# IGNF/StrataNet2-Vegetation-Coverage-Maps

Hardware: AMD Instinct MI355X
Metric: plots/s fwd+bwd, 32k-pt synthetic plots, batch 16/GPU (higher is better)
Workload: dtype f32; 1 GPU; C2 ref-arch: 16 plots/GPU x 32768 pts, SA npoint 1024/256 + global, r 1/2 m, train step fwd+P2+loss+bwd+Adam, inputs resident in HBM; plots_per_gpu=16, points_per_plot=32768, batches_per_geometry_pass=8, exchange=none (single GPU), parallelism=single GPU, ranks_seen=1, exchange_in_graph=False

## Files before the change

include/strata_hip.h:

```cpp
#ifndef STRATA_HIP_H
#define STRATA_HIP_H

#include <stddef.h>

#ifdef __cplusplus
extern "C" {
#endif

#define SN2_VERSION 102
#define SN2_EINVAL (-1)
#define SN2_ELIMIT (-2)

#define SN2_MAX_NEIGHBORS 2000
#define SN2_STAT_SLOTS 1024

int sn2_version(void);
int sn2_debug_mfma_chain(const float *a, const float *b, float *d, int mode, void *stream);
int sn2_debug_spin(int blocks, long long clocks, int *out, void *stream);

int sn2_debug_fp1_backward_parts(int mask);
int sn2_debug_fp_rows_form(int form);
int sn2_debug_fp_table_form(int form);
#define SN2_PROBE_SINK_WORDS 4096
int sn2_debug_stream_probe(const float *src, float *dst, size_t n_floats, int mode, float *sink, void *stream);
int sn2_debug_mfma_probe(int mode, int iters, float *sink, double *flops, void *stream);

typedef struct sn2_block {
    int cin, cout;
    const float *W, *b;
    const float *gamma, *beta;
    float *running_mean, *running_var;
    float *a, *c;
    float *mean, *invstd;
    float *stat_slots;
    float *dW, *db, *dgamma, *dbeta;
    int grad_replicas, grad_replica_stride;
    int mma_bf16;
    long long *num_batches_tracked;
    int frozen_stats;
} sn2_block;
#define SN2_BN_FROZEN_KEEP 2
int sn2_grad_reduce(float *flat, int n, int replicas, int stride, void *stream);


int sn2_pack_rows(const float *cloud, const float *xyz, int B, int C, int N, float *rows0, void *stream);

#define SN2_FPS_WS_WORDS(B, N) (6L * (B) * (N) + (4104L + 4096L) * (B) + 32L)
int sn2_fps(const float *pos_soa, int B, int N, int M, const int *start, int *idx, float *cpos_soa,
            float *cpos_aos, int *order_ws, void *stream);
int sn2_fps_waves(const float *pos_soa, int B, int N, int M, const int *start, int *idx, float *cpos_soa,
                  float *cpos_aos, int *order_ws, int waves, void *stream);
int sn2_fps_status(const float *pos_soa, int B, int N, int M, const int *start, int *idx, float *cpos_soa,
                   float *cpos_aos, int *order_ws, int waves, unsigned *status, void *stream);
int sn2_debug_fps_spin_limit(unsigned sweeps);

int sn2_ball_query(const float *src_soa, int B, int N, const float *cpos_soa, int M, float r2, int cap,
                   int *nbr, int *cnt, unsigned long long *total, const int *fps_ws, void *stream);

int sn2_count_sum(const int *cnt, int n, unsigned long long *total, void *stream);
int sn2_count_sum_group(const int *cnt, int G, int n, unsigned long long *total, size_t total_stride, void *stream);

#define SN2_THREE_NN_WS_WORDS(B, S) ((size_t)(B) * (4 * (size_t)(S) + 1032))
int sn2_three_nn(const float *src_soa, int B, int S, const float *dst_soa, int T, int k, int *idx, float *w,
                 void *ws, const int *dst_fps_ws, void *stream);
#define SN2_THREE_NN_XY_WS_WORDS(B, S, T) ((size_t)(B) * (4 * (size_t)(S) + 5 * (size_t)(T) + 1032))
int sn2_three_nn_xy(const float *src_soa, int B, int S, const float *dst_soa, int T, int k, int *idx, float *w,
                    void *ws, void *stream);

int sn2_prepare_plots(const float *raw, long T, const int *offsets, const float *centers, const float *fake_xy, int n_fake,
                      const int *idx, int B, int N, int train, const double *rot, const int *flips, const float *noise,
                      const long *noise_offsets, long noise_T, float z_max, float *cloud, float *xyz, void *stream);

#define SN2_SUBSAMPLE_LDS 1
#define SN2_SUBSAMPLE_GLOBAL 2
#define SN2_SUBSAMPLE_COARSE 4
#define SN2_SUBSAMPLE_LDS_MAX 16384
int sn2_subsample_form(int n_max, int N);
size_t sn2_subsample_ws_words(int B, int n_max, int N, int form);
int sn2_subsample(const int *offsets, int extra, int n_max, int B, int N, unsigned long long seed, const long long *plot_keys,
                  int form, int *ws, size_t ws_words, int *idx, void *stream);

#define SN2_ZNORM_WS_WORDS(n, cells) ((size_t)5 * (n) + 3 * (size_t)(cells) + 8)
int sn2_znorm(const float *x, const float *y, const float *z, int n, float radius, float x_min, float y_min, float x_max,
              float y_max, int *ws, float *zmin, float *z_out, void *stream);

size_t sn2_parcel_count_ws_words(int P, int rows);
size_t sn2_parcel_znorm_ws_words(long T, float radius, float x_min, float y_min, float x_max, float y_max);
int sn2_parcel_count(const float *cloud, long T, int L, int rows, const float *centers, int P, const int *cell_start,
                     const int *cell_items, int GX, int GY, double gx0, double gy0, double cell_inv, float radius, int *ws,
                     size_t ws_words, int *prefix, long long *total, void *stream);
int sn2_parcel_fill(const float *cloud, long T, int L, int rows, const float *centers, int P, const int *cell_start,
                    const int *cell_items, int GX, int GY, double gx0, double gy0, double cell_inv, float radius, int *prefix,
                    const int *plot_base, long sum_n, float *raw, int *point_index, void *stream);
int sn2_parcel_znorm(const float *cloud, long T, float x_min, float y_min, float x_max, float y_max, float radius,
                     float disc_radius, const int *offsets, const float *centers, int P, const int *point_index, long sum_n,
                     int *ws, size_t ws_words, float *raw, void *stream);

typedef struct sn2_sa {
    int B, Nsrc, M, cap;
    int cf;
    int nl;
    const float *feat; int feat_stride;
    const float *spos; int spos_stride;
    const float *cpos;
    const int *nbr, *cnt;
    const unsigned long long *total;
    const int *order;
    sn2_block blk[2];
    float *ext; int *arg;
    float *out;
    const float *dout;
    float *dfeat;
} sn2_sa;
#define SN2_SA_SOLO_MIN 64
#define SN2_SA_QUAD_MIN 8
#define SN2_SA_OCT_MIN 4
#define SN2_SA_SOLO_FLAG 0x40000000
#define SN2_SA_OCT_FLAG 0x20000000
#define SN2_SA_PACKED_ITEMS(M) ((M) / 8 + 2)
#define SN2_SA_ORDER_WORDS(B, M) ((size_t)4 * (B) * (M) + (size_t)16 * (B) * SN2_SA_PACKED_ITEMS(M) + 8)
int sn2_sa_order(const int *cnt, int B, int M, int *order, void *stream);
int sn2_sa_order_group(const int *cnt, int G, int B, int M, int *order, size_t stride_words, void *stream);
int sn2_sa_forward(const sn2_sa *p, int training, void *stream);
int sn2_sa_backward(const sn2_sa *p, void *stream);

typedef struct sn2_fp {
    int B, R_per_plot, S_per_plot;
    int ca, cb;
    const float *src; int src_stride; const float *src_a, *src_c;
    const int *knn_idx; const float *knn_w;
    const float *skip; int skip_stride;
    sn2_block blk;
    float *h; int h_stride;
    const float *dy;
    float *dsrc; int dsrc_stride;
    float *dskip; int dskip_stride;
    float *du_scratch;
    float *scatter_ws;
    int scatter_ready;
    const int *bn_sums_done;
    float *src_ws;
    int act_bf16;
    const int *row_perm;
} sn2_fp;
#define SN2_INTERP_CHUNKS(R, S) ((3 * (size_t)(R) + 62) / 63 + (size_t)(S))
#define SN2_FP_SRC_WS_WORDS(B, R, S, cout) ((size_t)(B) * SN2_INTERP_CHUNKS(R, S) * ((((cout) + 3) / 4) * 4))
#define SN2_INTERP_WS_WORDS(B, R, S) \
    ((size_t)(B) * (S) * (((R) + 2047) / 2048 + 6) + 6 * (size_t)(B) * (R) + 64 + 4 * (size_t)(B) * SN2_INTERP_CHUNKS(R, S))
int sn2_interp_index(const int *knn_idx, const float *knn_w, const float *src_pos, int B, int R_per_plot,
                     int S_per_plot, float *ws, void *stream);
int sn2_interp_index_perm(const int *knn_idx, const float *knn_w, const float *src_pos, const int *row_perm, int B,
                          int R_per_plot, int S_per_plot, float *ws, void *stream);
int sn2_interp_index_group(const int *knn_idx, const float *knn_w, const float *src_pos, const int *row_perm, int G, int B,
                           int R_per_plot, int S_per_plot, float *ws, size_t ws_stride_words, void *stream);
int sn2_fp_forward(const sn2_fp *p, int training, void *stream);
int sn2_fp_backward(const sn2_fp *p, void *stream);

int sn2_plot_max_forward(const float *h, const float *a, const float *c, int B, int R_per_plot, int C, float *out,
                         int *arg, void *stream);
int sn2_plot_max_backward(const float *dout, const int *arg, int B, int R_per_plot, int C, float *dy, void *stream);

int sn2_global_pool_backward(const float *du, int du_stride, const int *arg, const float *h, const float *mean,
                             const float *invstd, int B, int R_per_plot, int C, float *dx, float *dy, float *dgamma,
                             float *dbeta, void *stream);

#define SN2_GLOBAL_XCHG_WORDS(B) ((size_t)2 * (size_t)(B) * 4 * 128)
#define SN2_GLOBAL_CTL_WORDS 8
int sn2_global_level_forward(const sn2_fp *sa3, const sn2_fp *fp3, float *x3, int *arg3, unsigned long long *xchg,
                             unsigned *ctl, void *stream);
int sn2_debug_global_spin_limit(unsigned sweeps);

typedef struct sn2_head {
    int R, cin, f_stride;
    const float *f, *fa, *fc;
    const float *W1, *b1, *W2, *b2;
    float *coverages, *proba;
    const float *dcoverages, *dproba;
    float *dy;
    float *dW1, *db1, *dW2, *db2;
    int grad_replicas, grad_replica_stride;
    const int *drop_mask;
    float drop_scale;
    int act_bf16;
    float *zero_fill; long zero_fill_words;
} sn2_head;
int sn2_head_forward(const sn2_head *p, void *stream);
int sn2_fp_head_eval(const sn2_fp *p, const sn2_head *hd, void *stream);
int sn2_head_backward(const sn2_head *p, void *stream);
int sn2_head_bn_sums(const sn2_head *p, const float *gamma, const float *beta, const float *mean, const float *invstd,
                     float *dgamma, float *dbeta, int *ok, void *stream);
int sn2_fp_bn_sums(const sn2_fp *p, const float *gamma, const float *beta, const float *mean, const float *invstd,
                   float *dgamma, float *dbeta, int *ok, void *stream);


int sn2_plot_project_forward(const float *pred_pointwise, const float *cloud_xy, long plot_stride, int B, int N,
                             int D, unsigned long long *keys, int *pix, int *arg, int *nocc, float *pred,
                             void *stream);
#define SN2_P2_KEY_PARTS(N) (((N) + 4095) / 4096 < 1 ? 1 : (((N) + 4095) / 4096 > 64 ? 64 : ((N) + 4095) / 4096))
int sn2_plot_pixels(const float *cloud_xy, long plot_stride, int B, int N, int D, float *mm, int *pix, void *stream);
int sn2_plot_project_forward_pix(const float *pred_pointwise, const int *pix, int B, int N, int D,
                                 unsigned long long *keys, int *arg, int *nocc, float *pred, void *stream);
int sn2_plot_project_backward(const float *dpred, const int *arg, const int *nocc, const int *pix, int B, int N,
                              int D, float *dpointwise, void *stream);

int sn2_raster_project(const float *coverages, const float *cloud_xy, long plot_stride, int B, int N, int D,
                       int diam_meters, unsigned long long *keys, int *pix, float *rasters, void *stream);

int sn2_mosaic_merge(const float *rasters, const float *weights, const int *offsets, int B, int D, int H, int W,
                     float *mean, float *wsum, int win_y0, int win_x0, int win_h, int win_w, void *stream);

#define SN2_MOSAIC_HIST_WORDS 10004
int sn2_mosaic_finalize(const float *mean, const float *wsum, int H, int W, int *hist_ws, double *sum_ws, float *thr_out,
                        float *out, void *stream);

int sn2_kde_lookup(const float *cloud, int B, int C, int N, int z_channel, float z_max, const double *X, const double *Y,
                   int K, double *pdf, void *stream);
#define SN2_KDE_FIT_MAX_K 65536
#define SN2_KDE_FIT_ABS_SLOTS 256
#define SN2_KDE_FIT_SLICES 8
#define SN2_KDE_FIT_WS_WORDS(K) \
    (2 * ((4 + 3 * SN2_KDE_FIT_SLICES) * (size_t)(K) + 3 * (((size_t)(K) + 255) / 256)) + SN2_KDE_FIT_ABS_SLOTS)
int sn2_kde_fit(const float *z, long n, double bw, int K, void *ws, double *X, double *Y, void *stream);
#define SN2_LOSS_BLOCKS 1024
int sn2_loss_forward(const float *pred, const double *gt, int B, const float *proba, const double *pdf, int R, double m,
                     double e, double *partials, double *out, void *stream);
int sn2_loss_backward(const float *pred, const double *gt, int B, const float *proba, const double *pdf, int R, double m,
                      double e, const double *grad_total, float *dpred, float *dproba, void *stream);

#define SN2_PROJECTED_LOSS_WS (2 * 512 + 2)
int sn2_projected_loss_forward(const float *coverages, const int *pix, const float *proba, const double *pdf, const double *gt,
                               int B, int N, int D, double m, double e, unsigned long long *keys, int *arg, int *nocc,
                               float *pred, double *partials, double *out, void *stream);
int sn2_projected_loss_backward(const float *pred, const double *gt, int B, const float *proba, const double *pdf, int N, int D,
                                double m, double e, const double *grad_total, const int *arg, const int *nocc, const int *pix,
                                float *dcoverages, float *dproba, void *stream);

#define SN2_PLOT_LOSSES_SLICE_ROWS 2048
#define SN2_PLOT_LOSSES_SLICES(N) \
    (((N) + SN2_PLOT_LOSSES_SLICE_ROWS - 1) / SN2_PLOT_LOSSES_SLICE_ROWS < 1 ? 1 : \
     (((N) + SN2_PLOT_LOSSES_SLICE_ROWS - 1) / SN2_PLOT_LOSSES_SLICE_ROWS > 64 ? 64 : ((N) + SN2_PLOT_LOSSES_SLICE_ROWS - 1) / SN2_PLOT_LOSSES_SLICE_ROWS))
size_t sn2_plot_losses_ws_words(int B, int N, int D);
int sn2_plot_losses(const float *coverages, const int *pix, const float *proba, const double *pdf, const double *gt, int B, int N,
                    int D, double m, double e, void *ws, float *pred, double *out, void *stream);

int sn2_adam_step(float *param, const float *grad, float *exp_avg, float *exp_avg_sq, int n, float lr, float beta1,
                  float beta2, float eps, float weight_decay, int *step_dev ,
                  float grad_scale, void *stream);


typedef struct sn2_net_layer {
    int cin, cout;
    const float *W, *b, *gamma, *beta;
    float *running_mean, *running_var;
    long long *num_batches_tracked;
    int gW, gb, ggamma, gbeta;
    int mma_bf16;
} sn2_net_layer;

typedef struct sn2_net_model {
    sn2_net_layer sa1[2], sa2, sa3, fp3, fp2, fp1;
    const float *lin1_W, *lin1_b, *lin2_W, *lin2_b;
    int g_lin1_W, g_lin1_b, g_lin2_W, g_lin2_b;
    int n_flat;
    float r1_sq, r2_sq;
    int max_neighbors;
    float drop_p;
    int fuse_global_level;
    int fuse_eval_head;
    int source_side;
    int fps_waves_shared, fps_waves_many;
} sn2_net_model;

typedef struct sn2_net_dims {
    int B, N, M1, M2;
    int cap1, cap2;
    int act_bf16;
    int p2_diam_pix;
} sn2_net_dims;

typedef struct sn2_net_geo {
    const float *xyz;
    int *idx1; float *pos1_soa, *pos1_aos; int *ws1;
    int *nbr1, *cnt1; unsigned long long *tot1; int *ord1;
    int *idx2; float *pos2_soa, *pos2_aos; int *ws2;
    int *nbr2, *cnt2; unsigned long long *tot2; int *ord2;
    const float *pos3;
    int *knn3_idx; float *knn3_w;
    int *knn2_idx; float *knn2_w;
    int *knn1_idx; float *knn1_w;
    float *inv3, *inv2, *inv1;
    int *nn_ws2, *nn_ws1;
    const int *rank1;
    float *rows0;
    int *p2_pix; float *p2_mm;
} sn2_net_geo;

typedef struct sn2_net_act {
    float *aux;
    float *stats;
    float *ext1; int *arg1; float *x1;
    float *ext2; int *arg2; float *x2;
    float *h_sa3, *h3;
    float *x3; int *arg3;
    float *h2;
    void *h1;
    float *src_ws1, *src_ws2;
    float *cov, *proba;
    const int *drop_mask;
    float *bwd_arena; long bwd_arena_words;
} sn2_net_act;

typedef struct sn2_net_bwd {
    const float *dcov, *dproba;
    float *arena; long arena_words;
    int images, image_stride;
    float *dy2, *dy3, *dx1, *dx2, *dx3, *dy_sa3;
    void *dy1, *du1;
    float *du2, *du3;
    int *bn_ok;
    float *src_ws1, *src_ws2;
    int defer_grad_reduce;
    int arena_is_zero;
    int frozen_stats;
} sn2_net_bwd;

#define SN2_NET_FORK 1
#define SN2_NET_SHARED 2
#define SN2_NET_INVERTED 4
#define SN2_NET_DEFER_JOIN 8
#define SN2_NET_INPUT_ONLY 16
#define SN2_NET_HAS_ROWS0 32
#define SN2_NET_JOIN_PENDING 64
#define SN2_NET_WITH_GEOMETRY 128
#define SN2_NET_HAS_INVERTED 256

typedef struct sn2_net_io {
    const float *cloud;
    const int *fps_start;
    unsigned *fps_status;
    unsigned long long *gl_xchg; unsigned *gl_ctl;
    void *stream_b, *stream_c, *stream_pack;
    void *ctx;
    int flags;
    int training;
} sn2_net_io;

int sn2_net_ctx_create(void **ctx);
int sn2_net_ctx_destroy(void *ctx);
int sn2_net_geo_carve(const sn2_net_model *m, const sn2_net_dims *d, void *base, sn2_net_geo *out, size_t *bytes);
int sn2_net_act_carve(const sn2_net_model *m, const sn2_net_dims *d, int training, void *base, sn2_net_act *out, size_t *bytes);
int sn2_net_bwd_carve(const sn2_net_model *m, const sn2_net_dims *d, void *arena_base, void *scratch_base, sn2_net_bwd *out,
                      size_t *arena_bytes, size_t *scratch_bytes);
int sn2_net_geometry(const sn2_net_model *m, const sn2_net_dims *d, const sn2_net_geo *g, const sn2_net_io *io, void *stream);
int sn2_net_forward(const sn2_net_model *m, const sn2_net_dims *d, const sn2_net_geo *g, const sn2_net_act *a,
                    const sn2_net_io *io, void *stream);
int sn2_net_backward(const sn2_net_model *m, const sn2_net_dims *d, const sn2_net_geo *g, const sn2_net_act *a,
                     const sn2_net_bwd *b, void *stream);

int sn2_adam_step_images(float *param, float *grad_images, int replicas, int stride, float *exp_avg, float *exp_avg_sq, int n,
                         float lr, float beta1, float beta2, float eps, float weight_decay, int *step_dev, float grad_scale,
                         void *stream);

#ifdef __cplusplus
}
#endif
#endif
```

stratanet2_vegetation_coverage_maps_amd/_lib.py:

```python
import ctypes
import os
from ctypes import POINTER, Structure, c_double, c_float, c_int, c_long, c_longlong, c_void_p

HERE = os.path.dirname(os.path.abspath(__file__))
LIB_PATH = os.path.join(HERE, "csrc", "libstrata_hip.so")

SN2_VERSION = 102
MAX_NEIGHBORS = 2000
STAT_SLOTS = 1024


class Block(Structure):
    _fields_ = [("cin", c_int), ("cout", c_int), ("W", c_void_p), ("b", c_void_p), ("gamma", c_void_p),
                ("beta", c_void_p), ("running_mean", c_void_p), ("running_var", c_void_p), ("a", c_void_p),
                ("c", c_void_p), ("mean", c_void_p), ("invstd", c_void_p), ("stat_slots", c_void_p),
                ("dW", c_void_p), ("db", c_void_p), ("dgamma", c_void_p), ("dbeta", c_void_p),
                ("grad_replicas", c_int), ("grad_replica_stride", c_int), ("mma_bf16", c_int),
                ("num_batches_tracked", c_void_p), ("frozen_stats", c_int)]


BN_FROZEN_KEEP = 2


class SA(Structure):
    _fields_ = [("B", c_int), ("Nsrc", c_int), ("M", c_int), ("cap", c_int), ("cf", c_int), ("nl", c_int),
                ("feat", c_void_p), ("feat_stride", c_int), ("spos", c_void_p), ("spos_stride", c_int),
                ("cpos", c_void_p), ("nbr", c_void_p), ("cnt", c_void_p), ("total", c_void_p), ("order", c_void_p),
                ("blk", Block * 2),
                ("ext", c_void_p), ("arg", c_void_p), ("out", c_void_p), ("dout", c_void_p), ("dfeat", c_void_p)]


class FP(Structure):
    _fields_ = [("B", c_int), ("R_per_plot", c_int), ("S_per_plot", c_int), ("ca", c_int), ("cb", c_int),
                ("src", c_void_p), ("src_stride", c_int), ("src_a", c_void_p), ("src_c", c_void_p),
                ("knn_idx", c_void_p), ("knn_w", c_void_p), ("skip", c_void_p), ("skip_stride", c_int),
                ("blk", Block), ("h", c_void_p), ("h_stride", c_int), ("dy", c_void_p), ("dsrc", c_void_p),
                ("dsrc_stride", c_int), ("dskip", c_void_p), ("dskip_stride", c_int), ("du_scratch", c_void_p),
                ("scatter_ws", c_void_p), ("scatter_ready", c_int), ("bn_sums_done", c_void_p), ("src_ws", c_void_p),
                ("act_bf16", c_int), ("row_perm", c_void_p)]


class Head(Structure):
    _fields_ = [("R", c_int), ("cin", c_int), ("f_stride", c_int), ("f", c_void_p), ("fa", c_void_p),
                ("fc", c_void_p), ("W1", c_void_p), ("b1", c_void_p), ("W2", c_void_p), ("b2", c_void_p),
                ("coverages", c_void_p), ("proba", c_void_p), ("dcoverages", c_void_p), ("dproba", c_void_p),
                ("dy", c_void_p), ("dW1", c_void_p), ("db1", c_void_p), ("dW2", c_void_p), ("db2", c_void_p),
                ("grad_replicas", c_int), ("grad_replica_stride", c_int), ("drop_mask", c_void_p), ("drop_scale", c_float),
                ("act_bf16", c_int), ("zero_fill", c_void_p), ("zero_fill_words", c_long)]


class NetLayer(Structure):
    _fields_ = [("cin", c_int), ("cout", c_int), ("W", c_void_p), ("b", c_void_p), ("gamma", c_void_p), ("beta", c_void_p),
                ("running_mean", c_void_p), ("running_var", c_void_p), ("num_batches_tracked", c_void_p),
                ("gW", c_int), ("gb", c_int), ("ggamma", c_int), ("gbeta", c_int), ("mma_bf16", c_int)]


class NetModel(Structure):
    _fields_ = [("sa1", NetLayer * 2), ("sa2", NetLayer), ("sa3", NetLayer), ("fp3", NetLayer), ("fp2", NetLayer), ("fp1", NetLayer),
                ("lin1_W", c_void_p), ("lin1_b", c_void_p), ("lin2_W", c_void_p), ("lin2_b", c_void_p),
                ("g_lin1_W", c_int), ("g_lin1_b", c_int), ("g_lin2_W", c_int), ("g_lin2_b", c_int), ("n_flat", c_int),
                ("r1_sq", c_float), ("r2_sq", c_float), ("max_neighbors", c_int), ("drop_p", c_float),
                ("fuse_global_level", c_int), ("fuse_eval_head", c_int), ("source_side", c_int),
                ("fps_waves_shared", c_int), ("fps_waves_many", c_int)]


class NetDims(Structure):
    _fields_ = [("B", c_int), ("N", c_int), ("M1", c_int), ("M2", c_int), ("cap1", c_int), ("cap2", c_int), ("act_bf16", c_int),
                ("p2_diam_pix", c_int)]


class NetGeo(Structure):
    _fields_ = [(n, c_void_p) for n in (
        "xyz", "idx1", "pos1_soa", "pos1_aos", "ws1", "nbr1", "cnt1", "tot1", "ord1",
        "idx2", "pos2_soa", "pos2_aos", "ws2", "nbr2", "cnt2", "tot2", "ord2", "pos3",
        "knn3_idx", "knn3_w", "knn2_idx", "knn2_w", "knn1_idx", "knn1_w", "inv3", "inv2", "inv1", "nn_ws2", "nn_ws1",
        "rank1", "rows0", "p2_pix", "p2_mm")]


class NetAct(Structure):
    _fields_ = [(n, c_void_p) for n in (
        "aux", "stats", "ext1", "arg1", "x1", "ext2", "arg2", "x2", "h_sa3", "h3", "x3", "arg3", "h2", "h1", "src_ws1", "src_ws2",
        "cov", "proba", "drop_mask", "bwd_arena")] + [("bwd_arena_words", c_long)]


class NetBwd(Structure):
    _fields_ = [("dcov", c_void_p), ("dproba", c_void_p), ("arena", c_void_p), ("arena_words", c_long), ("images", c_int),
                ("image_stride", c_int)] + [(n, c_void_p) for n in (
                    "dy2", "dy3", "dx1", "dx2", "dx3", "dy_sa3", "dy1", "du1", "du2", "du3", "bn_ok", "src_ws1", "src_ws2")] + [
                        ("defer_grad_reduce", c_int), ("arena_is_zero", c_int), ("frozen_stats", c_int)]


class NetIO(Structure):
    _fields_ = [("cloud", c_void_p), ("fps_start", c_void_p), ("fps_status", c_void_p), ("gl_xchg", c_void_p), ("gl_ctl", c_void_p),
                ("stream_b", c_void_p), ("stream_c", c_void_p), ("stream_pack", c_void_p), ("ctx", c_void_p), ("flags", c_int),
                ("training", c_int)]


NET_FORK, NET_SHARED, NET_INVERTED, NET_DEFER_JOIN, NET_INPUT_ONLY = 1, 2, 4, 8, 16
NET_HAS_ROWS0, NET_JOIN_PENDING, NET_WITH_GEOMETRY, NET_HAS_INVERTED = 32, 64, 128, 256


SIGNATURES = {
    "sn2_version": [],
    "sn2_debug_mfma_chain": [c_void_p, c_void_p, c_void_p, c_int, c_void_p],
    "sn2_debug_spin": [c_int, c_longlong, c_void_p, c_void_p],
    "sn2_debug_fp1_backward_parts": [c_int],
    "sn2_debug_fp_rows_form": [c_int],
    "sn2_debug_fp_table_form": [c_int],
    "sn2_debug_stream_probe": [c_void_p, c_void_p, ctypes.c_size_t, c_int, c_void_p, c_void_p],
    "sn2_debug_mfma_probe": [c_int, c_int, c_void_p, POINTER(c_double), c_void_p],
    "sn2_pack_rows": [c_void_p, c_void_p, c_int, c_int, c_int, c_void_p, c_void_p],
    "sn2_fps": [c_void_p, c_int, c_int, c_int, c_void_p, c_void_p, c_void_p, c_void_p, c_void_p, c_void_p],
    "sn2_fps_waves": [c_void_p, c_int, c_int, c_int, c_void_p, c_void_p, c_void_p, c_void_p, c_void_p, c_int, c_void_p],
    "sn2_fps_status": [c_void_p, c_int, c_int, c_int, c_void_p, c_void_p, c_void_p, c_void_p, c_void_p, c_int, c_void_p, c_void_p],
    "sn2_debug_fps_spin_limit": [ctypes.c_uint],
    "sn2_ball_query": [c_void_p, c_int, c_int, c_void_p, c_int, c_float, c_int, c_void_p, c_void_p, c_void_p, c_void_p,
                       c_void_p],
    "sn2_three_nn": [c_void_p, c_int, c_int, c_void_p, c_int, c_int, c_void_p, c_void_p, c_void_p, c_void_p, c_void_p],
    "sn2_count_sum": [c_void_p, c_int, c_void_p, c_void_p],
    "sn2_count_sum_group": [c_void_p, c_int, c_int, c_void_p, ctypes.c_size_t, c_void_p],
    "sn2_three_nn_xy": [c_void_p, c_int, c_int, c_void_p, c_int, c_int, c_void_p, c_void_p, c_void_p, c_void_p],
    "sn2_prepare_plots": [c_void_p, c_long, c_void_p, c_void_p, c_void_p, c_int, c_void_p, c_int, c_int, c_int, c_void_p,
                          c_void_p, c_void_p, c_void_p, c_long, c_float, c_void_p, c_void_p, c_void_p],
    "sn2_znorm": [c_void_p, c_void_p, c_void_p, c_int, c_float, c_float, c_float, c_float, c_float, c_void_p, c_void_p,
                  c_void_p, c_void_p],
    "sn2_parcel_count": [c_void_p, c_long, c_int, c_int, c_void_p, c_int, c_void_p, c_void_p, c_int, c_int, c_double, c_double,
                         c_double, c_float, c_void_p, ctypes.c_size_t, c_void_p, c_void_p, c_void_p],
    "sn2_parcel_fill": [c_void_p, c_long, c_int, c_int, c_void_p, c_int, c_void_p, c_void_p, c_int, c_int, c_double, c_double,
                        c_double, c_float, c_void_p, c_void_p, c_long, c_void_p, c_void_p, c_void_p],
    "sn2_parcel_znorm": [c_void_p, c_long, c_float, c_float, c_float, c_float, c_float, c_float, c_void_p, c_void_p, c_int,
                         c_void_p, c_long, c_void_p, ctypes.c_size_t, c_void_p, c_void_p],
    "sn2_subsample_form": [c_int, c_int],
    "sn2_subsample": [c_void_p, c_int, c_int, c_int, c_int, ctypes.c_ulonglong, c_void_p, c_int, c_void_p, ctypes.c_size_t,
                      c_void_p, c_void_p],
    "sn2_sa_order": [c_void_p, c_int, c_int, c_void_p, c_void_p],
    "sn2_sa_order_group": [c_void_p, c_int, c_int, c_int, c_void_p, ctypes.c_size_t, c_void_p],
    "sn2_sa_forward": [POINTER(SA), c_int, c_void_p],
    "sn2_sa_backward": [POINTER(SA), c_void_p],
    "sn2_grad_reduce": [c_void_p, c_int, c_int, c_int, c_void_p],
    "sn2_interp_index": [c_void_p, c_void_p, c_void_p, c_int, c_int, c_int, c_void_p, c_void_p],
    "sn2_interp_index_perm": [c_void_p, c_void_p, c_void_p, c_void_p, c_int, c_int, c_int, c_void_p, c_void_p],
    "sn2_interp_index_group": [c_void_p, c_void_p, c_void_p, c_void_p, c_int, c_int, c_int, c_int, c_void_p, ctypes.c_size_t, c_void_p],
    "sn2_fp_forward": [POINTER(FP), c_int, c_void_p],
    "sn2_fp_backward": [POINTER(FP), c_void_p],
    "sn2_plot_max_forward": [c_void_p, c_void_p, c_void_p, c_int, c_int, c_int, c_void_p, c_void_p, c_void_p],
    "sn2_plot_max_backward": [c_void_p, c_void_p, c_int, c_int, c_int, c_void_p, c_void_p],
    "sn2_global_pool_backward": [c_void_p, c_int, c_void_p, c_void_p, c_void_p, c_void_p, c_int, c_int, c_int, c_void_p, c_void_p,
                                 c_void_p, c_void_p, c_void_p],
    "sn2_global_level_forward": [POINTER(FP), POINTER(FP), c_void_p, c_void_p, c_void_p, c_void_p, c_void_p],
    "sn2_debug_global_spin_limit": [ctypes.c_uint],
    "sn2_head_forward": [POINTER(Head), c_void_p],
    "sn2_fp_head_eval": [POINTER(FP), POINTER(Head), c_void_p],
    "sn2_fp_bn_sums": [POINTER(FP), c_void_p, c_void_p, c_void_p, c_void_p, c_void_p, c_void_p, c_void_p, c_void_p],
    "sn2_head_bn_sums": [POINTER(Head), c_void_p, c_void_p, c_void_p, c_void_p, c_void_p, c_void_p, c_void_p, c_void_p],
    "sn2_head_backward": [POINTER(Head), c_void_p],
    "sn2_plot_project_forward": [c_void_p, c_void_p, c_long, c_int, c_int, c_int, c_void_p, c_void_p, c_void_p,
                                 c_void_p, c_void_p, c_void_p],
    "sn2_plot_pixels": [c_void_p, c_long, c_int, c_int, c_int, c_void_p, c_void_p, c_void_p],
    "sn2_plot_project_forward_pix": [c_void_p, c_void_p, c_int, c_int, c_int, c_void_p, c_void_p, c_void_p, c_void_p, c_void_p],
    "sn2_plot_project_backward": [c_void_p, c_void_p, c_void_p, c_void_p, c_int, c_int, c_int, c_void_p, c_void_p],
    "sn2_raster_project": [c_void_p, c_void_p, c_long, c_int, c_int, c_int, c_int, c_void_p, c_void_p, c_void_p,
                           c_void_p],
    "sn2_mosaic_merge": [c_void_p, c_void_p, c_void_p, c_int, c_int, c_int, c_int, c_void_p, c_void_p,
                         c_int, c_int, c_int, c_int, c_void_p],
    "sn2_mosaic_finalize": [c_void_p, c_void_p, c_int, c_int, c_void_p, c_void_p, c_void_p, c_void_p, c_void_p],
    "sn2_kde_lookup": [c_void_p, c_int, c_int, c_int, c_int, c_float, c_void_p, c_void_p, c_int, c_void_p, c_void_p],
    "sn2_kde_fit": [c_void_p, c_long, c_double, c_int, c_void_p, c_void_p, c_void_p, c_void_p],
    "sn2_loss_forward": [c_void_p, c_void_p, c_int, c_void_p, c_void_p, c_int, c_double, c_double, c_void_p, c_void_p,
                         c_void_p],
    "sn2_loss_backward": [c_void_p, c_void_p, c_int, c_void_p, c_void_p, c_int, c_double, c_double, c_void_p, c_void_p,
                          c_void_p, c_void_p],
    "sn2_adam_step": [c_void_p, c_void_p, c_void_p, c_void_p, c_int, c_float, c_float, c_float, c_float, c_float,
                      c_void_p, c_float, c_void_p],
    "sn2_projected_loss_forward": [c_void_p, c_void_p, c_void_p, c_void_p, c_void_p, c_int, c_int, c_int, c_double, c_double, c_void_p,
                                   c_void_p, c_void_p, c_void_p, c_void_p, c_void_p, c_void_p],
    "sn2_projected_loss_backward": [c_void_p, c_void_p, c_int, c_void_p, c_void_p, c_int, c_int, c_double, c_double, c_void_p, c_void_p,
                                    c_void_p, c_void_p, c_void_p, c_void_p, c_void_p],
    "sn2_plot_losses": [c_void_p, c_void_p, c_void_p, c_void_p, c_void_p, c_int, c_int, c_int, c_double, c_double, c_void_p, c_void_p,
                        c_void_p, c_void_p],
    "sn2_adam_step_images": [c_void_p, c_void_p, c_int, c_int, c_void_p, c_void_p, c_int, c_float, c_float, c_float, c_float, c_float,
                             c_void_p, c_float, c_void_p],
    "sn2_net_ctx_create": [POINTER(c_void_p)],
    "sn2_net_ctx_destroy": [c_void_p],
    "sn2_net_geo_carve": [POINTER(NetModel), POINTER(NetDims), c_void_p, POINTER(NetGeo), POINTER(ctypes.c_size_t)],
    "sn2_net_act_carve": [POINTER(NetModel), POINTER(NetDims), c_int, c_void_p, POINTER(NetAct), POINTER(ctypes.c_size_t)],
    "sn2_net_bwd_carve": [POINTER(NetModel), POINTER(NetDims), c_void_p, c_void_p, POINTER(NetBwd), POINTER(ctypes.c_size_t),
                          POINTER(ctypes.c_size_t)],
    "sn2_net_geometry": [POINTER(NetModel), POINTER(NetDims), POINTER(NetGeo), POINTER(NetIO), c_void_p],
    "sn2_net_forward": [POINTER(NetModel), POINTER(NetDims), POINTER(NetGeo), POINTER(NetAct), POINTER(NetIO), c_void_p],
    "sn2_net_backward": [POINTER(NetModel), POINTER(NetDims), POINTER(NetGeo), POINTER(NetAct), POINTER(NetBwd), c_void_p],
}

SIZE_HELPERS = {
    "sn2_parcel_count_ws_words": [c_int, c_int],
    "sn2_parcel_znorm_ws_words": [c_long, c_float, c_float, c_float, c_float, c_float],
    "sn2_subsample_ws_words": [c_int, c_int, c_int, c_int],
    "sn2_plot_losses_ws_words": [c_int, c_int, c_int],
}

_lib = None


class StrataHipError(RuntimeError):
    pass


def load():
    global _lib
    if _lib is not None:
        return _lib
    if not os.path.exists(LIB_PATH):
        raise StrataHipError(
            f"{LIB_PATH} not found: build it with `python -m stratanet2_vegetation_coverage_maps_amd._build` "
            "(or __graft_entry__.build()); the HIP library is mandatory, there is no fallback path")
    lib = ctypes.CDLL(LIB_PATH)
    for name, argtypes in SIGNATURES.items():
        fn = getattr(lib, name)
        fn.argtypes = argtypes
        fn.restype = c_int
    for name, argtypes in SIZE_HELPERS.items():
        fn = getattr(lib, name)
        fn.argtypes = argtypes
        fn.restype = ctypes.c_size_t
    if lib.sn2_version() != SN2_VERSION:
        raise StrataHipError(f"libstrata_hip.so version {lib.sn2_version()} != binding {SN2_VERSION}: rebuild")
    _lib = lib
    return lib


def check(rc: int, what: str):
    if rc != 0:
        kind = "hipError_t" if rc > 0 else {-1: "SN2_EINVAL", -2: "SN2_ELIMIT"}.get(rc, "error")
        raise StrataHipError(f"{what} failed: {kind} {rc}")
```

stratanet2_vegetation_coverage_maps_amd/csrc/net.hip:

```cpp
#include "common.h"

#include <cstring>
#include <new>

namespace {

constexpr int WIDTHS[7] = {16, 16, 32, 64, 64, 34, 34};
constexpr int WIDTH_SUM = 260;
constexpr int GRAD_IMAGES = 32;

struct NetCtx {
    hipEvent_t fork, b_tables, b_nn, b_done, c_nn, c_done, pack_fork, packed;
};

inline long rows_stat_limit() { return 64L * SN2_STAT_SLOTS; }

inline bool fps_fills_ws(int B, int N, int m) {
    const bool many_small = N <= 4096 && B > 32;
    return N > 2048 && !many_small && m > 16 && ((long)B * N) % 4 == 0 && N <= 131072;
}
inline bool three_nn_uses_grid(int S, int T) { return S >= 128 && S <= 8192 && T > 2048; }
inline bool fp_src_ws_wanted(const sn2_net_model* m, long R, int cb, bool force) {
    return m->source_side && cb > 0 && cb <= 16 && cb % 4 == 0 && (R > rows_stat_limit() || force);
}

struct Carver {
    uintptr_t base;
    size_t off = 0;
    explicit Carver(void* b) : base(reinterpret_cast<uintptr_t>(b)) {}
    template <class T>
    T* take(size_t n_elems) {
        off = (off + 255) & ~(size_t)255;
        T* p = reinterpret_cast<T*>(base + off);
        off += n_elems * sizeof(T);
        return p;
    }
    size_t bytes() const { return (off + 255) & ~(size_t)255; }
};

int check_dims(const sn2_net_model* m, const sn2_net_dims* d) {
    if (!m || !d) return SN2_EINVAL;
    if (d->B <= 0 || d->N <= 0 || d->M1 <= 0 || d->M2 <= 0 || d->M1 > d->N || d->M2 > d->M1) return SN2_EINVAL;
    if (m->max_neighbors <= 0) return SN2_EINVAL;
    const int c1 = m->max_neighbors < d->N ? m->max_neighbors : d->N, c2 = m->max_neighbors < d->M1 ? m->max_neighbors : d->M1;
    if (d->cap1 != c1 || d->cap2 != c2) return SN2_EINVAL;
    if ((long)d->B * d->N >= (1L << 31) / 64) return SN2_ELIMIT;
    const int cin[7] = {11, 16, 19, 35, 96, 80, 42};
    const sn2_net_layer* L[7] = {&m->sa1[0], &m->sa1[1], &m->sa2, &m->sa3, &m->fp3, &m->fp2, &m->fp1};
    for (int i = 0; i < 7; ++i)
        if (L[i]->cin != cin[i] || L[i]->cout != WIDTHS[i]) return SN2_ELIMIT;
    return 0;
}

int check_model_ptrs(const sn2_net_model* m) {
    const sn2_net_layer* L[7] = {&m->sa1[0], &m->sa1[1], &m->sa2, &m->sa3, &m->fp3, &m->fp2, &m->fp1};
    for (int i = 0; i < 7; ++i)
        if (!L[i]->W || !L[i]->b || !L[i]->gamma || !L[i]->beta || !L[i]->running_mean || !L[i]->running_var) return SN2_EINVAL;
    if (!m->lin1_W || !m->lin1_b || !m->lin2_W || !m->lin2_b) return SN2_EINVAL;
    return 0;
}

struct GradDst {
    float* flat;
    int stride;
    int frozen;
};

void fill_block(sn2_block* blk, const sn2_net_layer* L, int k, const sn2_net_act* a, GradDst g) {
    int aux_off = 0, st_off = 0;
    for (int i = 0; i < k; ++i) aux_off += 4 * WIDTHS[i], st_off += SN2_STAT_SLOTS * 2 * WIDTHS[i];
    const int c = L->cout;
    blk->cin = L->cin, blk->cout = c;
    blk->W = L->W, blk->b = L->b, blk->gamma = L->gamma, blk->beta = L->beta;
    blk->running_mean = L->running_mean, blk->running_var = L->running_var;
    float* aux = a->aux + aux_off;
    blk->a = aux, blk->c = aux + c, blk->mean = aux + 2 * c, blk->invstd = aux + 3 * c;
    blk->stat_slots = a->stats + st_off;
    blk->mma_bf16 = L->mma_bf16 ? 1 : 0;
    blk->num_batches_tracked = L->num_batches_tracked;
    blk->frozen_stats = g.frozen;
    if (g.flat) {
        blk->dW = g.flat + L->gW, blk->db = g.flat + L->gb, blk->dgamma = g.flat + L->ggamma, blk->dbeta = g.flat + L->gbeta;
        blk->grad_replicas = GRAD_IMAGES, blk->grad_replica_stride = g.stride;
    } else {
        blk->dW = blk->db = blk->dgamma = blk->dbeta = nullptr;
        blk->grad_replicas = 1, blk->grad_replica_stride = 0;
    }
}

inline float* aux_row(const sn2_net_act* a, int k, int row) {
    int off = 0;
    for (int i = 0; i < k; ++i) off += 4 * WIDTHS[i];
    return a->aux + off + row * WIDTHS[k];
}

void sa1_desc(sn2_sa* s, const sn2_net_model* m, const sn2_net_dims* d, const sn2_net_geo* g, const sn2_net_act* a,
              GradDst gd, const float* dout) {
    memset(s, 0, sizeof(*s));
    s->B = d->B, s->Nsrc = d->N, s->M = d->M1, s->cap = d->cap1, s->cf = 8, s->nl = 2;
    s->feat = g->rows0, s->feat_stride = 12, s->spos = g->rows0 + 8, s->spos_stride = 12;
    s->cpos = g->pos1_aos, s->nbr = g->nbr1, s->cnt = g->cnt1, s->total = g->tot1, s->order = g->ord1;
    fill_block(&s->blk[0], &m->sa1[0], 0, a, gd);
    fill_block(&s->blk[1], &m->sa1[1], 1, a, gd);
    s->ext = a->ext1, s->arg = a->arg1, s->out = a->x1;
    s->dout = dout, s->dfeat = nullptr;
}
void sa2_desc(sn2_sa* s, const sn2_net_model* m, const sn2_net_dims* d, const sn2_net_geo* g, const sn2_net_act* a,
              GradDst gd, const float* dout, float* dfeat) {
    memset(s, 0, sizeof(*s));
    s->B = d->B, s->Nsrc = d->M1, s->M = d->M2, s->cap = d->cap2, s->cf = 16, s->nl = 1;
    s->feat = a->x1, s->feat_stride = 16, s->spos = g->pos1_aos, s->spos_stride = 4;
    s->cpos = g->pos2_aos, s->nbr = g->nbr2, s->cnt = g->cnt2, s->total = g->tot2, s->order = g->ord2;
    fill_block(&s->blk[0], &m->sa2, 2, a, gd);
    s->ext = a->ext2, s->arg = a->arg2, s->out = a->x2;
    s->dout = dout, s->dfeat = dfeat;
}

struct FpIn {
    int k;
    const sn2_net_layer* L;
    int Rp, Sp, ca, cb;
    const float* src; int src_stride; const float *src_a, *src_c;
    const int* knn_idx; const float* knn_w;
    const float* skip; int skip_stride;
    void* h;
    float* src_ws;
    int act_bf16;
};
void fp_desc(sn2_fp* p, const sn2_net_dims* d, const sn2_net_act* a, const FpIn& in, GradDst gd) {
    memset(p, 0, sizeof(*p));
    p->B = d->B, p->R_per_plot = in.Rp, p->S_per_plot = in.Sp, p->ca = in.ca, p->cb = in.cb;
    p->src = in.src, p->src_stride = in.src_stride, p->src_a = in.src_a, p->src_c = in.src_c;
    p->knn_idx = in.knn_idx, p->knn_w = in.knn_w;
    p->skip = in.cb > 0 ? in.skip : nullptr, p->skip_stride = in.cb > 0 ? in.skip_stride : 0;
    fill_block(&p->blk, in.L, in.k, a, gd);
    if ((long)d->B * in.Rp > rows_stat_limit()) p->blk.mma_bf16 = 0;
    p->h = static_cast<float*>(in.h), p->h_stride = (in.L->cout + 3) / 4 * 4;
    p->src_ws = in.src_ws;
    p->act_bf16 = in.act_bf16;
}

FpIn sa3_in(const sn2_net_model* m, const sn2_net_dims* d, const sn2_net_geo* g, const sn2_net_act* a) {
    FpIn in{};
    in.k = 3, in.L = &m->sa3, in.Rp = d->M2, in.Sp = d->M2, in.ca = 32, in.cb = 3;
    in.src = a->x2, in.src_stride = 32;
    in.skip = g->pos2_aos, in.skip_stride = 4;
    in.h = a->h_sa3;
    return in;
}
FpIn fp3_in(const sn2_net_model* m, const sn2_net_dims* d, const sn2_net_geo* g, const sn2_net_act* a) {
    FpIn in{};
    in.k = 4, in.L = &m->fp3, in.Rp = d->M2, in.Sp = 1, in.ca = 64, in.cb = 32;
    in.src = a->x3, in.src_stride = 64;
    in.knn_idx = g->knn3_idx, in.knn_w = g->knn3_w;
    in.skip = a->x2, in.skip_stride = 32;
    in.h = a->h3;
    return in;
}
FpIn fp2_in(const sn2_net_model* m, const sn2_net_dims* d, const sn2_net_geo* g, const sn2_net_act* a, float* src_ws) {
    FpIn in{};
    in.k = 5, in.L = &m->fp2, in.Rp = d->M1, in.Sp = d->M2, in.ca = 64, in.cb = 16;
    in.src = a->h3, in.src_stride = 64, in.src_a = aux_row(a, 4, 0), in.src_c = aux_row(a, 4, 1);
    in.knn_idx = g->knn2_idx, in.knn_w = g->knn2_w;
    in.skip = a->x1, in.skip_stride = 16;
    in.h = a->h2;
    in.src_ws = src_ws;
    return in;
}
FpIn fp1_in(const sn2_net_model* m, const sn2_net_dims* d, const sn2_net_geo* g, const sn2_net_act* a, float* src_ws) {
    FpIn in{};
    in.k = 6, in.L = &m->fp1, in.Rp = d->N, in.Sp = d->M1, in.ca = 34, in.cb = 8;
    in.src = a->h2, in.src_stride = 36, in.src_a = aux_row(a, 5, 0), in.src_c = aux_row(a, 5, 1);
    in.knn_idx = g->knn1_idx, in.knn_w = g->knn1_w;
    in.skip = g->rows0, in.skip_stride = 12;
    in.h = a->h1;
    in.src_ws = src_ws;
    in.act_bf16 = d->act_bf16;
    return in;
}

void head_desc(sn2_head* h, const sn2_net_model* m, const sn2_net_dims* d, const sn2_net_act* a, int training) {
    memset(h, 0, sizeof(*h));
    h->R = d->B * d->N, h->cin = 34, h->f_stride = 36;
    h->f = static_cast<const float*>(a->h1), h->fa = aux_row(a, 6, 0), h->fc = aux_row(a, 6, 1);
    h->W1 = m->lin1_W, h->b1 = m->lin1_b, h->W2 = m->lin2_W, h->b2 = m->lin2_b;
    h->coverages = a->cov, h->proba = a->proba;
    h->grad_replicas = 1, h->grad_replica_stride = 0;
    h->act_bf16 = d->act_bf16;
    if (training && a->drop_mask) {
        h->drop_mask = a->drop_mask;
        h->drop_scale = m->drop_p < 1.f ? 1.f / (1.f - m->drop_p) : 0.f;
    } else {
        h->drop_mask = nullptr, h->drop_scale = 1.f;
    }
}

#define NET_HIP(expr)                                         \
    do {                                                      \
        hipError_t e__ = (expr);                              \
        if (e__ != hipSuccess) return (int)e__;               \
    } while (0)

int inverted_tables(const sn2_net_dims* d, const sn2_net_geo* g, int which, void* st) {
    if (which == 3) {
        SN2_TRY(sn2_count_sum(g->cnt1, d->B * d->M1, g->tot1, st));
        SN2_TRY(sn2_count_sum(g->cnt2, d->B * d->M2, g->tot2, st));
    }
    if (which & 1) {
        if (!g->inv3 || !g->inv2) return SN2_EINVAL;
        SN2_TRY(sn2_interp_index_perm(g->knn3_idx, g->knn3_w, nullptr, nullptr, d->B, d->M2, 1, g->inv3, st));
        SN2_TRY(sn2_interp_index_perm(g->knn2_idx, g->knn2_w, nullptr, nullptr, d->B, d->M1, d->M2, g->inv2, st));
    }
    if (which & 2) {
        if (!g->inv1) return SN2_EINVAL;
        SN2_TRY(sn2_interp_index_perm(g->knn1_idx, g->knn1_w, g->pos1_aos, g->rank1, d->B, d->N, d->M1, g->inv1, st));
    }
    return 0;
}

int check_geo(const sn2_net_dims* d, const sn2_net_geo* g) {
    if (!g || !g->xyz || !g->idx1 || !g->pos1_soa || !g->pos1_aos || !g->nbr1 || !g->cnt1 || !g->tot1 || !g->ord1 || !g->idx2 ||
        !g->pos2_soa || !g->pos2_aos || !g->nbr2 || !g->cnt2 || !g->tot2 || !g->ord2 || !g->pos3 || !g->knn3_idx || !g->knn3_w ||
        !g->knn2_idx || !g->knn2_w || !g->knn1_idx || !g->knn1_w || !g->rows0)
        return SN2_EINVAL;
    return 0;
}
int check_geo_workspaces(const sn2_net_dims* d, const sn2_net_geo* g) {
    if (three_nn_uses_grid(d->M2, d->M1) && !g->nn_ws2) return SN2_EINVAL;
    if (three_nn_uses_grid(d->M1, d->N) && !g->nn_ws1) return SN2_EINVAL;
    return 0;
}

int three_nn_any(const float* src, int B, int S, const float* dst, int T, int k, int* idx, float* w, int* ws, void* st) {
    if (three_nn_uses_grid(S, T)) return sn2_three_nn_xy(src, B, S, dst, T, k, idx, w, ws, st);
    return sn2_three_nn(src, B, S, dst, T, k, idx, w, nullptr, nullptr, st);
}

int geometry_impl(const sn2_net_model* m, const sn2_net_dims* d, const sn2_net_geo* g, const sn2_net_io* io, int flags,
                  hipStream_t cur) {
    const int B = d->B, N = d->N, M1 = d->M1, M2 = d->M2;
    NetCtx* ctx = static_cast<NetCtx*>(io->ctx);
    const bool fork = (flags & SN2_NET_FORK) && ctx && io->stream_b && io->stream_c;
    const bool inverted = flags & SN2_NET_INVERTED;
    const int* start0 = io->fps_start;
    const int* start1 = io->fps_start ? io->fps_start + B : nullptr;
    int* ws1 = fps_fills_ws(B, N, M1) ? g->ws1 : nullptr;
    int* ws2 = fps_fills_ws(B, M1, M2) ? g->ws2 : nullptr;
    int waves = 0;
    if (flags & SN2_NET_SHARED) waves = B > 32 ? m->fps_waves_many : m->fps_waves_shared;
    SN2_TRY(sn2_fps_status(g->xyz, B, N, M1, start0, g->idx1, g->pos1_soa, g->pos1_aos, ws1, waves, io->fps_status, cur));
    hipStream_t sb = cur, sc = cur;
    if (fork) {
        sb = (hipStream_t)io->stream_b, sc = (hipStream_t)io->stream_c;
        NET_HIP(hipEventRecord(ctx->fork, cur));
        NET_HIP(hipStreamWaitEvent(sb, ctx->fork, 0));
        NET_HIP(hipStreamWaitEvent(sc, ctx->fork, 0));
    }
    SN2_TRY(sn2_fps_status(g->pos1_soa, B, M1, M2, start1, g->idx2, g->pos2_soa, g->pos2_aos, ws2, 0, io->fps_status, sb));
    SN2_TRY(sn2_ball_query(g->pos1_soa, B, M1, g->pos2_soa, M2, m->r2_sq, d->cap2, g->nbr2, g->cnt2, inverted ? g->tot2 : nullptr, ws2, sb));
    SN2_TRY(sn2_sa_order(g->cnt2, B, M2, g->ord2, sb));
    if (fork) NET_HIP(hipEventRecord(ctx->b_tables, sb));
    SN2_TRY(sn2_three_nn(g->pos3, B, 1, g->pos2_soa, M2, 1, g->knn3_idx, g->knn3_w, nullptr, nullptr, sb));
    SN2_TRY(three_nn_any(g->pos2_soa, B, M2, g->pos1_soa, M1, 3, g->knn2_idx, g->knn2_w, g->nn_ws2, sb));
    if (fork) NET_HIP(hipEventRecord(ctx->b_nn, sb));
    if (inverted) SN2_TRY(inverted_tables(d, g, 1, sb));
    SN2_TRY(three_nn_any(g->pos1_soa, B, M1, g->xyz, N, 3, g->knn1_idx, g->knn1_w, g->nn_ws1, sc));
    if (fork) NET_HIP(hipEventRecord(ctx->c_nn, sc));
    if (inverted) SN2_TRY(inverted_tables(d, g, 2, sc));
    if (flags & SN2_NET_INPUT_ONLY) {
        if (!io->cloud) return SN2_EINVAL;
        SN2_TRY(sn2_pack_rows(io->cloud, g->xyz, B, 10, N, g->rows0, cur));
        if (d->p2_diam_pix > 0 && g->p2_pix && g->p2_mm)
            SN2_TRY(sn2_plot_pixels(io->cloud, 10L * N, B, N, d->p2_diam_pix, g->p2_mm, g->p2_pix, cur));
    }
    SN2_TRY(sn2_ball_query(g->xyz, B, N, g->pos1_soa, M1, m->r1_sq, d->cap1, g->nbr1, g->cnt1, inverted ? g->tot1 : nullptr, ws1, cur));
    SN2_TRY(sn2_sa_order(g->cnt1, B, M1, g->ord1, cur));
    if (fork) {
        NET_HIP(hipEventRecord(ctx->b_done, sb));
        NET_HIP(hipEventRecord(ctx->c_done, sc));
        if (!(flags & SN2_NET_DEFER_JOIN)) {
            NET_HIP(hipStreamWaitEvent(cur, ctx->b_done, 0));
            NET_HIP(hipStreamWaitEvent(cur, ctx->c_done, 0));
        }
    }
    return 0;
}

}

extern "C" int sn2_net_ctx_create(void** out) {
    if (!out) return SN2_EINVAL;
    NetCtx* c = new (std::nothrow) NetCtx();
    if (!c) return SN2_EINVAL;
    hipEvent_t* ev[8] = {&c->fork, &c->b_tables, &c->b_nn, &c->b_done, &c->c_nn, &c->c_done, &c->pack_fork, &c->packed};
    for (int i = 0; i < 8; ++i) {
        hipError_t e = hipEventCreateWithFlags(ev[i], hipEventDisableTiming);
        if (e != hipSuccess) {
            for (int j = 0; j < i; ++j) (void)hipEventDestroy(*ev[j]);
            delete c;
            return (int)e;
        }
    }
    *out = c;
    return 0;
}

extern "C" int sn2_net_ctx_destroy(void* ctx) {
    if (!ctx) return SN2_EINVAL;
    NetCtx* c = static_cast<NetCtx*>(ctx);
    (void)hipEventDestroy(c->fork);
    (void)hipEventDestroy(c->b_tables);
    (void)hipEventDestroy(c->b_nn);
    (void)hipEventDestroy(c->b_done);
    (void)hipEventDestroy(c->c_nn);
    (void)hipEventDestroy(c->c_done);
    (void)hipEventDestroy(c->pack_fork);
    (void)hipEventDestroy(c->packed);
    delete c;
    return 0;
}

extern "C" int sn2_net_geo_carve(const sn2_net_model* m, const sn2_net_dims* d, void* base, sn2_net_geo* g, size_t* bytes) {
    SN2_TRY(check_dims(m, d));
    if (!g || !bytes) return SN2_EINVAL;
    const size_t B = d->B, N = d->N, M1 = d->M1, M2 = d->M2;
    memset(g, 0, sizeof(*g));
    Carver c(base);
    g->idx1 = c.take<int>(B * M1), g->pos1_soa = c.take<float>(B * 3 * M1), g->pos1_aos = c.take<float>(B * M1 * 4);
    g->ws1 = fps_fills_ws(d->B, d->N, d->M1) ? c.take<int>((size_t)SN2_FPS_WS_WORDS(B, N)) : nullptr;
    g->nbr1 = c.take<int>(B * M1 * (size_t)d->cap1), g->cnt1 = c.take<int>(B * M1);
    g->tot1 = c.take<unsigned long long>(1), g->ord1 = c.take<int>(SN2_SA_ORDER_WORDS(B, M1));
    g->idx2 = c.take<int>(B * M2), g->pos2_soa = c.take<float>(B * 3 * M2), g->pos2_aos = c.take<float>(B * M2 * 4);
    g->ws2 = fps_fills_ws(d->B, d->M1, d->M2) ? c.take<int>((size_t)SN2_FPS_WS_WORDS(B, M1)) : nullptr;
    g->nbr2 = c.take<int>(B * M2 * (size_t)d->cap2), g->cnt2 = c.take<int>(B * M2);
    g->tot2 = c.take<unsigned long long>(1), g->ord2 = c.take<int>(SN2_SA_ORDER_WORDS(B, M2));
    g->knn3_idx = c.take<int>(B * M2 * 3), g->knn3_w = c.take<float>(B * M2 * 3);
    g->knn2_idx = c.take<int>(B * M1 * 3), g->knn2_w = c.take<float>(B * M1 * 3);
    g->knn1_idx = c.take<int>(B * N * 3), g->knn1_w = c.take<float>(B * N * 3);
    g->inv3 = c.take<float>(SN2_INTERP_WS_WORDS(B, M2, 1));
    g->inv2 = c.take<float>(SN2_INTERP_WS_WORDS(B, M1, M2));
    g->inv1 = c.take<float>(SN2_INTERP_WS_WORDS(B, N, M1));
    g->nn_ws2 = three_nn_uses_grid(d->M2, d->M1) ? c.take<int>(SN2_THREE_NN_XY_WS_WORDS(B, M2, M1)) : nullptr;
    g->nn_ws1 = three_nn_uses_grid(d->M1, d->N) ? c.take<int>(SN2_THREE_NN_XY_WS_WORDS(B, M1, N)) : nullptr;
    g->rows0 = c.take<float>(B * N * 12);
    if (d->p2_diam_pix > 0) g->p2_pix = c.take<int>(B * N), g->p2_mm = c.take<float>(B * 4);
    *bytes = c.bytes();
    return 0;
}

extern "C" int sn2_net_act_carve(const sn2_net_model* m, const sn2_net_dims* d, int training, void* base, sn2_net_act* a,
                                 size_t* bytes) {
    SN2_TRY(check_dims(m, d));
    if (!a || !bytes) return SN2_EINVAL;
    const size_t B = d->B, N = d->N, M1 = d->M1, M2 = d->M2;
    memset(a, 0, sizeof(*a));
    Carver c(base);
    a->aux = c.take<float>(4 * WIDTH_SUM), a->stats = c.take<float>((size_t)SN2_STAT_SLOTS * 2 * WIDTH_SUM);
    a->ext1 = c.take<float>(B * M1 * 16), a->arg1 = c.take<int>(B * M1 * 16), a->x1 = c.take<float>(B * M1 * 16);
    a->ext2 = c.take<float>(B * M2 * 32), a->arg2 = c.take<int>(B * M2 * 32), a->x2 = c.take<float>(B * M2 * 32);
    a->h_sa3 = c.take<float>(B * M2 * 64), a->h3 = c.take<float>(B * M2 * 64);
    a->x3 = c.take<float>(B * 64), a->arg3 = c.take<int>(B * 64);
    a->h2 = c.take<float>(B * M1 * 36);
    const bool fused_eval = !training && m->fuse_eval_head && !d->act_bf16 && m->source_side;
    if (!fused_eval) a->h1 = d->act_bf16 ? (void*)c.take<unsigned short>(B * N * 36) : (void*)c.take<float>(B * N * 36);
    if (fp_src_ws_wanted(m, (long)B * N, 8, fused_eval)) a->src_ws1 = c.take<float>(SN2_FP_SRC_WS_WORDS(B, N, M1, 34));
    if (fp_src_ws_wanted(m, (long)B * M1, 16, false)) a->src_ws2 = c.take<float>(SN2_FP_SRC_WS_WORDS(B, M1, M2, 34));
    *bytes = c.bytes();
    return 0;
}

extern "C" int sn2_net_bwd_carve(const sn2_net_model* m, const sn2_net_dims* d, void* arena_base, void* scratch_base,
                                 sn2_net_bwd* b, size_t* arena_bytes, size_t* scratch_bytes) {
    SN2_TRY(check_dims(m, d));
    if (!b || !arena_bytes || !scratch_bytes || m->n_flat <= 0) return SN2_EINVAL;
    const size_t B = d->B, N = d->N, M1 = d->M1, M2 = d->M2;
    memset(b, 0, sizeof(*b));
    const size_t stride = ((size_t)m->n_flat + 63) / 64 * 64;
    float* ar = static_cast<float*>(arena_base);
    size_t o = GRAD_IMAGES * stride;
    auto take = [&](size_t n) {
        float* p = ar + o;
        o += (n + 3) / 4 * 4;
        return p;
    };
    b->arena = ar, b->images = GRAD_IMAGES, b->image_stride = (int)stride;
    b->dy2 = take(B * M1 * 36), b->dy3 = take(B * M2 * 64), b->dx1 = take(B * M1 * 16), b->dx2 = take(B * M2 * 32);
    b->dx3 = take(B * 64), b->dy_sa3 = take(B * M2 * 64);
    b->arena_words = (long)o;
    *arena_bytes = o * sizeof(float);
    Carver c(scratch_base);
    if (d->act_bf16) {
        b->dy1 = c.take<unsigned short>(B * N * 36), b->du1 = c.take<unsigned short>(B * N * 36);
    } else {
        b->dy1 = c.take<float>(B * N * 36), b->du1 = c.take<float>(B * N * 36);
    }
    b->du2 = c.take<float>(B * M1 * 64), b->du3 = c.take<float>(B * M2 * 64);
    b->bn_ok = c.take<int>(4);
    if (fp_src_ws_wanted(m, (long)B * N, 8, false)) b->src_ws1 = c.take<float>(SN2_FP_SRC_WS_WORDS(B, N, M1, 34));
    if (fp_src_ws_wanted(m, (long)B * M1, 16, false)) b->src_ws2 = c.take<float>(SN2_FP_SRC_WS_WORDS(B, M1, M2, 34));
    *scratch_bytes = c.bytes();
    return 0;
}

extern "C" int sn2_net_geometry(const sn2_net_model* m, const sn2_net_dims* d, const sn2_net_geo* g, const sn2_net_io* io,
                                void* stream) {
    SN2_TRY(check_dims(m, d));
    if (!io) return SN2_EINVAL;
    SN2_TRY(check_geo(d, g));
    SN2_TRY(check_geo_workspaces(d, g));
    if ((io->flags & SN2_NET_INVERTED) && (!g->inv1 || !g->inv2 || !g->inv3)) return SN2_EINVAL;
    return geometry_impl(m, d, g, io, io->flags, (hipStream_t)stream);
}

extern "C" int sn2_net_forward(const sn2_net_model* m, const sn2_net_dims* d, const sn2_net_geo* g, const sn2_net_act* a,
                               const sn2_net_io* io, void* stream) {
    SN2_TRY(check_dims(m, d));
    SN2_TRY(check_model_ptrs(m));
    if (!io || !a) return SN2_EINVAL;
    SN2_TRY(check_geo(d, g));
    if (!a->aux || !a->stats || !a->ext1 || !a->arg1 || !a->x1 || !a->ext2 || !a->arg2 || !a->x2 || !a->h_sa3 || !a->h3 || !a->x3 ||
        !a->arg3 || !a->h2 || !a->cov || !a->proba)
        return SN2_EINVAL;
    if (io->training < 0 || io->training > SN2_BN_FROZEN_KEEP) return SN2_EINVAL;
    const int mode = io->training, training = mode != 0 ? 1 : 0, batch_stats = mode == 1 ? 1 : 0, flags = io->flags;
    const int B = d->B, N = d->N, M2 = d->M2;
    hipStream_t cur = (hipStream_t)stream;
    NetCtx* ctx = static_cast<NetCtx*>(io->ctx);
    const bool fused_eval = !training && m->fuse_eval_head && !d->act_bf16 && m->source_side;
    if (!fused_eval && !a->h1) return SN2_EINVAL;
    if (training && !(g->inv1 && g->inv2 && g->inv3)) return SN2_EINVAL;
    const GradDst nograd{nullptr, 0, 0};
    bool join_b = false, join_c = false, wait_pack = false;
    bool have_rows0 = flags & SN2_NET_HAS_ROWS0;
    if (flags & SN2_NET_WITH_GEOMETRY) {
        if (!io->cloud) return SN2_EINVAL;
        SN2_TRY(check_geo_workspaces(d, g));
        int gflags = (flags & (SN2_NET_FORK | SN2_NET_SHARED)) | (training ? SN2_NET_INVERTED : 0);
        const bool fork = (flags & SN2_NET_FORK) && ctx && io->stream_b && io->stream_c;
        if (fork) {
            gflags |= SN2_NET_DEFER_JOIN;
            if (io->stream_pack && !have_rows0) {
                hipStream_t sp = (hipStream_t)io->stream_pack;
                NET_HIP(hipEventRecord(ctx->pack_fork, cur));
                NET_HIP(hipStreamWaitEvent(sp, ctx->pack_fork, 0));
                SN2_TRY(sn2_pack_rows(io->cloud, g->xyz, B, 10, N, g->rows0, sp));
                NET_HIP(hipEventRecord(ctx->packed, sp));
                wait_pack = have_rows0 = true;
            }
        } else {
            gflags &= ~SN2_NET_FORK;
        }
        SN2_TRY(geometry_impl(m, d, g, io, gflags, cur));
        join_b = join_c = fork;
    } else {
        if (flags & SN2_NET_JOIN_PENDING) {
            if (!ctx) return SN2_EINVAL;
            join_b = join_c = true;
        }
        if (training && !(flags & SN2_NET_HAS_INVERTED)) {
            if (join_b) NET_HIP(hipStreamWaitEvent(cur, ctx->b_done, 0));
            if (join_c) NET_HIP(hipStreamWaitEvent(cur, ctx->c_done, 0));
            join_b = join_c = false;
            SN2_TRY(inverted_tables(d, g, 3, cur));
        }
    }
    if (wait_pack) NET_HIP(hipStreamWaitEvent(cur, ctx->packed, 0));
    if (!have_rows0) {
        if (!io->cloud) return SN2_EINVAL;
        SN2_TRY(sn2_pack_rows(io->cloud, g->xyz, B, 10, N, g->rows0, cur));
    }
    sn2_sa sa;
    sa1_desc(&sa, m, d, g, a, nograd, nullptr);
    SN2_TRY(sn2_sa_forward(&sa, mode, cur));
    if (join_b) NET_HIP(hipStreamWaitEvent(cur, ctx->b_tables, 0));
    sa2_desc(&sa, m, d, g, a, nograd, nullptr, nullptr);
    SN2_TRY(sn2_sa_forward(&sa, mode, cur));
    if (join_b) NET_HIP(hipStreamWaitEvent(cur, ctx->b_nn, 0));
    sn2_fp p3, pf3;
    fp_desc(&p3, d, a, sa3_in(m, d, g, a), nograd);
    fp_desc(&pf3, d, a, fp3_in(m, d, g, a), nograd);
    if (batch_stats && m->fuse_global_level && io->gl_xchg && io->gl_ctl && B <= GL_MAX_PLOTS && !m->sa3.mma_bf16 &&
        !m->fp3.mma_bf16) {
        SN2_TRY(sn2_global_level_forward(&p3, &pf3, a->x3, a->arg3, io->gl_xchg, io->gl_ctl, cur));
    } else {
        SN2_TRY(sn2_fp_forward(&p3, mode, cur));
        SN2_TRY(sn2_plot_max_forward(a->h_sa3, p3.blk.a, p3.blk.c, B, M2, 64, a->x3, a->arg3, cur));
        SN2_TRY(sn2_fp_forward(&pf3, mode, cur));
    }
    sn2_fp p2;
    fp_desc(&p2, d, a, fp2_in(m, d, g, a, a->src_ws2), nograd);
    SN2_TRY(sn2_fp_forward(&p2, mode, cur));
    if (join_c) NET_HIP(hipStreamWaitEvent(cur, ctx->c_nn, 0));
    sn2_fp p1;
    sn2_head hd;
    if (fused_eval) {
        if (!a->src_ws1) return SN2_EINVAL;
        sn2_net_act a2 = *a;
        a2.h1 = nullptr;
        fp_desc(&p1, d, &a2, fp1_in(m, d, g, &a2, a->src_ws1), nograd);
        head_desc(&hd, m, d, &a2, 0);
        SN2_TRY(sn2_fp_head_eval(&p1, &hd, cur));
    } else {
        fp_desc(&p1, d, a, fp1_in(m, d, g, a, a->src_ws1), nograd);
        SN2_TRY(sn2_fp_forward(&p1, mode, cur));
        head_desc(&hd, m, d, a, batch_stats);
        if (training && a->bwd_arena && a->bwd_arena_words > 0) hd.zero_fill = a->bwd_arena, hd.zero_fill_words = a->bwd_arena_words;
        SN2_TRY(sn2_head_forward(&hd, cur));
    }
    if (join_b) NET_HIP(hipStreamWaitEvent(cur, ctx->b_done, 0));
    if (join_c) NET_HIP(hipStreamWaitEvent(cur, ctx->c_done, 0));
    return 0;
}

extern "C" int sn2_net_backward(const sn2_net_model* m, const sn2_net_dims* d, const sn2_net_geo* g, const sn2_net_act* a,
                                const sn2_net_bwd* b, void* stream) {
    SN2_TRY(check_dims(m, d));
    SN2_TRY(check_model_ptrs(m));
    if (!a || !b) return SN2_EINVAL;
    SN2_TRY(check_geo(d, g));
    if (!g->inv1 || !g->inv2 || !g->inv3) return SN2_EINVAL;
    if (!a->aux || !a->stats || !a->h1 || !a->h2 || !a->h3 || !a->h_sa3 || !a->x3 || !a->arg3) return SN2_EINVAL;
    if (!b->arena || b->images != GRAD_IMAGES || b->image_stride < m->n_flat || !b->dy1 || !b->du1 || !b->du2 || !b->du3 || !b->bn_ok ||
        !b->dy2 || !b->dy3 || !b->dx1 || !b->dx2 || !b->dx3 || !b->dy_sa3 || b->arena_words <= 0)
        return SN2_EINVAL;
    const int B = d->B, M2 = d->M2;
    hipStream_t cur = (hipStream_t)stream;
    if (!b->arena_is_zero) {
        sn2_fill_words(b->arena, 0u, (size_t)b->arena_words, cur);
        NET_HIP(hipGetLastError());
    }
    const GradDst gd{b->arena, b->image_stride, b->frozen_stats ? 1 : 0};
    sn2_head hd;
    head_desc(&hd, m, d, a, b->frozen_stats ? 0 : 1);
    hd.coverages = hd.proba = nullptr;
    hd.dcoverages = b->dcov, hd.dproba = b->dproba, hd.dy = static_cast<float*>(b->dy1);
    hd.dW1 = b->arena + m->g_lin1_W, hd.db1 = b->arena + m->g_lin1_b, hd.dW2 = b->arena + m->g_lin2_W, hd.db2 = b->arena + m->g_lin2_b;
    hd.grad_replicas = GRAD_IMAGES, hd.grad_replica_stride = b->image_stride;
    SN2_TRY(sn2_head_backward(&hd, cur));
    SN2_TRY(sn2_head_bn_sums(&hd, m->fp1.gamma, m->fp1.beta, aux_row(a, 6, 2), aux_row(a, 6, 3), b->arena + m->fp1.ggamma,
                             b->arena + m->fp1.gbeta, b->bn_ok + 0, cur));
    sn2_fp p1;
    fp_desc(&p1, d, a, fp1_in(m, d, g, a, b->src_ws1), gd);
    p1.dy = static_cast<const float*>(b->dy1), p1.dsrc = b->dy2, p1.dsrc_stride = 36, p1.dskip = nullptr, p1.dskip_stride = 0;
    p1.du_scratch = static_cast<float*>(b->du1), p1.scatter_ws = g->inv1, p1.scatter_ready = 1, p1.bn_sums_done = b->bn_ok + 0;
    p1.row_perm = (g->rank1 && p1.src_ws) ? g->rank1 : nullptr;
    SN2_TRY(sn2_fp_backward(&p1, cur));
    SN2_TRY(sn2_fp_bn_sums(&p1, m->fp2.gamma, m->fp2.beta, aux_row(a, 5, 2), aux_row(a, 5, 3), b->arena + m->fp2.ggamma,
                           b->arena + m->fp2.gbeta, b->bn_ok + 1, cur));
    sn2_fp p2;
    fp_desc(&p2, d, a, fp2_in(m, d, g, a, b->src_ws2), gd);
    p2.dy = b->dy2, p2.dsrc = b->dy3, p2.dsrc_stride = 64, p2.dskip = b->dx1, p2.dskip_stride = 16;
    p2.du_scratch = b->du2, p2.scatter_ws = g->inv2, p2.scatter_ready = 1, p2.bn_sums_done = b->bn_ok + 1;
    SN2_TRY(sn2_fp_backward(&p2, cur));
    SN2_TRY(sn2_fp_bn_sums(&p2, m->fp3.gamma, m->fp3.beta, aux_row(a, 4, 2), aux_row(a, 4, 3), b->arena + m->fp3.ggamma,
                           b->arena + m->fp3.gbeta, b->bn_ok + 2, cur));
    sn2_fp pf3;
    fp_desc(&pf3, d, a, fp3_in(m, d, g, a), gd);
    pf3.dy = b->dy3, pf3.dsrc = b->dx3, pf3.dsrc_stride = 64, pf3.dskip = b->dx2, pf3.dskip_stride = 32;
    pf3.du_scratch = b->du3, pf3.scatter_ws = g->inv3, pf3.scatter_ready = -1, pf3.bn_sums_done = b->bn_ok + 2;
    SN2_TRY(sn2_fp_backward(&pf3, cur));
    SN2_TRY(sn2_global_pool_backward(b->du3, 64, a->arg3, a->h_sa3, aux_row(a, 3, 2), aux_row(a, 3, 3), B, M2, 64, b->dx3, b->dy_sa3,
                                     b->arena + m->sa3.ggamma, b->arena + m->sa3.gbeta, cur));
    sn2_fp p3;
    fp_desc(&p3, d, a, sa3_in(m, d, g, a), gd);
    p3.dy = b->dy_sa3, p3.dsrc = b->dx2, p3.dsrc_stride = 32, p3.bn_sums_done = b->bn_ok + 3;
    SN2_TRY(sn2_fp_backward(&p3, cur));
    sn2_sa sa;
    sa2_desc(&sa, m, d, g, a, gd, b->dx2, b->dx1);
    SN2_TRY(sn2_sa_backward(&sa, cur));
    sa1_desc(&sa, m, d, g, a, gd, b->dx1);
    SN2_TRY(sn2_sa_backward(&sa, cur));
    if (b->defer_grad_reduce) return 0;
    return sn2_grad_reduce(b->arena, m->n_flat, GRAD_IMAGES, b->image_stride, cur);
}
```

stratanet2_vegetation_coverage_maps_amd/csrc/sa.hip:

```cpp
#include "mlp.h"

template <int CF, int NL, int C1, int C2, int PASS>
int sa_mfma_launch_fwd(const sn2_sa* p, int training, hipStream_t st, int* nblocks_out);
template <int CF, int NL, int C1, int C2, int PASS>
int sa_mfma_launch_bwd(const sn2_sa* p, hipStream_t st);

namespace {


__global__ __launch_bounds__(256) void sa_bwd_prep_kernel(const float* __restrict__ dout, const float* __restrict__ ext,
                                                          const int* __restrict__ arg, const float* __restrict__ mean,
                                                          const float* __restrict__ invstd, int rows, int C,
                                                          float* __restrict__ dgamma, float* __restrict__ dbeta) {
    const int o = threadIdx.x % C, g = threadIdx.x / C, G = 256 / C;
    float sb = 0.f, sg = 0.f;
    const float mu = mean[o], is = invstd[o];
    const int step = gridDim.x * G;
    for (int r0 = blockIdx.x * G + g; g < G && r0 < rows; r0 += 8 * step) {
        int ar[8];
        float dv[8], ev[8];
#pragma unroll
        for (int u = 0; u < 8; ++u) {
            const int r = r0 + u * step;
            const size_t i = (size_t)(r < rows ? r : r0) * C + o;
            ar[u] = r < rows ? arg[i] : -1;
            dv[u] = dout[i];
            ev[u] = ext[i];
        }
#pragma unroll
        for (int u = 0; u < 8; ++u)
            if (ar[u] >= 0) {
                sb += dv[u];
                sg = fmaf(dv[u], (ev[u] - mu) * is, sg);
            }
    }
    __shared__ float s_red[128];
    for (int i = threadIdx.x; i < 2 * C; i += 256) s_red[i] = 0.f;
    __syncthreads();
    if (g < G) {
        atomicAdd(&s_red[o], sb);
        atomicAdd(&s_red[C + o], sg);
    }
    __syncthreads();
    if (threadIdx.x < 2 * C) {
        const float v = s_red[threadIdx.x];
        if (v != 0.f) atomicAdd(threadIdx.x < C ? &dbeta[threadIdx.x] : &dgamma[threadIdx.x - C], v);
    }
}

int check(const sn2_sa* p) {
    if (!p || p->B <= 0 || p->Nsrc <= 0 || p->M <= 0 || p->cap <= 0) return SN2_EINVAL;
    if (!p->feat || !p->spos || !p->cpos || !p->nbr || !p->cnt || !p->total || !p->ext || !p->arg || !p->out)
        return SN2_EINVAL;
    if (p->feat_stride < p->cf || (p->feat_stride & 3) || p->spos_stride < 4 || (p->spos_stride & 3)) return SN2_EINVAL;
    const bool sa1 = p->cf == 8 && p->nl == 2 && p->blk[0].cin == 11 && p->blk[0].cout == 16 && p->blk[1].cin == 16 &&
                     p->blk[1].cout == 16;
    const bool sa2 = p->cf == 16 && p->nl == 1 && p->blk[0].cin == 19 && p->blk[0].cout == 32;
    const bool sa3 = p->cf == 32 && p->nl == 1 && p->blk[0].cin == 35 && p->blk[0].cout == 64;
    return (sa1 || sa2 || sa3) ? 0 : SN2_ELIMIT;
}

template <int CF, int NL, int C1, int C2>
int forward_t(const sn2_sa* p, int training, hipStream_t st) {
    const sn2_block* last = &p->blk[NL - 1];
    int nb = 0;
    const int batch_stats = training == 1;
    if constexpr (NL == 2) {
        if (batch_stats) SN2_TRY((sa_mfma_launch_fwd<CF, NL, C1, C2, 0>(p, training, st, &nb)));
        SN2_TRY(sn2_bn_finalize(&p->blk[0], nb, p->total, 0, batch_stats, st));
    }
    if (!training) {
        SN2_TRY(sn2_bn_finalize(last, 0, p->total, 0, 0, st));
        return sa_mfma_launch_fwd<CF, NL, C1, C2, 1>(p, 0, st, &nb);
    }
    SN2_TRY((sa_mfma_launch_fwd<CF, NL, C1, C2, 1>(p, training, st, &nb)));
    return sn2_bn_finalize_apply(last, batch_stats ? nb : 0, p->total, 0, batch_stats, p->ext, p->arg, p->out, (long)p->B * p->M, st);
}

template <int CF, int NL, int C1, int C2>
int backward_t(const sn2_sa* p, hipStream_t st) {
    const sn2_block* last = &p->blk[NL - 1];
    const int rows = p->B * p->M, C = last->cout;
    int pb = sn2_cdiv(rows, 256 / C);
    if (pb > 256) pb = 256;
    hipLaunchKernelGGL(sa_bwd_prep_kernel, dim3(pb), dim3(256), 0, st, p->dout, p->ext, p->arg, last->mean, last->invstd,
                       rows, C, last->dgamma, last->dbeta);
    if constexpr (NL == 2) SN2_TRY((sa_mfma_launch_bwd<CF, NL, C1, C2, 2>(p, st)));
    SN2_TRY((sa_mfma_launch_bwd<CF, NL, C1, C2, 3>(p, st)));
    return 0;
}

}

namespace {
__global__ __launch_bounds__(1024) void sa_order_sort_kernel(const int* __restrict__ cnt, int B, int M, int P2,
                                                             int* __restrict__ order_all, size_t stride) {
    extern __shared__ __attribute__((aligned(16))) unsigned s_key[];
    __shared__ int s_n[3];
    const int bg = blockIdx.x, tid = threadIdx.x, NT = (int)blockDim.x;
    const int hb = bg / B, b = bg - hb * B;
    int* __restrict__ order = order_all + (size_t)hb * stride;
    const int* cb = cnt + (size_t)bg * M;
    if (tid < 3) s_n[tid] = 0;
    __syncthreads();
    int n_here[3] = {0, 0, 0};
    for (int i = tid; i < P2; i += NT) {
        unsigned key = 0xFFFFFFFFu;
        if (i < M) {
            const int c = cb[i];
            key = ((unsigned)(0x3FFFF - c) << 14) | (unsigned)i;
            n_here[0] += c > SN2_SA_SOLO_MIN ? 1 : 0;
            n_here[1] += (c > SN2_SA_QUAD_MIN && c <= SN2_SA_SOLO_MIN) ? 1 : 0;
            n_here[2] += (c > SN2_SA_OCT_MIN && c <= SN2_SA_QUAD_MIN) ? 1 : 0;
        }
        s_key[i] = key;
    }
#pragma unroll
    for (int k = 0; k < 3; ++k)
        if (n_here[k]) atomicAdd(&s_n[k], n_here[k]);
    __syncthreads();
    for (int k = 2; k <= P2; k <<= 1) {
        for (int j = k >> 1; j > 0; j >>= 1) {
            for (int t = tid; t < (P2 >> 1); t += NT) {
                const int lo = ((t & ~(j - 1)) << 1) | (t & (j - 1)), hi = lo | j;
                const unsigned a = s_key[lo], c = s_key[hi];
                const bool up = (lo & k) == 0;
                if ((a > c) == up) {
                    s_key[lo] = c;
                    s_key[hi] = a;
                }
            }
            __syncthreads();
        }
    }
    const int nsolo = s_n[0], r_oct = nsolo + s_n[1], r_hex = r_oct + s_n[2];
    const int items_a = nsolo + ((s_n[1] + 3) >> 2), n_oct_items = (s_n[2] + 7) >> 3, n_hex_items = (M - r_hex + 15) >> 4;
    int* packed = order + (size_t)4 * B * M;
    for (int r = tid; r < M; r += NT) {
        const int id = b * M + (int)(s_key[r] & 0x3FFFu);
        if (r < nsolo) {
            int* dst = order + 4 * ((size_t)r * B + b);
            dst[0] = dst[1] = dst[2] = dst[3] = id | SN2_SA_SOLO_FLAG;
        } else if (r < r_oct) {
            const int rl = r - nsolo;
            order[4 * ((size_t)(nsolo + (rl >> 2)) * B + b) + (rl & 3)] = id;
        } else if (r < r_hex) {
            const int rl = r - r_oct;
            int* dst = packed + 16 * ((size_t)(rl >> 3) * B + b) + 2 * (rl & 7);
            dst[0] = dst[1] = id | SN2_SA_OCT_FLAG;
        } else {
            const int rl = r - r_hex;
            packed[16 * ((size_t)(n_oct_items + (rl >> 4)) * B + b) + (rl & 15)] = id;
        }
    }
    if (tid == 0) {
        int* trailer = packed + (size_t)16 * B * SN2_SA_PACKED_ITEMS(M);
        atomicMax(&trailer[0], items_a);
        atomicMax(&trailer[1], n_oct_items + n_hex_items);
    }
}
}

static int sa_order_impl(const int* cnt, int G, int B, int M, int* order, size_t stride, hipStream_t st);
extern "C" int sn2_sa_order(const int* cnt, int B, int M, int* order, void* stream) {
    if (!cnt || !order || B <= 0 || M <= 0) return SN2_EINVAL;
    return sa_order_impl(cnt, 1, B, M, order, SN2_SA_ORDER_WORDS(B, M), (hipStream_t)stream);
}
extern "C" int sn2_sa_order_group(const int* cnt, int G, int B, int M, int* order, size_t stride_words, void* stream) {
    if (!cnt || !order || G <= 0 || B <= 0 || M <= 0 || stride_words < SN2_SA_ORDER_WORDS(B, M)) return SN2_EINVAL;
    return sa_order_impl(cnt, G, B, M, order, stride_words, (hipStream_t)stream);
}
static int sa_order_impl(const int* cnt, int G, int B, int M, int* order, size_t stride, hipStream_t st) {
    if (M > 16384) return SN2_ELIMIT;
    sn2_fill_words(order, 0xFFFFFFFFu, (size_t)(G - 1) * stride + (size_t)SN2_SA_ORDER_WORDS(B, M), st);
    int P2 = 2;
    while (P2 < M) P2 <<= 1;
    if ((size_t)P2 * 4 > 48 * 1024)
        (void)hipFuncSetAttribute(reinterpret_cast<const void*>(&sa_order_sort_kernel),
                                  hipFuncAttributeMaxDynamicSharedMemorySize, P2 * 4);
    hipLaunchKernelGGL(sa_order_sort_kernel, dim3(G * B), dim3(sn2_small_sort_wg(B) ? 256 : 1024), (size_t)P2 * 4, st, cnt, B, M, P2,
                       order, stride);
    SN2_RETURN_LAUNCH();
}

extern "C" int sn2_sa_forward(const sn2_sa* p, int training, void* stream) {
    SN2_TRY(check(p));
    if (training < 0 || training > SN2_BN_FROZEN_KEEP) return SN2_EINVAL;
    if (p->nl == 2) return forward_t<8, 2, 16, 16>(p, training, (hipStream_t)stream);
    if (p->cf == 32) return forward_t<32, 1, 64, 64>(p, training, (hipStream_t)stream);
    return forward_t<16, 1, 32, 32>(p, training, (hipStream_t)stream);
}

extern "C" int sn2_sa_backward(const sn2_sa* p, void* stream) {
    SN2_TRY(check(p));
    if (!p->dout) return SN2_EINVAL;
    if (p->nl == 2) return backward_t<8, 2, 16, 16>(p, (hipStream_t)stream);
    if (p->cf == 32) return backward_t<32, 1, 64, 64>(p, (hipStream_t)stream);
    return backward_t<16, 1, 32, 32>(p, (hipStream_t)stream);
}
```

stratanet2_vegetation_coverage_maps_amd/csrc/sa_mfma.hip:

```cpp
#include "mlp.h"

namespace {

struct SaFwdArgs {
    int B, Nsrc, M, cap, feat_stride, spos_stride, group;
    const float *feat, *spos, *cpos;
    const int *nbr, *cnt, *order;
    const float *W0, *b0, *a0, *c0, *gamma0;
    const float *W1, *b1, *gamma1;
    float *slots;
    float* ext;
    int* arg;
    const float *al, *cl;
    float* out;
};

__device__ __forceinline__ float row_max(float v) {
    v = fmaxf(v, __int_as_float(SN2_DPP(__float_as_int(v), 0xB1, 0xF)));
    v = fmaxf(v, __int_as_float(SN2_DPP(__float_as_int(v), 0x4E, 0xF)));
    v = fmaxf(v, __int_as_float(SN2_DPP(__float_as_int(v), 0x141, 0xF)));
    v = fmaxf(v, __int_as_float(SN2_DPP(__float_as_int(v), 0x140, 0xF)));
    return v;
}
__device__ __forceinline__ unsigned row_min_u32(unsigned v) {
// ... 239 lines not shown
#pragma unroll
                    for (int r = 0; r < 4; ++r) acc[r] = fmaxf(acc[r], 0.f);
                    D1[io][t] = acc;
                }
            }
            if constexpr (PASS == 0) {
#pragma unroll
                for (int io = 0; io < TO1; ++io)
#pragma unroll
                    for (int t = 0; t < 4; ++t)
#pragma unroll
                        for (int r = 0; r < 4; ++r) {
                            const float h = val[t] ? D1[io][t][r] : 0.f;
                            ssum[io][r] += h;
                            ssq[io][r] = fmaf(h, h, ssq[io][r]);
                        }
            } else {
                f32x4 DL[TOL][4];
                if constexpr (NL == 2) {
#pragma unroll
                    for (int is = 0; is < TO1; ++is)
#pragma unroll
                        for (int t = 0; t < 4; ++t)
#pragma unroll
                            for (int r = 0; r < 4; ++r) D1[is][t][r] = fmaf(a1v[is][r], D1[is][t][r], c1v[is][r]);
#pragma unroll
                    for (int io = 0; io < TO2; ++io)
#pragma unroll
                        for (int t = 0; t < 4; ++t) {
                            f32x4 acc = {bias2[io][0], bias2[io][1], bias2[io][2], bias2[io][3]};
                            acc = contract<BF16, 4 * TO1>(acc, [&](int kk) { return A2[io][kk >> 2][kk & 3]; },
                                                          [&](int kk) { return D1[kk >> 2][t][kk & 3]; });
#pragma unroll
                            for (int r = 0; r < 4; ++r) acc[r] = fmaxf(acc[r], 0.f);
                            DL[io][t] = acc;
                        }
                } else {
#pragma unroll
                    for (int io = 0; io < TOL; ++io)
#pragma unroll
                        for (int t = 0; t < 4; ++t) DL[io][t] = D1[io][t];
                }
#pragma unroll
                for (int io = 0; io < TOL; ++io)
#pragma unroll
                    for (int t = 0; t < 4; ++t) {
                        const int e = e0 + it.le0 + it.eoff * t;
#pragma unroll
                        for (int r = 0; r < 4; ++r) {
                            if constexpr (STATS) {
                                const float h = val[t] ? DL[io][t][r] : 0.f;
                                ssum[io][r] += h;
                                ssq[io][r] = fmaf(h, h, ssq[io][r]);
                            }
                            const float s = sgn[io][r] * DL[io][t][r];
                            if constexpr (STATS) {
                                if (val[t] && s > best[t][io][r]) {
                                    best[t][io][r] = s;
                                    barg[t][io][r] = e;
                                }
                            } else {
                                best[t][io][r] = fmaxf(best[t][io][r], val[t] ? s : -INFINITY);
                            }
                        }
                    }
            }
        }
        if constexpr (PASS == 1) {
            if (it.solo) {
#pragma unroll
                for (int t = 1; t < 4; ++t)
#pragma unroll
                    for (int io = 0; io < TOL; ++io)
#pragma unroll
                        for (int r = 0; r < 4; ++r) {
                            if constexpr (STATS) {
                                const bool take = best[t][io][r] > best[0][io][r] ||
                                                  (best[t][io][r] == best[0][io][r] && barg[t][io][r] < barg[0][io][r]);
                                best[0][io][r] = take ? best[t][io][r] : best[0][io][r];
                                barg[0][io][r] = take ? barg[t][io][r] : barg[0][io][r];
                            } else {
                                best[0][io][r] = fmaxf(best[0][io][r], best[t][io][r]);
                            }
                        }
            }
            const int W = it.W;
            const bool writer = (c & (W - 1)) == 0;
#pragma unroll
            for (int t = 0; t < 4; ++t) {
                if (it.solo && t > 0) continue;
#pragma unroll
                for (int io = 0; io < TOL; ++io) {
                    float ev[4];
                    int av[4];
#pragma unroll
                    for (int r = 0; r < 4; ++r) {
                        const float m = seg_max(best[t][io][r], W);
                        ev[r] = it.ln[t] > 0 ? sgn[io][r] * m : 0.f;
                        if constexpr (STATS) {
                            const unsigned am = seg_min_u32(best[t][io][r] == m ? (unsigned)barg[t][io][r] : 0xFFFFFFFFu, W);
                            av[r] = it.ln[t] > 0 ? (int)am : -1;
                        } else {
                            av[r] = 0;
                            ev[r] = it.ln[t] > 0 ? fmaf(alv[io][r], ev[r], clv[io][r]) : 0.f;
                        }
                    }
                    if (writer && it.ln[t] >= 0) {
                        const size_t o = (size_t)it.lc[t] * CL + 16 * io + 4 * q;
                        if constexpr (STATS) {
                            *reinterpret_cast<float4*>(a.ext + o) = make_float4(ev[0], ev[1], ev[2], ev[3]);
                            *reinterpret_cast<int4*>(a.arg + o) = make_int4(av[0], av[1], av[2], av[3]);
                        } else {
                            *reinterpret_cast<float4*>(a.out + o) = make_float4(ev[0], ev[1], ev[2], ev[3]);
                        }
                    }
                }
            }
        }
    }

    if (STATS && a.slots) {
        const int wv = threadIdx.x >> 6;
        for (int i = threadIdx.x; i < 4 * 2 * CS; i += 256) (&s_red[0][0])[i] = 0.f;
        __syncthreads();
#pragma unroll
        for (int io = 0; io < TOS; ++io)
#pragma unroll
            for (int r = 0; r < 4; ++r) {
                const float s1 = row_sum(ssum[io][r]), s2 = row_sum(ssq[io][r]);
                if (c == 0) {
                    s_red[wv][16 * io + 4 * q + r] = s1;
                    s_red[wv][CS + 16 * io + 4 * q + r] = s2;
                }
            }
        __syncthreads();
        for (int i = threadIdx.x; i < 2 * CS; i += 256)
            a.slots[(size_t)blockIdx.x * 2 * CS + i] = (s_red[0][i] + s_red[1][i]) + (s_red[2][i] + s_red[3][i]);
    }
}


struct SaBwdArgs {
    int B, Nsrc, M, cap, feat_stride, spos_stride, group, frozen;
    const float *feat, *spos, *cpos;
    const int *nbr, *cnt, *order;
    const unsigned long long* total;
    const float *W0, *b0, *a0, *c0, *gamma0, *mean0, *invstd0, *dgamma0, *dbeta0;
    const float *W1, *b1, *gamma1, *mean1, *invstd1, *dgamma1, *dbeta1;
    const float* dout;
    const int* arg;
    float *dW0, *db0, *dW1, *db1, *dgamma0_out, *dbeta0_out;
    int rep_k, rep_stride;
    float* dfeat;
};

#ifdef SN2_SA_STAMPS
__device__ unsigned long long g_sa_dbg[4096 * 10];
extern "C" int sn2_debug_sa_stamps(unsigned long long* out) {
    return (int)hipMemcpyFromSymbol(out, HIP_SYMBOL(g_sa_dbg), sizeof(g_sa_dbg));
}
#define SASTAMP(i)                                                                                  \
    if (CF == 8 && PASS == 3 && (threadIdx.x & 63) == 0 && wave < 4096) {                              \
        unsigned long long t_;                                                                      \
        asm volatile("s_memtime %0\n\ts_waitcnt lgkmcnt(0)" : "=s"(t_)::"memory");                   \
        g_sa_dbg[wave * 10 + (i)] = t_;                                                              \
    }
#define SACOUNT(i, v) if (CF == 8 && PASS == 3 && (threadIdx.x & 63) == 0 && wave < 4096) g_sa_dbg[wave * 10 + (i)] = (v);
#else
#define SASTAMP(i)
#define SACOUNT(i, v)
#endif

template <int CF, int NL, int C1, int C2, int PASS, bool BF16>
__global__ __launch_bounds__(256) void sa_mfma_bwd_kernel(const SaBwdArgs a) {
    constexpr int CIN = CF + 3, KB1 = CF / 4 + 1, TO1 = C1 / 16, TO2 = C2 / 16;
    constexpr bool LAST2 = NL == 2 && PASS == 2;
    constexpr int PO = LAST2 ? C2 : C1;
    constexpr int QK = LAST2 ? C1 : CIN + 1;
    using Acc = OuterAcc<PO, QK>;
    constexpr int PS = Acc::PS, QS = Acc::QS, TP = Acc::TO, TQ = Acc::TK;
    extern __shared__ __attribute__((aligned(16))) float smem[];
    const int lane = threadIdx.x & 63, q = lane >> 4, c = lane & 15;
    const int wib = threadIdx.x >> 6;
    const int wave = __builtin_amdgcn_readfirstlane((int)(blockIdx.x * 4 + wib));
    const int nwaves = gridDim.x * 4;
    const int ncent = a.B * a.M;
    const SaFirst first = sa_first(a.order, a.cnt, a.B, a.M, wave);
    float* lds_p = smem + wib * Acc::LDS_FLOATS;
    float* lds_q = lds_p + 64 * PS;
    SASTAMP(0);
    for (int i = lane; i < Acc::LDS_FLOATS; i += 64) lds_p[i] = 0.f;

    const unsigned long long etot = *a.total;
    const float invE = (etot > 0 && !a.frozen) ? (float)(1.0 / (double)etot) : 0.f;

    float A1[TO1][KB1], bias1[TO1][4];
#pragma unroll
    for (int io = 0; io < TO1; ++io) {
#pragma unroll
        for (int kb = 0; kb < KB1; ++kb) {
            const int k = 4 * kb + q, o = 16 * io + c;
            A1[io][kb] = k < CIN ? a.W0[o * CIN + k] : ((k == CIN && !BF16) ? a.b0[o] : 0.f);
        }
#pragma unroll
        for (int r = 0; r < 4; ++r) bias1[io][r] = BF16 ? a.b0[16 * io + 4 * q + r] : 0.f;
    }
    float A2[NL == 2 ? TO2 : 1][TO1][4], A2T[TO1][NL == 2 ? TO2 : 1][4], bias2[NL == 2 ? TO2 : 1][4], a1v[TO1][4], c1v[TO1][4];
    float cA0[TO1][4], cC0[TO1][4], cD0[TO1][4], mu0[TO1][4], is0[TO1][4];
    float cA1[NL == 2 ? TO2 : 1][4], cC1[NL == 2 ? TO2 : 1][4], cD1[NL == 2 ? TO2 : 1][4];
#pragma unroll
    for (int is = 0; is < TO1; ++is)
#pragma unroll
        for (int r = 0; r < 4; ++r) {
            const int ch = 16 * is + 4 * q + r;
            mu0[is][r] = a.mean0[ch];
            is0[is][r] = a.invstd0[ch];
            a1v[is][r] = NL == 2 ? a.a0[ch] : 0.f;
            c1v[is][r] = NL == 2 ? a.c0[ch] : 0.f;
            if (NL == 1 || PASS == 3) {
                const float g = a.gamma0[ch], dg = a.dgamma0[ch], db = a.dbeta0[ch], m = mu0[is][r], s = is0[is][r];
                cA0[is][r] = g * s;
                cC0[is][r] = g * s * s * dg * invE;
                cD0[is][r] = g * s * (m * s * dg - db) * invE;
            } else {
                cA0[is][r] = cC0[is][r] = cD0[is][r] = 0.f;
            }
        }
    if constexpr (NL == 2) {
#pragma unroll
        for (int io = 0; io < TO2; ++io) {
#pragma unroll
            for (int is = 0; is < TO1; ++is)
#pragma unroll
                for (int kb = 0; kb < 4; ++kb) {
                    A2[io][is][kb] = a.W1[(16 * io + c) * C1 + 16 * is + 4 * q + kb];
                    A2T[is][io][kb] = a.W1[(16 * io + 4 * q + kb) * C1 + 16 * is + c];
                }
#pragma unroll
            for (int r = 0; r < 4; ++r) {
                const int ch = 16 * io + 4 * q + r;
                bias2[io][r] = a.b1[ch];
                const float g = a.gamma1[ch], dg = a.dgamma1[ch], db = a.dbeta1[ch], m = a.mean1[ch], s = a.invstd1[ch];
                cA1[io][r] = g * s;
                cC1[io][r] = g * s * s * dg * invE;
                cD1[io][r] = g * s * (m * s * dg - db) * invE;
            }
        }
    }
    constexpr int TF = CF / 16 > 0 ? CF / 16 : 1;
    float A0T[TF][TO1][4];
    if (PASS == 3 && a.dfeat) {
#pragma unroll
        for (int kt = 0; kt < TF; ++kt)
#pragma unroll
            for (int io = 0; io < TO1; ++io)
#pragma unroll
                for (int kb = 0; kb < 4; ++kb) {
                    const int k = 16 * kt + c;
                    A0T[kt][io][kb] = k < CF ? a.W0[(16 * io + 4 * q + kb) * CIN + k] : 0.f;
                }
    }

    f32x4 acc[TP][TQ];
#pragma unroll
    for (int i = 0; i < TP; ++i)
#pragma unroll
        for (int j = 0; j < TQ; ++j) acc[i][j] = f32x4{0.f, 0.f, 0.f, 0.f};
    float dbias[LAST2 ? TO2 : 1][4], dbe0[TO1][4], dga0[TO1][4];
#pragma unroll
    for (int i = 0; i < (LAST2 ? TO2 : 1); ++i)
#pragma unroll
        for (int r = 0; r < 4; ++r) dbias[i][r] = 0.f;
#pragma unroll
    for (int i = 0; i < TO1; ++i)
#pragma unroll
        for (int r = 0; r < 4; ++r) dbe0[i][r] = dga0[i][r] = 0.f;

    constexpr int CL = NL == 2 ? C2 : C1, TOL = CL / 16;
    SASTAMP(1);
    unsigned long long n_items_dbg = 0, n_steps_dbg = 0;
    const int nA = first.nA, nB = first.nB;
    const int G = a.group > 0 && a.group < a.B ? a.group : a.B;
    const int nitems = a.order ? (nA + nB) * G * ((a.B + G - 1) / G) : (ncent + 3) >> 2;
    for (int round = 0;; ++round) {
        const int qi = round * nwaves + ((round & 1) ? nwaves - 1 - wave : wave);
        if (round * nwaves >= nitems) break;
        if (qi >= nitems) continue;
        SaItem it;
        if (!sa_item(it, a.order, a.cnt, a.B, a.M, nA, nB, G, qi, c, round == 0 ? first.rec : nullptr)) continue;
        if (n_items_dbg == 0) { SASTAMP(2); }
        ++n_items_dbg;
        n_steps_dbg += (it.nmax + it.estep - 1) / it.estep;
        const int nmax = it.nmax, estep = it.estep;
        float cpq[4];
        float dov[4][TOL][4];
        int arv[4][TOL][4];
#pragma unroll
        for (int t = 0; t < 4; ++t) {
            cpq[t] = a.cpos[(size_t)it.lc[t] * 4 + (q < 3 ? q : 0)];
#pragma unroll
            for (int io = 0; io < TOL; ++io) {
                const size_t o = (size_t)it.lc[t] * CL + 16 * io + 4 * q;
                const float4 dv = *reinterpret_cast<const float4*>(a.dout + o);
                const int4 av = *reinterpret_cast<const int4*>(a.arg + o);
                dov[t][io][0] = dv.x; dov[t][io][1] = dv.y; dov[t][io][2] = dv.z; dov[t][io][3] = dv.w;
                arv[t][io][0] = av.x; arv[t][io][1] = av.y; arv[t][io][2] = av.z; arv[t][io][3] = av.w;
            }
        }
        int jn[4];
#pragma unroll
        for (int t = 0; t < 4; ++t) {
            const int e = it.le0 + it.eoff * t;
            jn[t] = a.nbr[(size_t)it.lc[t] * a.cap + (e < a.cap ? e : 0)];
        }
#pragma unroll
        for (int t = 0; t < 4; ++t) jn[t] = it.le0 + it.eoff * t < it.ln[t] ? jn[t] : 0;
        for (int e0 = 0; e0 < nmax; e0 += estep) {
            f32x4 D1[TO1][4];
            float bks[4][KB1];
            bool val[4];
            size_t rows[4];
            int jc[4];
#pragma unroll
            for (int t = 0; t < 4; ++t) {
                jc[t] = jn[t];
                const int en = e0 + estep + it.le0 + it.eoff * t;
                const bool more = en < it.ln[t];
                const int jr = a.nbr[(size_t)it.lc[t] * a.cap + (more ? en : 0)];
                jn[t] = more ? jr : 0;
                rows[t] = (size_t)it.bt[t] * a.Nsrc + jc[t];
#pragma unroll
                for (int kb = 0; kb < KB1 - 1; ++kb) bks[t][kb] = a.feat[rows[t] * a.feat_stride + 4 * kb + q];
                bks[t][KB1 - 1] = a.spos[rows[t] * a.spos_stride + (q < 3 ? q : 0)];
            }
#pragma unroll
            for (int t = 0; t < 4; ++t) {
                const int e = e0 + it.le0 + it.eoff * t;
                val[t] = e < it.ln[t];
                bks[t][KB1 - 1] = q < 3 ? bks[t][KB1 - 1] - cpq[t] : 1.0f;
#pragma unroll
                for (int io = 0; io < TO1; ++io) {
                    f32x4 v = {bias1[io][0], bias1[io][1], bias1[io][2], bias1[io][3]};
                    v = contract<BF16, KB1>(v, [&](int kb) { return A1[io][kb]; }, [&](int kb) { return bks[t][kb]; });
#pragma unroll
                    for (int r = 0; r < 4; ++r) v[r] = fmaxf(v[r], 0.f);
                    D1[io][t] = v;
                }
            }
            f32x4 dy1[TO1][4];
            if constexpr (NL == 2) {
                f32x4 Y1[TO1][4], dp2[TO2][4];
#pragma unroll
                for (int is = 0; is < TO1; ++is)
#pragma unroll
                    for (int t = 0; t < 4; ++t)
#pragma unroll
                        for (int r = 0; r < 4; ++r) Y1[is][t][r] = fmaf(a1v[is][r], D1[is][t][r], c1v[is][r]);
#pragma unroll
                for (int io = 0; io < TO2; ++io)
#pragma unroll
                    for (int t = 0; t < 4; ++t) {
                        f32x4 v = {bias2[io][0], bias2[io][1], bias2[io][2], bias2[io][3]};
                        v = contract<BF16, 4 * TO1>(v, [&](int kk) { return A2[io][kk >> 2][kk & 3]; },
                                                    [&](int kk) { return Y1[kk >> 2][t][kk & 3]; });
                        const int e = e0 + it.le0 + it.eoff * t;
#pragma unroll
                        for (int r = 0; r < 4; ++r) {
                            const float h = fmaxf(v[r], 0.f);
                            const float dy = (val[t] && arv[t][io][r] == e) ? dov[t][io][r] : 0.f;
                            dp2[io][t][r] = (val[t] && h > 0.f) ? fmaf(cA1[io][r], dy, fmaf(-cC1[io][r], h, cD1[io][r])) : 0.f;
                        }
                    }
#pragma unroll
                for (int is = 0; is < TO1; ++is)
#pragma unroll
                    for (int t = 0; t < 4; ++t) {
                        f32x4 v = {0.f, 0.f, 0.f, 0.f};
                        v = contract<BF16, 4 * TO2>(v, [&](int kk) { return A2T[is][kk >> 2][kk & 3]; },
                                                    [&](int kk) { return dp2[kk >> 2][t][kk & 3]; });
                        dy1[is][t] = v;
                    }
                if constexpr (PASS == 2) {
#pragma unroll
                    for (int t = 0; t < 4; ++t) {
#pragma unroll
                        for (int io = 0; io < TO2; ++io)
                            *reinterpret_cast<float4*>(lds_p + (16 * t + c) * PS + 16 * io + 4 * q) =
                                make_float4(dp2[io][t][0], dp2[io][t][1], dp2[io][t][2], dp2[io][t][3]);
#pragma unroll
                        for (int is = 0; is < TO1; ++is)
                            *reinterpret_cast<float4*>(lds_q + (16 * t + c) * QS + 16 * is + 4 * q) =
                                make_float4(Y1[is][t][0], Y1[is][t][1], Y1[is][t][2], Y1[is][t][3]);
                    }
#pragma unroll
                    for (int io = 0; io < TO2; ++io)
#pragma unroll
                        for (int t = 0; t < 4; ++t)
#pragma unroll
                            for (int r = 0; r < 4; ++r) dbias[io][r] += dp2[io][t][r];
#pragma unroll
                    for (int is = 0; is < TO1; ++is)
#pragma unroll
                        for (int t = 0; t < 4; ++t)
#pragma unroll
                            for (int r = 0; r < 4; ++r) {
                                dbe0[is][r] += dy1[is][t][r];
                                dga0[is][r] = fmaf(dy1[is][t][r], (D1[is][t][r] - mu0[is][r]) * is0[is][r], dga0[is][r]);
                            }
                }
            } else {
#pragma unroll
                for (int is = 0; is < TO1; ++is)
#pragma unroll
                    for (int t = 0; t < 4; ++t) {
                        const int e = e0 + it.le0 + it.eoff * t;
#pragma unroll
                        for (int r = 0; r < 4; ++r) dy1[is][t][r] = (val[t] && arv[t][is][r] == e) ? dov[t][is][r] : 0.f;
                    }
            }
            if constexpr (PASS == 3) {
                f32x4 dp1[TO1][4];
#pragma unroll
                for (int is = 0; is < TO1; ++is)
#pragma unroll
                    for (int t = 0; t < 4; ++t)
#pragma unroll
                        for (int r = 0; r < 4; ++r) {
                            const float h = D1[is][t][r];
                            dp1[is][t][r] = (val[t] && h > 0.f)
                                                ? fmaf(cA0[is][r], dy1[is][t][r], fmaf(-cC0[is][r], h, cD0[is][r])) : 0.f;
                        }
#pragma unroll
                for (int t = 0; t < 4; ++t) {
#pragma unroll
                    for (int is = 0; is < TO1; ++is)
                        *reinterpret_cast<float4*>(lds_p + (16 * t + c) * PS + 16 * is + 4 * q) =
                            make_float4(dp1[is][t][0], dp1[is][t][1], dp1[is][t][2], dp1[is][t][3]);
#pragma unroll
                    for (int kb = 0; kb < KB1; ++kb) lds_q[(16 * t + c) * QS + 4 * kb + q] = bks[t][kb];
                }
                if (a.dfeat) {
#pragma unroll
                    for (int kt = 0; kt < TF; ++kt)
#pragma unroll
                        for (int t = 0; t < 4; ++t) {
                            f32x4 v = {0.f, 0.f, 0.f, 0.f};
                            v = contract<BF16, 4 * TO1>(v, [&](int kk) { return A0T[kt][kk >> 2][kk & 3]; },
                                                        [&](int kk) { return dp1[kk >> 2][t][kk & 3]; });
                            if (val[t]) {
#pragma unroll
                                for (int r = 0; r < 4; ++r) {
                                    const int k = 16 * kt + 4 * q + r;
                                    if (k < CF) atomicAdd(&a.dfeat[rows[t] * CF + k], v[r]);
                                }
                            }
                        }
                }
            }
            __builtin_amdgcn_fence(__ATOMIC_RELEASE, "wavefront");
            __builtin_amdgcn_wave_barrier();
            {
                const float* rp = lds_p + q * PS + c;
                const float* rq = lds_q + q * QS + c;
                if constexpr (!BF16) {
#pragma unroll 4
                    for (int st = 0; st < 16; ++st) {
                        float av[TP], bv[TQ];
#pragma unroll
                        for (int i = 0; i < TP; ++i) av[i] = rp[st * 4 * PS + 16 * i];
#pragma unroll
                        for (int j = 0; j < TQ; ++j) bv[j] = rq[st * 4 * QS + 16 * j];
#pragma unroll
                        for (int i = 0; i < TP; ++i)
#pragma unroll
                            for (int j = 0; j < TQ; ++j)
                                acc[i][j] = __builtin_amdgcn_mfma_f32_16x16x4f32(av[i], bv[j], acc[i][j], 0, 0, 0);
                    }
                } else {
#pragma unroll
                    for (int s8 = 0; s8 < 2; ++s8) {
                        float av[TP][8], bv[TQ][8];
#pragma unroll
                        for (int u = 0; u < 8; ++u) {
#pragma unroll
                            for (int i = 0; i < TP; ++i) av[i][u] = rp[(8 * s8 + u) * 4 * PS + 16 * i];
#pragma unroll
                            for (int j = 0; j < TQ; ++j) bv[j][u] = rq[(8 * s8 + u) * 4 * QS + 16 * j];
                        }
#pragma unroll
                        for (int i = 0; i < TP; ++i)
#pragma unroll
                            for (int j = 0; j < TQ; ++j)
                                acc[i][j] = contract<true, 8>(acc[i][j], [&](int u) { return av[i][u]; }, [&](int u) { return bv[j][u]; });
                    }
                }
            }
            __builtin_amdgcn_fence(__ATOMIC_ACQUIRE, "wavefront");
            __builtin_amdgcn_wave_barrier();
        }
        if (n_items_dbg == 1) { SASTAMP(3); }
    }
    SASTAMP(4);
    SACOUNT(8, n_items_dbg);
    SACOUNT(9, n_steps_dbg);

    constexpr int NW = PO * QK, NB = LAST2 ? C2 : 0, NG = LAST2 ? 2 * C1 : 0;
    static_assert(NW + NB + NG <= Acc::LDS_FLOATS, "a wave's image fits its staging region");
    float* slab = lds_p;
#pragma unroll
    for (int i = 0; i < TP; ++i)
#pragma unroll
        for (int j = 0; j < TQ; ++j)
#pragma unroll
            for (int r = 0; r < 4; ++r) {
                const int o = 16 * i + 4 * q + r, k = 16 * j + c;
                if (o < PO && k < QK) slab[o * QK + k] = acc[i][j][r];
            }
    if constexpr (LAST2) {
#pragma unroll
        for (int io = 0; io < TO2; ++io)
#pragma unroll
            for (int r = 0; r < 4; ++r) {
                const float v = row_sum(dbias[io][r]);
                if (c == 0) slab[NW + 16 * io + 4 * q + r] = v;
            }
#pragma unroll
        for (int is = 0; is < TO1; ++is)
#pragma unroll
            for (int r = 0; r < 4; ++r) {
                const float v1 = row_sum(dbe0[is][r]), v2 = row_sum(dga0[is][r]);
                if (c == 0) {
                    slab[NW + NB + 16 * is + 4 * q + r] = v1;
                    slab[NW + NB + C1 + 16 * is + 4 * q + r] = v2;
                }
            }
    }
    SASTAMP(5);
    __syncthreads();
    SASTAMP(6);
    const int img = sn2_grad_image(a.rep_k, a.rep_stride);
    for (int i = threadIdx.x; i < NW + NB + NG; i += 256) {
        const float v = (smem[i] + smem[Acc::LDS_FLOATS + i]) + (smem[2 * Acc::LDS_FLOATS + i] + smem[3 * Acc::LDS_FLOATS + i]);
        if (v == 0.f) continue;
        if (i < NW) {
            if constexpr (LAST2) {
                SN2_FLUSH_ADD(&a.dW1[img + i], v);
            } else {
                const int o = i / QK, k = i - o * QK;
                if (k < CIN) SN2_FLUSH_ADD(&a.dW0[img + o * CIN + k], v);
                else SN2_FLUSH_ADD(&a.db0[img + o], v);
            }
        } else if (i < NW + NB) {
            SN2_FLUSH_ADD(&a.db1[img + i - NW], v);
        } else if (i < NW + NB + C1) {
            SN2_FLUSH_ADD(&a.dbeta0_out[i - NW - NB], v);
        } else {
            SN2_FLUSH_ADD(&a.dgamma0_out[i - NW - NB - C1], v);
        }
    }
    SASTAMP(7);
}

}

static int sa_plot_group(int B) {
    static const int g_env = getenv("SN2_SA_GROUP") ? atoi(getenv("SN2_SA_GROUP")) : 0;
    if (g_env > 0) return g_env;
    return B <= 32 ? B : 8;
}

template <int CF, int NL, int C1, int C2, int PASS>
int sa_mfma_launch_fwd(const sn2_sa* p, int training, hipStream_t st, int* nblocks_out) {
    const bool bf16 = p->blk[0].mma_bf16 != 0;
    SaFwdArgs a;
    a.B = p->B; a.Nsrc = p->Nsrc; a.M = p->M; a.cap = p->cap; a.feat_stride = p->feat_stride; a.spos_stride = p->spos_stride;
    a.feat = p->feat; a.spos = p->spos; a.cpos = p->cpos; a.nbr = p->nbr; a.cnt = p->cnt; a.order = p->order;
    a.group = sa_plot_group(p->B);
    const sn2_block& k0 = p->blk[0];
    const sn2_block& k1 = p->blk[NL == 2 ? 1 : 0];
    a.W0 = k0.W; a.b0 = k0.b; a.a0 = k0.a; a.c0 = k0.c; a.gamma0 = k0.gamma;
    a.W1 = k1.W; a.b1 = k1.b; a.gamma1 = k1.gamma;
    a.slots = training == 1 ? (PASS == 0 ? k0.stat_slots : k1.stat_slots) : nullptr;
    a.ext = p->ext; a.arg = p->arg;
    a.al = k1.a; a.cl = k1.c; a.out = p->out;
    int blocks = sn2_cdiv((long)p->B * p->M, 16);
    if (blocks > SN2_STAT_SLOTS) blocks = SN2_STAT_SLOTS;
    static const int occ_env = getenv("SN2_SA_FWD_OCC") ? atoi(getenv("SN2_SA_FWD_OCC")) : 0;
    const int occ = occ_env > 0 ? occ_env : (CF == 8 ? (PASS == 0 ? 4 : 3) : (CF == 16 ? 2 : 1));
    if (blocks > sn2_cu_count() * occ) blocks = sn2_cu_count() * occ;
    if (nblocks_out) *nblocks_out = blocks;
    if constexpr (PASS == 1) {
        if (!training) {
            if (bf16) hipLaunchKernelGGL((sa_mfma_fwd_kernel<CF, NL, C1, C2, PASS, true, false>), dim3(blocks), dim3(256), 0, st, a);
            else hipLaunchKernelGGL((sa_mfma_fwd_kernel<CF, NL, C1, C2, PASS, false, false>), dim3(blocks), dim3(256), 0, st, a);
            SN2_RETURN_LAUNCH();
        }
    }
    if (bf16) hipLaunchKernelGGL((sa_mfma_fwd_kernel<CF, NL, C1, C2, PASS, true>), dim3(blocks), dim3(256), 0, st, a);
    else hipLaunchKernelGGL((sa_mfma_fwd_kernel<CF, NL, C1, C2, PASS, false>), dim3(blocks), dim3(256), 0, st, a);
    SN2_RETURN_LAUNCH();
}

template int sa_mfma_launch_fwd<8, 2, 16, 16, 0>(const sn2_sa*, int, hipStream_t, int*);
template int sa_mfma_launch_fwd<8, 2, 16, 16, 1>(const sn2_sa*, int, hipStream_t, int*);
template int sa_mfma_launch_fwd<16, 1, 32, 32, 1>(const sn2_sa*, int, hipStream_t, int*);
template int sa_mfma_launch_fwd<32, 1, 64, 64, 1>(const sn2_sa*, int, hipStream_t, int*);

template <int CF, int NL, int C1, int C2, int PASS>
int sa_mfma_launch_bwd(const sn2_sa* p, hipStream_t st) {
    constexpr int CIN = CF + 3;
    constexpr bool LAST2 = NL == 2 && PASS == 2;
    using Acc = OuterAcc<(LAST2 ? C2 : C1), (LAST2 ? C1 : CIN + 1)>;
    SaBwdArgs a;
    a.B = p->B; a.Nsrc = p->Nsrc; a.M = p->M; a.cap = p->cap; a.feat_stride = p->feat_stride; a.spos_stride = p->spos_stride;
    a.feat = p->feat; a.spos = p->spos; a.cpos = p->cpos; a.nbr = p->nbr; a.cnt = p->cnt; a.order = p->order; a.total = p->total;
    a.group = sa_plot_group(p->B);
    const sn2_block& k0 = p->blk[0];
    const sn2_block& k1 = p->blk[NL == 2 ? 1 : 0];
    a.frozen = (k0.frozen_stats || k1.frozen_stats) ? 1 : 0;
    a.W0 = k0.W; a.b0 = k0.b; a.a0 = k0.a; a.c0 = k0.c; a.gamma0 = k0.gamma; a.mean0 = k0.mean; a.invstd0 = k0.invstd;
    a.dgamma0 = k0.dgamma; a.dbeta0 = k0.dbeta;
    a.W1 = k1.W; a.b1 = k1.b; a.gamma1 = k1.gamma; a.mean1 = k1.mean; a.invstd1 = k1.invstd; a.dgamma1 = k1.dgamma;
    a.dbeta1 = k1.dbeta;
    a.dout = p->dout; a.arg = p->arg;
    a.dW0 = k0.dW; a.db0 = k0.db; a.dW1 = k1.dW; a.db1 = k1.db; a.dgamma0_out = k0.dgamma; a.dbeta0_out = k0.dbeta;
    a.rep_k = k0.grad_replicas; a.rep_stride = k0.grad_replica_stride;
    a.dfeat = p->dfeat;
    int blocks = sn2_cdiv((long)p->B * p->M, 16);
    static const int occ_env = getenv("SN2_SA_BWD_OCC") ? atoi(getenv("SN2_SA_BWD_OCC")) : 0;
    const int occ = occ_env > 0 ? occ_env : (CF == 8 ? 2 : 1);
    if (blocks > sn2_cu_count() * occ) blocks = sn2_cu_count() * occ;
    const size_t lds = (size_t)Acc::LDS_FLOATS * 4 * sizeof(float);
    auto kern = p->blk[0].mma_bf16 ? &sa_mfma_bwd_kernel<CF, NL, C1, C2, PASS, true> : &sa_mfma_bwd_kernel<CF, NL, C1, C2, PASS, false>;
    if (lds > 48 * 1024)
        (void)hipFuncSetAttribute(reinterpret_cast<const void*>(kern), hipFuncAttributeMaxDynamicSharedMemorySize, (int)lds);
    hipLaunchKernelGGL(kern, dim3(blocks), dim3(256), lds, st, a);
    SN2_RETURN_LAUNCH();
}

template int sa_mfma_launch_bwd<8, 2, 16, 16, 2>(const sn2_sa*, hipStream_t);
template int sa_mfma_launch_bwd<8, 2, 16, 16, 3>(const sn2_sa*, hipStream_t);
template int sa_mfma_launch_bwd<16, 1, 32, 32, 3>(const sn2_sa*, hipStream_t);
template int sa_mfma_launch_bwd<32, 1, 64, 64, 3>(const sn2_sa*, hipStream_t);
```

stratanet2_vegetation_coverage_maps_amd/hip_ops.py:

```python
import math
from typing import Optional

import numpy as np
import torch

from . import _lib
from ._lib import FP, SA, Block, Head, StrataHipError, check

I32, F32, F64, I64, BF16 = torch.int32, torch.float32, torch.float64, torch.int64, torch.bfloat16


_timing = None


class timing:

    def __init__(self, names=None):
        self.names = None if names is None else set(names)
        self.events = []

    def __enter__(self):
        global _timing
        self._prev, _timing = _timing, self
        return self
# ... 451 lines not shown
          _ptr(rot), _ptr(flips), _ptr(noise), _ptr(noise_offsets), Tn, float(z_max), _ptr(cloud), _ptr(xyz), _stream())
    return cloud, xyz


SUBSAMPLE_LDS, SUBSAMPLE_GLOBAL, SUBSAMPLE_COARSE = 1, 2, 4
SUBSAMPLE_LDS_MAX = 16384


def subsample_form(n_max: int, N: int) -> int:
    return int(_lib.load().sn2_subsample_form(int(n_max), int(N)))


def subsample_ws_words(B: int, n_max: int, N: int, form: int = 0) -> int:
    return int(_lib.load().sn2_subsample_ws_words(int(B), int(n_max), int(N), int(form)))


def subsample(offsets, extra: int, N: int, seed: int, plot_keys, n_max: Optional[int] = None, form: int = 0):
    _chk(offsets, I32, None, "offsets")
    if offsets.dim() != 1 or offsets.numel() < 2:
        raise ValueError("offsets: expected (B+1,) with B >= 1")
    B = offsets.numel() - 1
    _chk(plot_keys, I64, (B,), "plot_keys")
    extra, N, seed, form = int(extra), int(N), int(seed), int(form)
    if N <= 0 or extra < 0:
        raise ValueError("subsample: N must be positive and extra non-negative")
    if not 0 <= seed < 2 ** 64:
        raise ValueError("subsample: seed must fit 64 unsigned bits")
    if n_max is None:
        n_max = int((offsets[1:] - offsets[:-1]).max()) + extra
    n_max = int(n_max)
    if n_max <= 0 or n_max >= 2 ** 31:
        raise ValueError("subsample: n_max must be in 1 .. 2^31 - 1 (a plot needs at least one candidate)")
    if form not in (0, 1, 2, 5, 6):
        raise ValueError("subsample: form must be 0, SUBSAMPLE_LDS or SUBSAMPLE_GLOBAL (| SUBSAMPLE_COARSE)")
    if form & 3 == SUBSAMPLE_LDS and n_max > SUBSAMPLE_LDS_MAX:
        raise ValueError(f"subsample: the LDS form takes at most {SUBSAMPLE_LDS_MAX} candidates per plot")
    dev = offsets.device
    nw = subsample_ws_words(B, n_max, N, form)
    ws = torch.empty(nw + 4, dtype=I32, device=dev) if nw else None
    idx = torch.empty(B, N, dtype=I32, device=dev)
    _call("sn2_subsample", _ptr(offsets), extra, n_max, B, N, seed, _ptr(plot_keys), form, _ptr(ws), nw, _ptr(idx), _stream())
    return idx


def znorm(xyz: torch.Tensor, radius: float):
    _, n = xyz.shape
    _chk(xyz, F32, (3, n), "xyz")
    if not radius > 0:
        raise ValueError("znorm: radius must be positive")
    lo = xyz[:2].min(1).values.tolist()
    hi = xyz[:2].max(1).values.tolist()
    cells = (int((hi[0] - lo[0]) / radius) + 2) * (int((hi[1] - lo[1]) / radius) + 2)
    ws = torch.empty(5 * n + 3 * cells + 8, dtype=I32, device=xyz.device)
    zmin = torch.empty(n, dtype=F32, device=xyz.device)
    zout = torch.empty(n, dtype=F32, device=xyz.device)
    _call("sn2_znorm", _ptr(xyz[0]), _ptr(xyz[1]), _ptr(xyz[2]), n, float(radius), lo[0], lo[1], hi[0], hi[1], _ptr(ws),
          _ptr(zmin), _ptr(zout), _stream())
    return zmin, zout


def parcel_count_ws_words(P: int, rows: int) -> int:
    return int(_lib.load().sn2_parcel_count_ws_words(int(P), int(rows)))


def parcel_znorm_ws_words(T: int, radius: float, x_min: float, y_min: float, x_max: float, y_max: float) -> int:
    return int(_lib.load().sn2_parcel_znorm_ws_words(int(T), float(radius), float(x_min), float(y_min), float(x_max),
                                                     float(y_max)))


def _chk_center_grid(grid, P: int):
    start, items, GX, GY, gx0, gy0, inv = grid
    _chk(start, I32, (GX * GY + 1,), "cell_start")
    _chk(items, I32, None, "cell_items")
    if items.dim() != 1 or items.numel() < 1 or items.numel() > P:
        raise ValueError("cell_items: expected 1..P centre ids")
    return start, items, int(GX), int(GY), float(gx0), float(gy0), float(inv)


def parcel_count(cloud: torch.Tensor, centers: torch.Tensor, grid, radius: float, L: int, rows: int):
    _, T = cloud.shape
    _chk(cloud, F32, (10, T), "cloud")
    P = centers.shape[0]
    _chk(centers, F32, (P, 2), "centers")
    start, items, GX, GY, gx0, gy0, inv = _chk_center_grid(grid, P)
    dev = cloud.device
    nw = parcel_count_ws_words(P, rows)
    ws = torch.empty(nw + 4, dtype=I32, device=dev)
    prefix = torch.empty(P * rows + 1, dtype=I32, device=dev)
    total = torch.empty(1, dtype=I64, device=dev)
    _call("sn2_parcel_count", _ptr(cloud), T, int(L), int(rows), _ptr(centers), P, _ptr(start), _ptr(items), GX, GY, gx0, gy0,
          inv, float(radius), _ptr(ws), nw, _ptr(prefix), _ptr(total), _stream())
    return prefix, total


def parcel_fill(cloud: torch.Tensor, centers: torch.Tensor, grid, radius: float, L: int, rows: int, prefix: torch.Tensor,
                plot_base: torch.Tensor, sum_n: int):
    _, T = cloud.shape
    _chk(cloud, F32, (10, T), "cloud")
    P = centers.shape[0]
    _chk(centers, F32, (P, 2), "centers")
    start, items, GX, GY, gx0, gy0, inv = _chk_center_grid(grid, P)
    _chk(prefix, I32, (P * rows + 1,), "prefix")
    _chk(plot_base, I32, (P,), "plot_base")
    dev = cloud.device
    raw = torch.empty(10, sum_n, dtype=F32, device=dev)
    pidx = torch.empty(sum_n, dtype=I32, device=dev)
    _call("sn2_parcel_fill", _ptr(cloud), T, int(L), int(rows), _ptr(centers), P, _ptr(start), _ptr(items), GX, GY, gx0, gy0,
          inv, float(radius), _ptr(prefix), _ptr(plot_base), int(sum_n), _ptr(raw), _ptr(pidx), _stream())
    return raw, pidx


def parcel_znorm(cloud: torch.Tensor, bbox, radius: float, disc_radius: float, offsets: torch.Tensor, centers: torch.Tensor,
                 point_index: torch.Tensor, raw: torch.Tensor):
    _, T = cloud.shape
    _chk(cloud, F32, (10, T), "cloud")
    P = centers.shape[0]
    _chk(centers, F32, (P, 2), "centers")
    _chk(offsets, I32, (P + 1,), "offsets")
    sum_n = point_index.shape[0]
    _chk(point_index, I32, (sum_n,), "point_index")
    _chk(raw, F32, (10, sum_n), "raw")
    nw = parcel_znorm_ws_words(T, radius, *bbox)
    if nw == 0:
        raise ValueError("parcel_znorm: the parcel's extent needs more than 2^26 cells of the z-norm radius")
    ws = torch.empty(nw + 4, dtype=I32, device=cloud.device)
    _call("sn2_parcel_znorm", _ptr(cloud), T, *[float(v) for v in bbox], float(radius), float(disc_radius), _ptr(offsets),
          _ptr(centers), P, _ptr(point_index), sum_n, _ptr(ws), nw, _ptr(raw), _stream())
    return raw


def sa_order_len(B: int, M: int) -> int:
    return 4 * B * M + 16 * B * (M // 8 + 2) + 8


def sa_order(cnt: torch.Tensor, B: int, M: int, out: Optional[torch.Tensor] = None) -> torch.Tensor:
    _chk(cnt, I32, (B * M,), "cnt")
    n = sa_order_len(B, M)
    if out is None:
        out = torch.empty(n, dtype=I32, device=cnt.device)
    else:
        _chk(out, I32, (n,), "out order")
    _call("sn2_sa_order", _ptr(cnt), B, M, _ptr(out), _stream())
    return out


def sa_order_group(cnt: torch.Tensor, G: int, B: int, M: int, out_all: torch.Tensor, stride: int):
    _chk(cnt, I32, (G * B * M,), "cnt")
    if stride < sa_order_len(B, M):
        raise ValueError("sa_order_group: stride smaller than a table")
    _chk(out_all, I32, (G * stride,), "out order tables")
    _call("sn2_sa_order_group", _ptr(cnt), G, B, M, _ptr(out_all), stride, _stream(), key="sn2_sa_order")


def sa_desc(blocks, feat, cf, spos, cpos_aos, nbr, cnt, total, B, Nsrc, M, ext, arg, out, dout=None, dfeat=None,
            with_grads=False, order=None) -> SA:
    cap = nbr.shape[1]
    cl = blocks[-1].cout
    feat_stride = _chk_rows(feat, F32, B * Nsrc, cf, "feat")
    spos_stride = _chk_rows(spos, F32, B * Nsrc, 4, "spos")
    _chk(cpos_aos, F32, (B * M, 4), "cpos_aos")
    _chk(nbr, I32, (B * M, cap), "nbr")
    _chk(cnt, I32, (B * M,), "cnt")
    _chk(total, I64, (1,), "total")
    _chk(ext, F32, (B * M, cl), "ext")
    _chk(arg, I32, (B * M, cl), "arg")
    _chk(out, F32, (B * M, cl), "out")
    d = SA()
    d.B, d.Nsrc, d.M, d.cap, d.cf, d.nl = B, Nsrc, M, cap, cf, len(blocks)
    d.feat, d.feat_stride, d.spos, d.spos_stride = _ptr(feat), feat_stride, _ptr(spos), spos_stride
    d.cpos, d.nbr, d.cnt, d.total = _ptr(cpos_aos), _ptr(nbr), _ptr(cnt), _ptr(total)
    if order is not None:
        _chk(order, I32, (sa_order_len(B, M),), "order")
    d.order = _ptr(order)
    for i, bb in enumerate(blocks):
        bb.fill(d.blk[i], with_grads)
    d.ext, d.arg, d.out = _ptr(ext), _ptr(arg), _ptr(out)
    if dout is not None:
        _chk(dout, F32, (B * M, cl), "dout")
    if dfeat is not None:
        _chk(dfeat, F32, (B * Nsrc, cf), "dfeat")
    d.dout, d.dfeat = _ptr(dout), _ptr(dfeat)
    return d


def sa_forward(d: SA, training: bool):
    _call("sn2_sa_forward", d, int(training), _stream(), tag=f"cf={d.cf}")


def sa_backward(d: SA):
    _call("sn2_sa_backward", d, _stream(), tag=f"cf={d.cf}")


def interp_ws_words(B: int, R_per_plot: int, S_per_plot: int) -> int:
    return (B * S_per_plot * ((R_per_plot + 2047) // 2048 + 6) + 6 * B * R_per_plot + 64
            + 4 * B * interp_chunks(R_per_plot, S_per_plot))


def interp_chunks(R_per_plot: int, S_per_plot: int) -> int:
    return (3 * R_per_plot + 62) // 63 + S_per_plot


def interp_index(knn, B: int, R_per_plot: int, S_per_plot: int, out: Optional[torch.Tensor] = None,
                 src_pos: Optional[torch.Tensor] = None, row_perm: Optional[torch.Tensor] = None) -> torch.Tensor:
    if src_pos is not None:
        _chk(src_pos, F32, (B * S_per_plot, 4), "src_pos")
    if row_perm is not None:
        _chk(row_perm, I32, (B * R_per_plot,), "row_perm")
    R = B * R_per_plot
    _chk(knn[0], I32, (R, 3), "knn_idx")
    _chk(knn[1], F32, (R, 3), "knn_w")
    n = interp_ws_words(B, R_per_plot, S_per_plot)
    if out is None:
        out = torch.empty(n, dtype=F32, device=knn[0].device)
    else:
        _chk(out, F32, (n,), "out index")
    _call("sn2_interp_index_perm", _ptr(knn[0]), _ptr(knn[1]), _ptr(src_pos), _ptr(row_perm), B, R_per_plot, S_per_plot, _ptr(out),
          _stream(), key="sn2_interp_index")
    return out


def interp_index_group(knn, G: int, B: int, R_per_plot: int, S_per_plot: int, out_all: torch.Tensor, stride: int,
                       src_pos: Optional[torch.Tensor] = None, row_perm: Optional[torch.Tensor] = None):
    R = G * B * R_per_plot
    _chk(knn[0], I32, (R, 3), "knn_idx")
    _chk(knn[1], F32, (R, 3), "knn_w")
    if src_pos is not None:
        _chk(src_pos, F32, (G * B * S_per_plot, 4), "src_pos")
    if row_perm is not None:
        _chk(row_perm, I32, (R,), "row_perm")
    if stride % 4 or stride < interp_ws_words(B, R_per_plot, S_per_plot):
        raise ValueError("interp_index_group: stride must be a multiple of 4 words and hold one index")
    _chk(out_all, F32, (G * stride,), "out indices")
    _call("sn2_interp_index_group", _ptr(knn[0]), _ptr(knn[1]), _ptr(src_pos), _ptr(row_perm), G, B, R_per_plot, S_per_plot, _ptr(out_all),
          stride, _stream(), key="sn2_interp_index")


SOURCE_SIDE = True


def fp_desc(block: BlockBuffers, B, R_per_plot, S_per_plot, ca, cb, src, h, src_affine=None, knn=None, skip=None,
            dy=None, dsrc=None, dskip=None, du_scratch=None, with_grads=False, interp_index=None,
            bn_sums_done=None, row_perm=None, force_src_ws=False, gather=True) -> FP:
    R = B * R_per_plot
    hs = (block.cout + 3) // 4 * 4
    AT = BF16 if (h is not None and h.dtype == BF16) else F32
    n_src_rows = R if knn is None else B * S_per_plot
    src_stride = _chk_rows(src, F32, n_src_rows, ca, "src")
    if src.shape[1] < (ca + 3) // 4 * 4 and src_stride < (ca + 3) // 4 * 4:
        raise ValueError("fp: src rows must be padded to a multiple of 4 floats")
    if h is not None or not force_src_ws:
        _chk(h, AT, (R, hs), "h")
    d = FP()
    d.B, d.R_per_plot, d.S_per_plot, d.ca, d.cb = B, R_per_plot, S_per_plot, ca, cb
    d.src, d.src_stride = _ptr(src), src_stride
    if src_affine is not None:
        _chk(src_affine[0], F32, (ca,), "src_a")
        _chk(src_affine[1], F32, (ca,), "src_c")
        d.src_a, d.src_c = _ptr(src_affine[0]), _ptr(src_affine[1])
    else:
        d.src_a = d.src_c = None
    if knn is not None:
        _chk(knn[0], I32, (R, 3), "knn_idx")
        _chk(knn[1], F32, (R, 3), "knn_w")
        d.knn_idx, d.knn_w = _ptr(knn[0]), _ptr(knn[1])
    else:
        d.knn_idx = d.knn_w = None
    if cb > 0:
        d.skip_stride = _chk_rows(skip, F32, R, cb, "skip", align=4 if cb % 4 == 0 else 1)
        d.skip = _ptr(skip)
    else:
        d.skip, d.skip_stride = None, 0
    block.fill(d.blk, with_grads)
    if R > 64 * _lib.STAT_SLOTS:
        d.blk.mma_bf16 = 0
    d.h, d.h_stride = _ptr(h), hs
    if dy is not None:
        _chk(dy, AT, (R, hs), "dy")
    d.dsrc_stride = d.dskip_stride = 0
    if dsrc is not None:
        d.dsrc_stride = _chk_rows(dsrc, F32, n_src_rows, ca, "dsrc", align=1)
    if dskip is not None:
        d.dskip_stride = _chk_rows(dskip, F32, R, cb, "dskip", align=1)
    d.scatter_ws, d.scatter_ready = None, 0
    if bn_sums_done is not None:
        _chk(bn_sums_done, I32, (1,), "bn_sums_done")
    d.bn_sums_done = _ptr(bn_sums_done)
    d._src_ws = None
    if SOURCE_SIDE and knn is not None and 0 < cb <= 16 and cb % 4 == 0 and (R > 64 * _lib.STAT_SLOTS or force_src_ws):
        d._src_ws = torch.empty(B * interp_chunks(R_per_plot, S_per_plot) * hs, dtype=F32, device=src.device)
    d.src_ws = _ptr(d._src_ws)
    d.row_perm = None
    if row_perm is not None and d._src_ws is not None and du_scratch is not None:
        _chk(row_perm, I32, (R,), "row_perm")
        d.row_perm = _ptr(row_perm)
    d.act_bf16 = int(AT == BF16)
    if d.act_bf16 and d._src_ws is None:
        raise ValueError("fp: bfloat16 activation rows need the source-side form (a k-NN layer of more than 65 536 rows)")
    if du_scratch is not None:
        _chk(du_scratch, AT, (R, max(ca, hs)), "du_scratch")
        if knn is not None and dsrc is not None:
            words = interp_ws_words(B, R_per_plot, S_per_plot)
            if interp_index is not None:
                _chk(interp_index, F32, (words,), "interp_index")
                d._scatter_ws, d.scatter_ready = interp_index, 1
            else:
                d._scatter_ws = torch.empty(words, dtype=F32, device=src.device)
            d.scatter_ws = _ptr(d._scatter_ws)
            if not gather:
                d.scatter_ready = -1
    d.dy, d.dsrc, d.dskip, d.du_scratch = _ptr(dy), _ptr(dsrc), _ptr(dskip), _ptr(du_scratch)
    return d


def fp_bn_sums(d: FP, gamma, beta, mean, invstd, dgamma, dbeta, ok):
    for t, n in ((gamma, "gamma"), (beta, "beta"), (mean, "mean"), (invstd, "invstd"), (dgamma, "dgamma"), (dbeta, "dbeta")):
        _chk(t, F32, (d.ca,), n)
    _chk(ok, I32, (1,), "ok")
    _call("sn2_fp_bn_sums", d, _ptr(gamma), _ptr(beta), _ptr(mean), _ptr(invstd), _ptr(dgamma), _ptr(dbeta), _ptr(ok), _stream())


def fp_forward(d: FP, training: bool):
    _call("sn2_fp_forward", d, int(training), _stream(), tag=f"{d.ca}+{d.cb}->{d.blk.cout}")


def fp_backward(d: FP):
    _call("sn2_fp_backward", d, _stream(), tag=f"{d.ca}+{d.cb}->{d.blk.cout}")


def plot_max_forward(h, a, c, B, R_per_plot, C):
    hs = (C + 3) // 4 * 4
    _chk(h, F32, (B * R_per_plot, hs), "h")
    _chk(a, F32, (C,), "a")
    _chk(c, F32, (C,), "c")
    out = torch.empty(B, C, dtype=F32, device=h.device)
# ... 463 lines not shown
```

stratanet2_vegetation_coverage_maps_amd/point_net2.py:

```python
import os
from collections import OrderedDict

import torch
import torch.nn as nn
from torch.nn import BatchNorm1d as BN
from torch.nn import Linear as Lin
from torch.nn import ReLU
from torch.nn import Sequential as Seq

from . import executor as X
from . import hip_ops as ops
from ._lib import BN_FROZEN_KEEP, MAX_NEIGHBORS as _MAXN, STAT_SLOTS, StrataHipError

MAX_NEIGHBORS = _MAXN

F32, I32, I64, F64 = torch.float32, torch.int32, torch.int64, torch.float64


def MLP(channels):
    return Seq(*[Seq(Lin(channels[i - 1], channels[i]), ReLU(), BN(channels[i])) for i in range(1, len(channels))])


class PointConv(nn.Module):

# ... 409 lines not shown
            g.has_rows0 = cloud2 is not None
            g.p2_diam_pix = gp.p2_diam_pix if cloud2 is not None else None
            g.has_inverted = True
            if clouds is not None and cloud2 is None:
                self._input_only(g, clouds[h], g.xyz)
        return halves

    def prefetch_geometry(self, cloud_data, lane: int = 0):
        dev = self.lin1.weight.device
        if dev.type != "cuda":
            raise StrataHipError("prefetch_geometry needs a HIP device")
        with torch.cuda.device(dev):
            xyz_d, fs = self._stage_positions(cloud_data, dev)
            side = ops.shared_stream(dev, f"side{lane}")
            side.wait_stream(torch.cuda.current_stream())
            xyz_d.record_stream(side)
            fs.record_stream(side)
            with torch.cuda.stream(side):
                cl = cloud_data.get("cloud", None) if isinstance(cloud_data, dict) else None
                cl = cl if (isinstance(cl, torch.Tensor) and cl.is_cuda and cl.dtype == F32 and cl.is_contiguous()) else None
                g = self._geometry(xyz_d, fs, shared=True, fork=False, inverted=self.training, cloud=cl)
                g.fps_start = fs
                g.ready = torch.cuda.Event()
                g.ready.record(side)
            g.stream = side
        return g

    def _stage_positions(self, cloud_data, dev, ring=None):
        xyz = cloud_data["xyz"]
        if ring is not None and not xyz.is_cuda:
            xyz_d = ring.upload(xyz, dtype=F32)
        else:
            xyz_d = xyz.to(device=dev, dtype=F32, non_blocking=True).contiguous()
        B, _, N = xyz_d.shape
        fs = cloud_data.get("fps_start", None) if isinstance(cloud_data, dict) else None
        if fs is None:
            m1 = ops.fps_num_samples(N, self.sa1_module.ratio)
            fs = torch.stack([torch.randint(0, N, (B,)), torch.randint(0, m1, (B,))])
        fs = torch.as_tensor(fs).to(device=dev, dtype=I32, non_blocking=True).contiguous()
        if fs.shape != (2, B):
            raise ValueError(f"fps_start must have shape (2,{B})")
        return xyz_d, fs

    def _forward_impl(self, xyz, cloud, fps_start, training, geo=None, drop_keep=None, need_grad=True):
        if self._use_executor():
            cov, proba, s = X.forward(self, self._net_model(), xyz, cloud, fps_start, training, geo, drop_keep, need_grad=need_grad)
            if self.log_embeddings:
                self.last_G_tensor = s.x3
            return cov, proba, s
        dev = xyz.device
        B, _, N = xyz.shape
        M1, M2 = self._sizes(N)
        cur_stream = torch.cuda.current_stream(dev)
        frozen = (not training) and bool(need_grad)
        keep = bool(training) or frozen
        mode = 1 if training else (BN_FROZEN_KEEP if frozen else 0)
        rows0, packed = None, None
        if geo is not None and getattr(geo, "has_rows0", False) and geo.rows0.shape[0] == B * N:
            rows0 = geo.rows0
        if geo is None:
            if self.geometry_fork:
                rows0 = torch.empty(B * N, 12, dtype=F32, device=dev)
                pack_stream = ops.shared_stream(dev, "pack")
                pack_stream.wait_stream(cur_stream)
                with torch.cuda.stream(pack_stream):
                    ops.pack_rows(cloud, xyz, out=rows0)
                    packed = torch.cuda.Event()
                    packed.record(pack_stream)
            geo = self._geometry(xyz, fps_start, defer_join=True, inverted=keep)
        elif (geo.B, geo.N, geo.M1, geo.M2) != (B, N, M1, M2):
            raise ValueError("prefetched geometry does not match this batch")
        join = getattr(geo, "_join", None)
        geo._join = None
        if join == "ctx":
            raise StrataHipError("a geometry pass launched by the executor with a deferred join must be consumed by the executor")
        if keep and not getattr(geo, "has_inverted", True):
            if join is not None:
                cur_stream.wait_stream(join[0])
                cur_stream.wait_stream(join[1])
                join = None
            ops.count_sum(geo.cnt1, geo.tot1)
            ops.count_sum(geo.cnt2, geo.tot2)
            ops.interp_index(geo.knn3, B, M2, 1, out=geo.inv3)
            ops.interp_index(geo.knn2, B, M1, M2, out=geo.inv2)
            ops.interp_index(geo.knn1, B, N, M1, out=geo.inv1, src_pos=geo.pos1_aos, row_perm=getattr(geo, "rank1", None))
            geo.has_inverted = True
        s = _Saved()
        s.__dict__.update({k: v for k, v in geo.__dict__.items()
                           if k not in ("ready", "stream", "ws1", "ws2", "totals", "nn_ws", "fps_start", "_join", "has_rows0")})
        s.xyz = xyz
        widths = [16, 16, 32, 64, 64, 34, 34]
        aux = torch.empty(4 * sum(widths), dtype=F32, device=dev)
        stats = torch.empty(STAT_SLOTS * 2 * sum(widths), dtype=F32, device=dev)
        cur = [0, 0]
        bf = lambda prefix: self.mma_dtype == "bf16" and prefix in self.BF16_BLOCKS
        s.b_sa1 = _blocks_of(self.sa1_module.conv.local_nn, aux, stats, cur, bf("sa1_module.conv.local_nn"))
        s.b_sa2 = _blocks_of(self.sa2_module.conv.local_nn, aux, stats, cur, bf("sa2_module.conv.local_nn"))
        s.b_sa3 = _blocks_of(self.sa3_module.nn, aux, stats, cur, bf("sa3_module.nn"))[0]
        s.b_fp3 = _blocks_of(self.fp3_module.nn, aux, stats, cur, bf("fp3_module.nn"))[0]
        s.b_fp2 = _blocks_of(self.fp2_module.nn, aux, stats, cur, bf("fp2_module.nn"))[0]
        s.b_fp1 = _blocks_of(self.fp1_module.nn, aux, stats, cur)[0]
        s.aux, s.stats = aux, stats
        for bb in s.b_sa1 + s.b_sa2 + [s.b_sa3, s.b_fp3, s.b_fp2, s.b_fp1]:
            bb.frozen = frozen

        if packed is not None:
            cur_stream.wait_event(packed)
            s.rows0 = rows0
        elif rows0 is not None:
            s.rows0 = rows0
        else:
            s.rows0 = ops.pack_rows(cloud, xyz)
        s.ext1 = torch.empty(B * M1, 16, dtype=F32, device=dev)
        s.arg1 = torch.empty(B * M1, 16, dtype=I32, device=dev)
        s.x1 = torch.empty(B * M1, 16, dtype=F32, device=dev)
        ops.sa_forward(self._sa1_desc(s), mode)
        if join is not None:
            cur_stream.wait_stream(join[0])
        s.ext2 = torch.empty(B * M2, 32, dtype=F32, device=dev)
        s.arg2 = torch.empty(B * M2, 32, dtype=I32, device=dev)
        s.x2 = torch.empty(B * M2, 32, dtype=F32, device=dev)
        ops.sa_forward(self._sa2_desc(s), mode)
        s.h_sa3 = torch.empty(B * M2, 64, dtype=F32, device=dev)
        s.h3 = torch.empty(B * M2, 64, dtype=F32, device=dev)
        if training and self.fuse_global_level and B <= 28 and not (s.b_sa3.mma_bf16 or s.b_fp3.mma_bf16):
            s.x3 = torch.empty(B, 64, dtype=F32, device=dev)
            s.arg3 = torch.empty(B, 64, dtype=I32, device=dev)
            ops.global_level_forward(self._sa3_desc(s), self._fp3_desc(s), s.x3, s.arg3, owner=self)
        else:
            ops.fp_forward(self._sa3_desc(s), mode)
            s.x3, s.arg3 = ops.plot_max_forward(s.h_sa3, s.b_sa3.a, s.b_sa3.c, B, M2, 64)
            ops.fp_forward(self._fp3_desc(s), mode)
        if self.log_embeddings:
            self.last_G_tensor = s.x3
        s.h2 = torch.empty(B * M1, 36, dtype=F32, device=dev)
        ops.fp_forward(self._fp2_desc(s), mode)
        if join is not None:
            cur_stream.wait_stream(join[1])
        cov = torch.empty(B * N, 4, dtype=F32, device=dev)
        proba = torch.empty(B * N, 4, dtype=F32, device=dev)
        s.drop_keep = drop_keep
        if not keep and self.fuse_eval_head and self._act_dtype(B * N) == F32 and ops.SOURCE_SIDE:
            s.h1 = None
            d1 = ops.fp_desc(s.b_fp1, B, N, M1, 34, 8, s.h2, None, src_affine=(s.b_fp2.a, s.b_fp2.c), knn=s.knn1,
                             skip=s.rows0[:, 0:8], force_src_ws=True)
            ops.fp_head_eval(d1, ops.head_desc(None, s.b_fp1.a, s.b_fp1.c, self.lin1, self.lin2, cov, proba, rows=B * N))
            return cov, proba, s
        s.h1 = torch.empty(B * N, 36, dtype=self._act_dtype(B * N), device=dev)
        ops.fp_forward(self._fp1_desc(s), mode)
        ops.head_forward(ops.head_desc(s.h1, s.b_fp1.a, s.b_fp1.c, self.lin1, self.lin2, cov, proba, drop_mask=drop_keep,
                                       drop_p=self.drop))
        return cov, proba, s

    def _sa1_desc(self, s, dout=None, g=False):
        return ops.sa_desc(s.b_sa1, s.rows0[:, 0:8], 8, s.rows0[:, 8:12], s.pos1_aos, s.nbr1, s.cnt1, s.tot1, s.B, s.N,
                           s.M1, s.ext1, s.arg1, s.x1, dout=dout, dfeat=None, with_grads=g, order=getattr(s, "ord1", None))

    def _sa2_desc(self, s, dout=None, dfeat=None, g=False):
        return ops.sa_desc(s.b_sa2, s.x1, 16, s.pos1_aos, s.pos2_aos, s.nbr2, s.cnt2, s.tot2, s.B, s.M1, s.M2, s.ext2,
                           s.arg2, s.x2, dout=dout, dfeat=dfeat, with_grads=g, order=getattr(s, "ord2", None))

    def _sa3_desc(self, s, **kw):
        return ops.fp_desc(s.b_sa3, s.B, s.M2, s.M2, 32, 3, s.x2, s.h_sa3, skip=s.pos2_aos, **kw)

    def _fp3_desc(self, s, **kw):
        return ops.fp_desc(s.b_fp3, s.B, s.M2, 1, 64, 32, s.x3, s.h3, knn=s.knn3, skip=s.x2, **kw)

    def _fp2_desc(self, s, **kw):
        return ops.fp_desc(s.b_fp2, s.B, s.M1, s.M2, 64, 16, s.h3, s.h2, src_affine=(s.b_fp3.a, s.b_fp3.c), knn=s.knn2,
                           skip=s.x1, **kw)

    def _fp1_desc(self, s, **kw):
        return ops.fp_desc(s.b_fp1, s.B, s.N, s.M1, 34, 8, s.h2, s.h1, src_affine=(s.b_fp2.a, s.b_fp2.c), knn=s.knn1,
                           skip=s.rows0[:, 0:8], row_perm=getattr(s, "rank1", None), **kw)

    def _backward_impl(self, s, dcov, dproba):
        if isinstance(s, X.NetSaved):
            return X.backward(self, s, dcov, dproba)
        dev = s.xyz.device
        B, N, M1, M2 = s.B, s.N, s.M1, s.M2
        params = self._params()
        sizes = OrderedDict(dy2=B * M1 * 36, dy3=B * M2 * 64, dx1=B * M1 * 16, dx2=B * M2 * 32, dx3=B * 64,
                            dy_sa3=B * M2 * 64)
        flat, buf, views, images, arena = self._grad_arena(params, sizes, dev)

        def attach(bb):
            bb.grads = (views[id(bb.lin.weight)], views[id(bb.lin.bias)], views[id(bb.bn.weight)], views[id(bb.bn.bias)])
            bb.grad_images = images

        for bb in s.b_sa1 + s.b_sa2 + [s.b_sa3, s.b_fp3, s.b_fp2, s.b_fp1]:
            attach(bb)
        dcov = None if dcov is None else dcov.contiguous()
        dproba = None if dproba is None else dproba.contiguous()
        dy1 = torch.empty(B * N, 36, dtype=s.h1.dtype, device=dev)
        hg = (views[id(self.lin1.weight)], views[id(self.lin1.bias)], views[id(self.lin2.weight)], views[id(self.lin2.bias)])
        hd = ops.head_desc(s.h1, s.b_fp1.a, s.b_fp1.c, self.lin1, self.lin2, dcov=dcov, dproba=dproba, dy=dy1, grads=hg,
                           grad_images=images, drop_mask=getattr(s, "drop_keep", None), drop_p=self.drop)
        ops.head_backward(hd)
        bn1 = self.fp1_module.nn[0][2]
        bn_ok = torch.empty(4, dtype=I32, device=dev)
        ops.head_bn_sums(hd, bn1.weight.detach(), bn1.bias.detach(), s.b_fp1.aux[2], s.b_fp1.aux[3], views[id(bn1.weight)],
                         views[id(bn1.bias)], bn_ok[0:1])
        dy2 = buf["dy2"].view(B * M1, 36)
        d1 = self._fp1_desc(s, dy=dy1, dsrc=dy2, du_scratch=torch.empty(B * N, 36, dtype=s.h1.dtype, device=dev), with_grads=True,
                            interp_index=s.inv1, bn_sums_done=bn_ok[0:1])
        ops.fp_backward(d1)
        bn2 = self.fp2_module.nn[0][2]
        ops.fp_bn_sums(d1, bn2.weight.detach(), bn2.bias.detach(), s.b_fp2.aux[2], s.b_fp2.aux[3], views[id(bn2.weight)],
                       views[id(bn2.bias)], bn_ok[1:2])
        dy3, dx1 = buf["dy3"].view(B * M2, 64), buf["dx1"].view(B * M1, 16)
        d2 = self._fp2_desc(s, dy=dy2, dsrc=dy3, dskip=dx1, du_scratch=torch.empty(B * M1, 64, dtype=F32, device=dev),
                            with_grads=True, interp_index=s.inv2, bn_sums_done=bn_ok[1:2])
        ops.fp_backward(d2)
        bn3 = self.fp3_module.nn[0][2]
        ops.fp_bn_sums(d2, bn3.weight.detach(), bn3.bias.detach(), s.b_fp3.aux[2], s.b_fp3.aux[3], views[id(bn3.weight)],
                       views[id(bn3.bias)], bn_ok[2:3])
        dx3, dx2 = buf["dx3"].view(B, 64), buf["dx2"].view(B * M2, 32)
        du3 = torch.empty(B * M2, 64, dtype=F32, device=dev)
        ops.fp_backward(self._fp3_desc(s, dy=dy3, dsrc=dx3, dskip=dx2, du_scratch=du3, with_grads=True,
                                       interp_index=s.inv3, bn_sums_done=bn_ok[2:3], gather=False))
        dy_sa3 = buf["dy_sa3"].view(B * M2, 64)
        bn_sa3 = self.sa3_module.nn[0][2]
        ops.global_pool_backward(du3, s.arg3, s.h_sa3, s.b_sa3.aux[2], s.b_sa3.aux[3], B, M2, dx3, dy_sa3,
                                 views[id(bn_sa3.weight)], views[id(bn_sa3.bias)])
        ops.fp_backward(self._sa3_desc(s, dy=dy_sa3, dsrc=dx2, with_grads=True, bn_sums_done=bn_ok[3:4]))
        ops.sa_backward(self._sa2_desc(s, dout=dx2, dfeat=dx1, g=True))
        ops.sa_backward(self._sa1_desc(s, dout=dx1, g=True))
        if getattr(self, "defer_grad_reduce", False):
            self._grad_images_pending = (arena,) + tuple(images)
        else:
            ops.grad_reduce(arena, flat.numel(), images)
            self._grad_images_pending = None
        s.flat_grad = flat
        self._last_flat_grad = flat
        return [views[id(p)] for p in params]

    @staticmethod
    def _grad_arena(params, sizes, dev):
        poffs, n_flat = ops.flat_layout(params)
        offs, tot = {}, 0
        for k, n in sizes.items():
            offs[k] = tot
            tot += (n + 3) // 4 * 4
        arena, flat, images, extra = ops.grad_images_alloc(n_flat, dev, tot)
        buf = {k: extra[offs[k]:offs[k] + n] for k, n in sizes.items()}
        views = {id(p): flat[o:o + p.numel()].view(p.shape) for p, o in zip(params, poffs)}
        return flat, buf, views, images, arena

    @staticmethod
    def get_long_form(data):
        B, f, N = data.shape
        return data.permute(1, 0, 2).reshape(f, B * N).transpose(1, 0)

    def get_batch_format(self, data):
        n = self.subsample_size
        return data.view(-1, n, data.shape[1]).transpose(1, 2)

    def set_patience_attributes(self, args):
        self.stopped_early = False
        self.best_metric_value = 10 ** 6
        self.best_metric_epoch = 1
        self.patience_in_epochs = args.patience_in_epochs

    def stop_early(self, val_metric, epoch, args):
        if val_metric < self.best_metric_value:
            self.best_metric_value, self.best_metric_epoch = val_metric, epoch
            self.save_state(args)
            return False
        if epoch < args.epoch_to_start_early_stop:
            return False
        if epoch >= self.best_metric_epoch + self.patience_in_epochs:
            self.stopped_early = True
            return True
        return False

    @staticmethod
    def _checkpoint_path(args):
        tag = f"fold_n={args.current_fold_id}" if args.current_fold_id > 0 else "full"
        return os.path.join(args.stats_path, f"PCC_model_{tag}.pt")

    def save_state(self, args):
        torch.save({"best_metric_epoch": self.best_metric_epoch, "state_dict": self.state_dict(),
                    "best_metric_value": self.best_metric_value}, self._checkpoint_path(args))

    def load_state(self, save_path):
        checkpoint = torch.load(save_path, map_location=None if self.cuda_device is not None else torch.device("cpu"))
        self.load_state_dict(checkpoint["state_dict"])
        self.best_metric_epoch = checkpoint["best_metric_epoch"]
        self.best_metric_value = checkpoint["best_metric_value"]
        return self

    def load_best_state(self, args):
        return self.load_state(self._checkpoint_path(args))
```

stratanet2_vegetation_coverage_maps_amd/point_net2_3sa.py:

```python
from collections import OrderedDict

import torch
from torch import nn

from . import hip_ops as ops
from ._lib import BN_FROZEN_KEEP, STAT_SLOTS
from . import point_net2 as _p2
from .point_net2 import (F32, I32, I64, MLP, FPModule, GlobalSAModule, PointNet2, SAModule, _blocks_of, _Saved)


class PointNet2ThreeSA(PointNet2):
    def __init__(self, args):
        nn.Module.__init__(self)
        self.cuda_device = args.cuda
        self.subsample_size = args.subsample_size
        self.n_class = args.n_class
        self.drop = args.drop
        self.n_input_feats = args.n_input_feats - 2
        self.set_patience_attributes(args)
        self.log_embeddings = args.log_embeddings
        self.last_G_tensor = None
        self._last_flat_grad = None
        self._last_cloud_dev = None
        if self.n_class != 4 or self.n_input_feats != 8:
# ... 112 lines not shown
            setattr(g, f"ord{lvl}", e(ops.sa_order_len(B, M), dt=I32))
        g.totals = torch.zeros(3, dtype=I64, device=dev)
        g.tot1, g.tot2, g.tot3 = g.totals[0:1], g.totals[1:2], g.totals[2:3]
        g.posg = torch.zeros(B, 3, 1, dtype=F32, device=dev)
        g.knn4, g.knn3 = (e(B * M3, 3, dt=I32), e(B * M3, 3)), (e(B * M2, 3, dt=I32), e(B * M2, 3))
        g.knn2, g.knn1 = (e(B * M1, 3, dt=I32), e(B * M1, 3)), (e(B * N, 3, dt=I32), e(B * N, 3))
        g.inv4, g.inv3, g.inv2, g.inv1 = (e(ops.interp_ws_words(B, R, S)) for R, S in ((M3, 1), (M2, M3), (M1, M2), (N, M1)))
        g.nn_ws = tuple(e(ops.three_nn_ws_words(B, S, T), dt=I32) if ops.three_nn_uses_grid(S, T) else None
                        for S, T in ((M3, M2), (M2, M1), (M1, N)))
        g.rank1 = ops.fps_ws_rank(g.ws1, B, N) if (self.fp1_morton_rows and g.ws1 is not None and self._fp1_source_side(B * N)) else None
        self._alloc_input_only(g, B, N, dev)
        g.ready = None
        return g

    def _geometry(self, xyz, fps_start, out=None, fork=None, shared=False, defer_join=False, inverted=True, cloud=None):
        dev = xyz.device
        B, _, N = xyz.shape
        M1, M2, M3 = self._sizes3(N)
        g = out if out is not None else self.alloc_geometry(B, N, dev)
        if (g.B, g.N, g.M1, g.M2, g.M3) != (B, N, M1, M2, M3):
            raise ValueError("geometry buffers do not match this batch")
        g.xyz = xyz
        g.has_rows0 = False
        if cloud is not None:
            self._input_only(g, cloud, xyz)
        cap = _p2.MAX_NEIGHBORS
        src = xyz
        for lvl, (M, mod) in enumerate(((M1, self.sa1_module), (M2, self.sa2_module), (M3, self.sa3_module)), 1):
            ws = getattr(g, f"ws{lvl}")
            cs = getattr(g, f"pos{lvl}_soa")
            ops.fps(src, M, fps_start[lvl - 1], out=(getattr(g, f"idx{lvl}"), cs, getattr(g, f"pos{lvl}_aos"), ws),
                    waves=(self.fps_waves_many if B > 32 else self.fps_waves_shared) if (shared and lvl == 1) else 0)
            ops.ball_query(src, cs, mod.r, cap, getattr(g, f"tot{lvl}"), fps_ws=ws,
                           out=(getattr(g, f"nbr{lvl}"), getattr(g, f"cnt{lvl}")))
            ops.sa_order(getattr(g, f"cnt{lvl}"), B, M, out=getattr(g, f"ord{lvl}"))
            src = cs
        ops.three_nn(g.posg, g.pos3_soa, 1, out=g.knn4)
        ops.three_nn(g.pos3_soa, g.pos2_soa, 3, out=g.knn3, ws=g.nn_ws[0])
        ops.three_nn(g.pos2_soa, g.pos1_soa, 3, out=g.knn2, ws=g.nn_ws[1])
        ops.three_nn(g.pos1_soa, xyz, 3, out=g.knn1, ws=g.nn_ws[2])
        if inverted:
            self._inverted_tables(g)
        g.has_inverted = bool(inverted)
        g._join = None
        return g

    @staticmethod
    def _inverted_tables(g):
        B, N, M1, M2, M3 = g.B, g.N, g.M1, g.M2, g.M3
        ops.interp_index(g.knn4, B, M3, 1, out=g.inv4)
        ops.interp_index(g.knn3, B, M2, M3, out=g.inv3)
        ops.interp_index(g.knn2, B, M1, M2, out=g.inv2)
        ops.interp_index(g.knn1, B, N, M1, out=g.inv1, src_pos=g.pos1_aos, row_perm=getattr(g, "rank1", None))

    def _stage_positions(self, cloud_data, dev, ring=None):
        xyz = cloud_data["xyz"]
        if ring is not None and not xyz.is_cuda:
            xyz_d = ring.upload(xyz, dtype=F32)
        else:
            xyz_d = xyz.to(device=dev, dtype=F32, non_blocking=True).contiguous()
        B, _, N = xyz_d.shape
        fs = cloud_data.get("fps_start", None) if isinstance(cloud_data, dict) else None
        if fs is None:
            M1, M2, _ = self._sizes3(N)
            fs = torch.stack([torch.randint(0, N, (B,)), torch.randint(0, M1, (B,)), torch.randint(0, M2, (B,))])
        fs = torch.as_tensor(fs).to(device=dev, dtype=I32, non_blocking=True).contiguous()
        if fs.shape != (3, B):
            raise ValueError(f"fps_start must have shape (3,{B})")
        return xyz_d, fs

    def _forward_impl(self, xyz, cloud, fps_start, training, geo=None, drop_keep=None, need_grad=True):
        dev = xyz.device
        B, _, N = xyz.shape
        M1, M2, M3 = self._sizes3(N)
        frozen = (not training) and bool(need_grad)
        keep = bool(training) or frozen
        mode = 1 if training else (BN_FROZEN_KEEP if frozen else 0)
        if geo is None:
            geo = self._geometry(xyz, fps_start, inverted=keep)
        elif (geo.B, geo.N, geo.M1, geo.M2, geo.M3) != (B, N, M1, M2, M3):
            raise ValueError("prefetched geometry does not match this batch")
        if keep and not getattr(geo, "has_inverted", True):
            self._inverted_tables(geo)
            geo.has_inverted = True
        s = _Saved()
        s.__dict__.update({k: v for k, v in geo.__dict__.items()
                           if k not in ("ready", "stream", "totals", "nn_ws", "fps_start", "_join", "has_inverted", "has_rows0")})
        s.xyz = xyz
        widths = [16, 16, 32, 64, 64, 64, 64, 34, 34]
        aux = torch.empty(4 * sum(widths), dtype=F32, device=dev)
        stats = torch.empty(STAT_SLOTS * 2 * sum(widths), dtype=F32, device=dev)
        cur = [0, 0]
        bf = lambda prefix: self.mma_dtype == "bf16" and prefix in self.BF16_BLOCKS
        s.b_sa1 = _blocks_of(self.sa1_module.conv.local_nn, aux, stats, cur, bf("sa1_module.conv.local_nn"))
        s.b_sa2 = _blocks_of(self.sa2_module.conv.local_nn, aux, stats, cur, bf("sa2_module.conv.local_nn"))
        s.b_sa3 = _blocks_of(self.sa3_module.conv.local_nn, aux, stats, cur, bf("sa3_module.conv.local_nn"))
        s.b_sa4 = _blocks_of(self.sa4_module.nn, aux, stats, cur, bf("sa4_module.nn"))[0]
        s.b_fp4 = _blocks_of(self.fp4_module.nn, aux, stats, cur, bf("fp4_module.nn"))[0]
        s.b_fp3 = _blocks_of(self.fp3_module.nn, aux, stats, cur, bf("fp3_module.nn"))[0]
        s.b_fp2 = _blocks_of(self.fp2_module.nn, aux, stats, cur, bf("fp2_module.nn"))[0]
        s.b_fp1 = _blocks_of(self.fp1_module.nn, aux, stats, cur)[0]
        s.aux, s.stats = aux, stats
        for bb in s.b_sa1 + s.b_sa2 + s.b_sa3 + [s.b_sa4, s.b_fp4, s.b_fp3, s.b_fp2, s.b_fp1]:
            bb.frozen = frozen
        e = lambda *shape, dt=F32: torch.empty(*shape, dtype=dt, device=dev)
        if getattr(geo, "has_rows0", False) and geo.rows0.shape[0] == B * N:
            s.rows0 = geo.rows0
        else:
            s.rows0 = ops.pack_rows(cloud, xyz)
        s.ext1, s.arg1, s.x1 = e(B * M1, 16), e(B * M1, 16, dt=I32), e(B * M1, 16)
        ops.sa_forward(self._sa1_desc(s), mode)
        s.ext2, s.arg2, s.x2 = e(B * M2, 32), e(B * M2, 32, dt=I32), e(B * M2, 32)
        ops.sa_forward(self._sa2_desc(s), mode)
        s.ext3, s.arg3l, s.x3 = e(B * M3, 64), e(B * M3, 64, dt=I32), e(B * M3, 64)
        ops.sa_forward(self._sa3l_desc(s), mode)
        s.h_sa4 = e(B * M3, 64)
        ops.fp_forward(self._sa4_desc(s), mode)
        s.xg, s.argg = ops.plot_max_forward(s.h_sa4, s.b_sa4.a, s.b_sa4.c, B, M3, 64)
        if self.log_embeddings:
            self.last_G_tensor = s.xg
        s.h4 = e(B * M3, 64)
        ops.fp_forward(self._fp4_desc(s), mode)
        s.h3 = e(B * M2, 64)
        ops.fp_forward(self._fp3_desc(s), mode)
        s.h2 = e(B * M1, 36)
        ops.fp_forward(self._fp2_desc(s), mode)
        s.h1 = torch.empty(B * N, 36, dtype=self._act_dtype(B * N), device=dev)
        ops.fp_forward(self._fp1_desc(s), mode)
        cov, proba = e(B * N, 4), e(B * N, 4)
        s.drop_keep = drop_keep
        ops.head_forward(ops.head_desc(s.h1, s.b_fp1.a, s.b_fp1.c, self.lin1, self.lin2, cov, proba, drop_mask=drop_keep,
                                       drop_p=self.drop))
        return cov, proba, s

    def _sa3l_desc(self, s, dout=None, dfeat=None, g=False):
        return ops.sa_desc(s.b_sa3, s.x2, 32, s.pos2_aos, s.pos3_aos, s.nbr3, s.cnt3, s.tot3, s.B, s.M2, s.M3, s.ext3,
                           s.arg3l, s.x3, dout=dout, dfeat=dfeat, with_grads=g, order=s.ord3)

    def _sa4_desc(self, s, **kw):
        return ops.fp_desc(s.b_sa4, s.B, s.M3, s.M3, 64, 3, s.x3, s.h_sa4, skip=s.pos3_aos, **kw)

    def _fp4_desc(self, s, **kw):
        return ops.fp_desc(s.b_fp4, s.B, s.M3, 1, 64, 64, s.xg, s.h4, knn=s.knn4, skip=s.x3, **kw)

    def _fp3_desc(self, s, **kw):
        return ops.fp_desc(s.b_fp3, s.B, s.M2, s.M3, 64, 32, s.h4, s.h3, src_affine=(s.b_fp4.a, s.b_fp4.c), knn=s.knn3,
                           skip=s.x2, **kw)

    def _backward_impl(self, s, dcov, dproba):
        dev = s.xyz.device
        B, N, M1, M2, M3 = s.B, s.N, s.M1, s.M2, s.M3
        params = list(self.parameters())
        sizes = OrderedDict(dy2=B * M1 * 36, dy3=B * M2 * 64, dy4=B * M3 * 64, dx1=B * M1 * 16, dx2=B * M2 * 32,
                            dx3=B * M3 * 64, dxg=B * 64, dy_sa4=B * M3 * 64)
        flat, buf, views, images, arena = self._grad_arena(params, sizes, dev)
        for bb in s.b_sa1 + s.b_sa2 + s.b_sa3 + [s.b_sa4, s.b_fp4, s.b_fp3, s.b_fp2, s.b_fp1]:
            bb.grads = (views[id(bb.lin.weight)], views[id(bb.lin.bias)], views[id(bb.bn.weight)], views[id(bb.bn.bias)])
            bb.grad_images = images
        dcov = None if dcov is None else dcov.contiguous()
        dproba = None if dproba is None else dproba.contiguous()
        e = lambda *shape: torch.empty(*shape, dtype=F32, device=dev)
        dy1 = torch.empty(B * N, 36, dtype=s.h1.dtype, device=dev)
        hg = (views[id(self.lin1.weight)], views[id(self.lin1.bias)], views[id(self.lin2.weight)], views[id(self.lin2.bias)])
        hd = ops.head_desc(s.h1, s.b_fp1.a, s.b_fp1.c, self.lin1, self.lin2, dcov=dcov, dproba=dproba, dy=dy1, grads=hg,
                           grad_images=images, drop_mask=getattr(s, "drop_keep", None), drop_p=self.drop)
        ops.head_backward(hd)
        bn_ok = torch.empty(4, dtype=I32, device=dev)

        def bn_of(mod):
            return mod.nn[0][2]

        def sums(fn, d, bn, blk, k):
            fn(d, bn.weight.detach(), bn.bias.detach(), blk.aux[2], blk.aux[3], views[id(bn.weight)], views[id(bn.bias)],
               bn_ok[k:k + 1])

        sums(ops.head_bn_sums, hd, bn_of(self.fp1_module), s.b_fp1, 0)
        dy2, dy3, dy4 = buf["dy2"].view(B * M1, 36), buf["dy3"].view(B * M2, 64), buf["dy4"].view(B * M3, 64)
        dx1, dx2, dx3 = buf["dx1"].view(B * M1, 16), buf["dx2"].view(B * M2, 32), buf["dx3"].view(B * M3, 64)
        dxg, dy_sa4 = buf["dxg"].view(B, 64), buf["dy_sa4"].view(B * M3, 64)
        d1 = self._fp1_desc(s, dy=dy1, dsrc=dy2, du_scratch=torch.empty(B * N, 36, dtype=s.h1.dtype, device=dev), with_grads=True, interp_index=s.inv1,
                            bn_sums_done=bn_ok[0:1])
        ops.fp_backward(d1)
        sums(ops.fp_bn_sums, d1, bn_of(self.fp2_module), s.b_fp2, 1)
        d2 = self._fp2_desc(s, dy=dy2, dsrc=dy3, dskip=dx1, du_scratch=e(B * M1, 64), with_grads=True, interp_index=s.inv2,
                            bn_sums_done=bn_ok[1:2])
        ops.fp_backward(d2)
        sums(ops.fp_bn_sums, d2, bn_of(self.fp3_module), s.b_fp3, 2)
        d3 = self._fp3_desc(s, dy=dy3, dsrc=dy4, dskip=dx2, du_scratch=e(B * M2, 64), with_grads=True, interp_index=s.inv3,
                            bn_sums_done=bn_ok[2:3])
        ops.fp_backward(d3)
        sums(ops.fp_bn_sums, d3, bn_of(self.fp4_module), s.b_fp4, 3)
        ops.fp_backward(self._fp4_desc(s, dy=dy4, dsrc=dxg, dskip=dx3, du_scratch=e(B * M3, 64), with_grads=True,
                                       interp_index=s.inv4, bn_sums_done=bn_ok[3:4]))
        ops.plot_max_backward(dxg, s.argg, B, M3, 64, dy_sa4)
        ops.fp_backward(self._sa4_desc(s, dy=dy_sa4, dsrc=dx3, with_grads=True))
        ops.sa_backward(self._sa3l_desc(s, dout=dx3, dfeat=dx2, g=True))
        ops.sa_backward(self._sa2_desc(s, dout=dx2, dfeat=dx1, g=True))
        ops.sa_backward(self._sa1_desc(s, dout=dx1, g=True))
        ops.grad_reduce(arena, flat.numel(), images)
        s.flat_grad = flat
        self._last_flat_grad = flat
        return [views[id(p)] for p in params]
```

Baseline: 23080 plots/s.

## Fuse SA1 backward passes into one kernel with replica workspace and combine

For the first two-layer set-abstraction backward (no dfeat, fp32 MMA), the pass-2 kernel now also accumulates the layer-0 weight gradient directly. It stages masked gradients, normalized activations and inputs in extra LDS and runs MFMA outer products. The BN-correction sums go into a small 32-replica workspace, and a tiny combine kernel folds them into dW0/db0. This removes the separate pass-3 re-traversal of all neighbourhoods. The cost is more LDS per wave, a tighter launch-bounds occupancy hint, extra atomics, and a new workspace carved from the grad arena.

```diff
diff --git a/include/strata_hip.h b/include/strata_hip.h
--- a/include/strata_hip.h
+++ b/include/strata_hip.h
@@ -111,7 +111,10 @@
     float *out;
     const float *dout;
     float *dfeat;
+    float *bwd_ws;
 } sn2_sa;
+#define SN2_SA_BWD_WS_REPLICAS 32
+#define SN2_SA_BWD_WS_WORDS (SN2_SA_BWD_WS_REPLICAS * 2 * 16 * 12)
 #define SN2_SA_SOLO_MIN 64
 #define SN2_SA_QUAD_MIN 8
 #define SN2_SA_OCT_MIN 4
@@ -315,6 +318,7 @@
     float *arena; long arena_words;
     int images, image_stride;
     float *dy2, *dy3, *dx1, *dx2, *dx3, *dy_sa3;
+    float *sa1_ws;
     void *dy1, *du1;
     float *du2, *du3;
     int *bn_ok;
diff --git a/stratanet2_vegetation_coverage_maps_amd/_lib.py b/stratanet2_vegetation_coverage_maps_amd/_lib.py
--- a/stratanet2_vegetation_coverage_maps_amd/_lib.py
+++ b/stratanet2_vegetation_coverage_maps_amd/_lib.py
@@ -27,7 +27,8 @@
                 ("feat", c_void_p), ("feat_stride", c_int), ("spos", c_void_p), ("spos_stride", c_int),
                 ("cpos", c_void_p), ("nbr", c_void_p), ("cnt", c_void_p), ("total", c_void_p), ("order", c_void_p),
                 ("blk", Block * 2),
-                ("ext", c_void_p), ("arg", c_void_p), ("out", c_void_p), ("dout", c_void_p), ("dfeat", c_void_p)]
+                ("ext", c_void_p), ("arg", c_void_p), ("out", c_void_p), ("dout", c_void_p), ("dfeat", c_void_p),
+                ("bwd_ws", c_void_p)]
 
 
 class FP(Structure):
@@ -86,7 +87,7 @@
 class NetBwd(Structure):
     _fields_ = [("dcov", c_void_p), ("dproba", c_void_p), ("arena", c_void_p), ("arena_words", c_long), ("images", c_int),
                 ("image_stride", c_int)] + [(n, c_void_p) for n in (
-                    "dy2", "dy3", "dx1", "dx2", "dx3", "dy_sa3", "dy1", "du1", "du2", "du3", "bn_ok", "src_ws1", "src_ws2")] + [
+                    "dy2", "dy3", "dx1", "dx2", "dx3", "dy_sa3", "sa1_ws", "dy1", "du1", "du2", "du3", "bn_ok", "src_ws1", "src_ws2")] + [
                         ("defer_grad_reduce", c_int), ("arena_is_zero", c_int), ("frozen_stats", c_int)]
 
 
diff --git a/stratanet2_vegetation_coverage_maps_amd/csrc/net.hip b/stratanet2_vegetation_coverage_maps_amd/csrc/net.hip
--- a/stratanet2_vegetation_coverage_maps_amd/csrc/net.hip
+++ b/stratanet2_vegetation_coverage_maps_amd/csrc/net.hip
@@ -95,7 +95,7 @@
 }
 
 void sa1_desc(sn2_sa* s, const sn2_net_model* m, const sn2_net_dims* d, const sn2_net_geo* g, const sn2_net_act* a,
-              GradDst gd, const float* dout) {
+              GradDst gd, const float* dout, float* bwd_ws = nullptr) {
     memset(s, 0, sizeof(*s));
     s->B = d->B, s->Nsrc = d->N, s->M = d->M1, s->cap = d->cap1, s->cf = 8, s->nl = 2;
     s->feat = g->rows0, s->feat_stride = 12, s->spos = g->rows0 + 8, s->spos_stride = 12;
@@ -103,7 +103,7 @@
     fill_block(&s->blk[0], &m->sa1[0], 0, a, gd);
     fill_block(&s->blk[1], &m->sa1[1], 1, a, gd);
     s->ext = a->ext1, s->arg = a->arg1, s->out = a->x1;
-    s->dout = dout, s->dfeat = nullptr;
+    s->dout = dout, s->dfeat = nullptr, s->bwd_ws = bwd_ws;
 }
 void sa2_desc(sn2_sa* s, const sn2_net_model* m, const sn2_net_dims* d, const sn2_net_geo* g, const sn2_net_act* a,
               GradDst gd, const float* dout, float* dfeat) {
@@ -386,6 +386,7 @@
     b->arena = ar, b->images = GRAD_IMAGES, b->image_stride = (int)stride;
     b->dy2 = take(B * M1 * 36), b->dy3 = take(B * M2 * 64), b->dx1 = take(B * M1 * 16), b->dx2 = take(B * M2 * 32);
     b->dx3 = take(B * 64), b->dy_sa3 = take(B * M2 * 64);
+    b->sa1_ws = take(SN2_SA_BWD_WS_WORDS);
     b->arena_words = (long)o;
     *arena_bytes = o * sizeof(float);
     Carver c(scratch_base);
@@ -568,7 +569,7 @@
     sn2_sa sa;
     sa2_desc(&sa, m, d, g, a, gd, b->dx2, b->dx1);
     SN2_TRY(sn2_sa_backward(&sa, cur));
-    sa1_desc(&sa, m, d, g, a, gd, b->dx1);
+    sa1_desc(&sa, m, d, g, a, gd, b->dx1, b->sa1_ws);
     SN2_TRY(sn2_sa_backward(&sa, cur));
     if (b->defer_grad_reduce) return 0;
     return sn2_grad_reduce(b->arena, m->n_flat, GRAD_IMAGES, b->image_stride, cur);
diff --git a/stratanet2_vegetation_coverage_maps_amd/csrc/sa.hip b/stratanet2_vegetation_coverage_maps_amd/csrc/sa.hip
--- a/stratanet2_vegetation_coverage_maps_amd/csrc/sa.hip
+++ b/stratanet2_vegetation_coverage_maps_amd/csrc/sa.hip
@@ -3,7 +3,7 @@
 template <int CF, int NL, int C1, int C2, int PASS>
 int sa_mfma_launch_fwd(const sn2_sa* p, int training, hipStream_t st, int* nblocks_out);
 template <int CF, int NL, int C1, int C2, int PASS>
-int sa_mfma_launch_bwd(const sn2_sa* p, hipStream_t st);
+int sa_mfma_launch_bwd(const sn2_sa* p, float* ws, hipStream_t st);
 
 namespace {
 
@@ -48,6 +48,30 @@
     }
 }
 
+__global__ __launch_bounds__(256) void sa_bwd_combine_kernel(const float* __restrict__ ws, const float* __restrict__ dgamma,
+                                                             const float* __restrict__ dbeta,
+                                                             const unsigned long long* __restrict__ total, int C, int CIN,
+                                                             float* __restrict__ dW, float* __restrict__ db) {
+    const int n = C * (CIN + 1), i = threadIdx.x;
+    if (i >= n) return;
+    float part[2][SN2_SA_BWD_WS_REPLICAS];
+#pragma unroll
+    for (int r = 0; r < SN2_SA_BWD_WS_REPLICAS; ++r) {
+        part[0][r] = ws[(size_t)r * 2 * n + i];
+        part[1][r] = ws[(size_t)r * 2 * n + n + i];
+    }
+    const unsigned long long etot = *total;
+    const float invE = etot > 0 ? (float)(1.0 / (double)etot) : 0.f;
+    const int o = i / (CIN + 1), k = i - o * (CIN + 1);
+    const float dg = dgamma[o] * invE, de = dbeta[o] * invE;
+    float sx = 0.f, sm = 0.f;
+#pragma unroll
+    for (int r = 0; r < SN2_SA_BWD_WS_REPLICAS; ++r) sx += part[0][r], sm += part[1][r];
+    const float v = -fmaf(dg, sx, de * sm);
+    float* dst = k < CIN ? &dW[o * CIN + k] : &db[o];
+    *dst += v;
+}
+
 int check(const sn2_sa* p) {
     if (!p || p->B <= 0 || p->Nsrc <= 0 || p->M <= 0 || p->cap <= 0) return SN2_EINVAL;
     if (!p->feat || !p->spos || !p->cpos || !p->nbr || !p->cnt || !p->total || !p->ext || !p->arg || !p->out)
@@ -85,8 +109,19 @@
     if (pb > 256) pb = 256;
     hipLaunchKernelGGL(sa_bwd_prep_kernel, dim3(pb), dim3(256), 0, st, p->dout, p->ext, p->arg, last->mean, last->invstd,
                        rows, C, last->dgamma, last->dbeta);
-    if constexpr (NL == 2) SN2_TRY((sa_mfma_launch_bwd<CF, NL, C1, C2, 2>(p, st)));
-    SN2_TRY((sa_mfma_launch_bwd<CF, NL, C1, C2, 3>(p, st)));
+    if constexpr (NL == 2) {
+        const sn2_block* k0 = &p->blk[0];
+        if (!p->dfeat && p->bwd_ws && !k0->mma_bf16) {
+            SN2_TRY((sa_mfma_launch_bwd<CF, NL, C1, C2, 2>(p, p->bwd_ws, st)));
+            if (k0->frozen_stats || last->frozen_stats) return 0;
+            static_assert(C1 * (CF + 4) <= 256, "one thread per element of [dW0 | db0]");
+            hipLaunchKernelGGL(sa_bwd_combine_kernel, dim3(1), dim3((C1 * (CF + 4) + 63) / 64 * 64), 0, st, p->bwd_ws, k0->dgamma,
+                               k0->dbeta, p->total, C1, CF + 3, k0->dW, k0->db);
+            SN2_RETURN_LAUNCH();
+        }
+        SN2_TRY((sa_mfma_launch_bwd<CF, NL, C1, C2, 2>(p, nullptr, st)));
+    }
+    SN2_TRY((sa_mfma_launch_bwd<CF, NL, C1, C2, 3>(p, nullptr, st)));
     return 0;
 }
 
diff --git a/stratanet2_vegetation_coverage_maps_amd/csrc/sa_mfma.hip b/stratanet2_vegetation_coverage_maps_amd/csrc/sa_mfma.hip
--- a/stratanet2_vegetation_coverage_maps_amd/csrc/sa_mfma.hip
+++ b/stratanet2_vegetation_coverage_maps_amd/csrc/sa_mfma.hip
@@ -415,6 +415,7 @@
     float *dW0, *db0, *dW1, *db1, *dgamma0_out, *dbeta0_out;
     int rep_k, rep_stride;
     float* dfeat;
+    float* ws;
 };
 
 #ifdef SN2_SA_STAMPS
@@ -435,13 +436,25 @@
 #endif
 
 template <int CF, int NL, int C1, int C2, int PASS, bool BF16>
-__global__ __launch_bounds__(256) void sa_mfma_bwd_kernel(const SaBwdArgs a) {
+struct SaBwdLds {
+    static constexpr bool LAST2 = NL == 2 && PASS == 2;
+    static constexpr int OWN = OuterAcc<(LAST2 ? C2 : C1), (LAST2 ? C1 : CF + 4)>::LDS_FLOATS;
+    static constexpr int FLOATS = OWN + ((LAST2 && !BF16) ? 2 * 64 * 16 : 0);
+};
+
+template <int CF, int NL, int C1, int C2, int PASS, bool BF16>
+__global__ __launch_bounds__(256, (NL == 2 && PASS == 2 && !BF16) ? 2 : 1) void sa_mfma_bwd_kernel(const SaBwdArgs a) {
     constexpr int CIN = CF + 3, KB1 = CF / 4 + 1, TO1 = C1 / 16, TO2 = C2 / 16;
     constexpr bool LAST2 = NL == 2 && PASS == 2;
     constexpr int PO = LAST2 ? C2 : C1;
     constexpr int QK = LAST2 ? C1 : CIN + 1;
     using Acc = OuterAcc<PO, QK>;
     constexpr int PS = Acc::PS, QS = Acc::QS, TP = Acc::TO, TQ = Acc::TK;
+    constexpr bool ONE = LAST2 && !BF16;
+    static_assert(!ONE || (C1 == 16 && C2 == 16 && CIN + 1 <= 16), "one-pass round: 16-column images");
+    constexpr int QK0 = CIN + 1;
+    constexpr int WAVE_LDS = SaBwdLds<CF, NL, C1, C2, PASS, BF16>::FLOATS;
+    const bool one = ONE && a.ws != nullptr;
     extern __shared__ __attribute__((aligned(16))) float smem[];
     const int lane = threadIdx.x & 63, q = lane >> 4, c = lane & 15;
     const int wib = threadIdx.x >> 6;
@@ -449,10 +462,12 @@
     const int nwaves = gridDim.x * 4;
     const int ncent = a.B * a.M;
     const SaFirst first = sa_first(a.order, a.cnt, a.B, a.M, wave);
-    float* lds_p = smem + wib * Acc::LDS_FLOATS;
+    float* lds_p = smem + wib * WAVE_LDS;
     float* lds_q = lds_p + 64 * PS;
+    float* lds_x0 = lds_p + Acc::LDS_FLOATS;
+    float* lds_q0 = lds_x0 + 64 * 16;
     SASTAMP(0);
-    for (int i = lane; i < Acc::LDS_FLOATS; i += 64) lds_p[i] = 0.f;
+    for (int i = lane; i < WAVE_LDS; i += 64) lds_p[i] = 0.f;
 
     const unsigned long long etot = *a.total;
     const float invE = (etot > 0 && !a.frozen) ? (float)(1.0 / (double)etot) : 0.f;
@@ -529,6 +544,9 @@
     for (int i = 0; i < TP; ++i)
 #pragma unroll
         for (int j = 0; j < TQ; ++j) acc[i][j] = f32x4{0.f, 0.f, 0.f, 0.f};
+    f32x4 acc0[3];
+#pragma unroll
+    for (int i = 0; i < 3; ++i) acc0[i] = f32x4{0.f, 0.f, 0.f, 0.f};
     float dbias[LAST2 ? TO2 : 1][4], dbe0[TO1][4], dga0[TO1][4];
 #pragma unroll
     for (int i = 0; i < (LAST2 ? TO2 : 1); ++i)
@@ -610,6 +628,25 @@
                     D1[io][t] = v;
                 }
             }
+            unsigned onm = 0;
+            if constexpr (ONE) {
+                if (one) {
+#pragma unroll
+                    for (int t = 0; t < 4; ++t) {
+                        float mx[4];
+#pragma unroll
+                        for (int r = 0; r < 4; ++r) {
+                            const float h = D1[0][t][r];
+                            const bool on = val[t] && h > 0.f;
+                            onm |= on ? 1u << (4 * t + r) : 0u;
+                            mx[r] = on ? (h - mu0[0][r]) * is0[0][r] : 0.f;
+                        }
+                        *reinterpret_cast<float4*>(lds_x0 + (16 * t + c) * 16 + 4 * q) = make_float4(mx[0], mx[1], mx[2], mx[3]);
+#pragma unroll
+                        for (int kb = 0; kb < 4; ++kb) lds_q0[(16 * t + c) * 16 + 4 * kb + q] = kb < KB1 ? bks[t][kb < KB1 ? kb : 0] : 0.f;
+                    }
+                }
+            }
             f32x4 dy1[TO1][4];
             if constexpr (NL == 2) {
                 f32x4 Y1[TO1][4], dp2[TO2][4];
@@ -760,6 +797,37 @@
             }
             __builtin_amdgcn_fence(__ATOMIC_ACQUIRE, "wavefront");
             __builtin_amdgcn_wave_barrier();
+            if constexpr (ONE) {
+                if (one) {
+#pragma unroll
+                    for (int t = 0; t < 4; ++t) {
+                        float mg[4], mm[4];
+#pragma unroll
+                        for (int r = 0; r < 4; ++r) {
+                            const bool on = (onm >> (4 * t + r)) & 1u;
+                            mg[r] = on ? dy1[0][t][r] : 0.f;
+                            mm[r] = on ? 1.f : 0.f;
+                        }
+                        *reinterpret_cast<float4*>(lds_p + (16 * t + c) * PS + 4 * q) = make_float4(mg[0], mg[1], mg[2], mg[3]);
+                        *reinterpret_cast<float4*>(lds_q + (16 * t + c) * QS + 4 * q) = make_float4(mm[0], mm[1], mm[2], mm[3]);
+                    }
+                    __builtin_amdgcn_fence(__ATOMIC_RELEASE, "wavefront");
+                    __builtin_amdgcn_wave_barrier();
+                    const float* rg = lds_p + q * PS + c;
+                    const float* rm = lds_q + q * QS + c;
+                    const float* rx = lds_x0 + q * 16 + c;
+                    const float* ri = lds_q0 + q * 16 + c;
+#pragma unroll 4
+                    for (int st = 0; st < 16; ++st) {
+                        const float vg = rg[st * 4 * PS], vx = rx[st * 4 * 16], vm = rm[st * 4 * QS], vi = ri[st * 4 * 16];
+                        acc0[0] = __builtin_amdgcn_mfma_f32_16x16x4f32(vg, vi, acc0[0], 0, 0, 0);
+                        acc0[1] = __builtin_amdgcn_mfma_f32_16x16x4f32(vx, vi, acc0[1], 0, 0, 0);
+                        acc0[2] = __builtin_amdgcn_mfma_f32_16x16x4f32(vm, vi, acc0[2], 0, 0, 0);
+                    }
+                    __builtin_amdgcn_fence(__ATOMIC_ACQUIRE, "wavefront");
+                    __builtin_amdgcn_wave_barrier();
+                }
+            }
         }
         if (n_items_dbg == 1) { SASTAMP(3); }
     }
@@ -768,7 +836,8 @@
     SACOUNT(9, n_steps_dbg);
 
     constexpr int NW = PO * QK, NB = LAST2 ? C2 : 0, NG = LAST2 ? 2 * C1 : 0;
-    static_assert(NW + NB + NG <= Acc::LDS_FLOATS, "a wave's image fits its staging region");
+    constexpr int N0 = ONE ? C1 * QK0 : 0;
+    static_assert(NW + NB + NG + 3 * N0 <= WAVE_LDS, "a wave's image fits its staging region");
     float* slab = lds_p;
 #pragma unroll
     for (int i = 0; i < TP; ++i)
@@ -798,13 +867,34 @@
                 }
             }
     }
+    if constexpr (ONE) {
+        if (one) {
+#pragma unroll
+            for (int i = 0; i < 3; ++i)
+#pragma unroll
+                for (int r = 0; r < 4; ++r)
+                    if (c < QK0) slab[NW + NB + NG + (16 * i + 4 * q + r) * QK0 + c] = acc0[i][r] * a1v[0][r];
+        }
+    }
     SASTAMP(5);
     __syncthreads();
     SASTAMP(6);
     const int img = sn2_grad_image(a.rep_k, a.rep_stride);
-    for (int i = threadIdx.x; i < NW + NB + NG; i += 256) {
-        const float v = (smem[i] + smem[Acc::LDS_FLOATS + i]) + (smem[2 * Acc::LDS_FLOATS + i] + smem[3 * Acc::LDS_FLOATS + i]);
+    const int nred = NW + NB + NG + (one ? (a.frozen ? N0 : 3 * N0) : 0);
+    for (int i = threadIdx.x; i < nred; i += 256) {
+        const float v = (smem[i] + smem[WAVE_LDS + i]) + (smem[2 * WAVE_LDS + i] + smem[3 * WAVE_LDS + i]);
         if (v == 0.f) continue;
+        if (ONE && i >= NW + NB + NG) {
+            const int j = i - (NW + NB + NG);
+            if (j < N0) {
+                const int o = j / QK0, k = j - o * QK0;
+                if (k < CIN) SN2_FLUSH_ADD(&a.dW0[img + o * CIN + k], v);
+                else SN2_FLUSH_ADD(&a.db0[img + o], v);
+            } else {
+                SN2_FLUSH_ADD(&a.ws[(size_t)(blockIdx.x % SN2_SA_BWD_WS_REPLICAS) * 2 * N0 + (j - N0)], v);
+            }
+            continue;
+        }
         if (i < NW) {
             if constexpr (LAST2) {
                 SN2_FLUSH_ADD(&a.dW1[img + i], v);
@@ -870,10 +960,8 @@
 template int sa_mfma_launch_fwd<32, 1, 64, 64, 1>(const sn2_sa*, int, hipStream_t, int*);
 
 template <int CF, int NL, int C1, int C2, int PASS>
-int sa_mfma_launch_bwd(const sn2_sa* p, hipStream_t st) {
-    constexpr int CIN = CF + 3;
-    constexpr bool LAST2 = NL == 2 && PASS == 2;
-    using Acc = OuterAcc<(LAST2 ? C2 : C1), (LAST2 ? C1 : CIN + 1)>;
+int sa_mfma_launch_bwd(const sn2_sa* p, float* ws, hipStream_t st) {
+    if (ws && (PASS != 2 || NL != 2 || p->blk[0].mma_bf16)) return SN2_EINVAL;
     SaBwdArgs a;
     a.B = p->B; a.Nsrc = p->Nsrc; a.M = p->M; a.cap = p->cap; a.feat_stride = p->feat_stride; a.spos_stride = p->spos_stride;
     a.feat = p->feat; a.spos = p->spos; a.cpos = p->cpos; a.nbr = p->nbr; a.cnt = p->cnt; a.order = p->order; a.total = p->total;
@@ -889,11 +977,13 @@
     a.dW0 = k0.dW; a.db0 = k0.db; a.dW1 = k1.dW; a.db1 = k1.db; a.dgamma0_out = k0.dgamma; a.dbeta0_out = k0.dbeta;
     a.rep_k = k0.grad_replicas; a.rep_stride = k0.grad_replica_stride;
     a.dfeat = p->dfeat;
+    a.ws = ws;
     int blocks = sn2_cdiv((long)p->B * p->M, 16);
     static const int occ_env = getenv("SN2_SA_BWD_OCC") ? atoi(getenv("SN2_SA_BWD_OCC")) : 0;
     const int occ = occ_env > 0 ? occ_env : (CF == 8 ? 2 : 1);
     if (blocks > sn2_cu_count() * occ) blocks = sn2_cu_count() * occ;
-    const size_t lds = (size_t)Acc::LDS_FLOATS * 4 * sizeof(float);
+    const size_t lds = (size_t)(p->blk[0].mma_bf16 ? SaBwdLds<CF, NL, C1, C2, PASS, true>::FLOATS
+                                                   : SaBwdLds<CF, NL, C1, C2, PASS, false>::FLOATS) * 4 * sizeof(float);
     auto kern = p->blk[0].mma_bf16 ? &sa_mfma_bwd_kernel<CF, NL, C1, C2, PASS, true> : &sa_mfma_bwd_kernel<CF, NL, C1, C2, PASS, false>;
     if (lds > 48 * 1024)
         (void)hipFuncSetAttribute(reinterpret_cast<const void*>(kern), hipFuncAttributeMaxDynamicSharedMemorySize, (int)lds);
@@ -901,7 +991,7 @@
     SN2_RETURN_LAUNCH();
 }
 
-template int sa_mfma_launch_bwd<8, 2, 16, 16, 2>(const sn2_sa*, hipStream_t);
-template int sa_mfma_launch_bwd<8, 2, 16, 16, 3>(const sn2_sa*, hipStream_t);
-template int sa_mfma_launch_bwd<16, 1, 32, 32, 3>(const sn2_sa*, hipStream_t);
-template int sa_mfma_launch_bwd<32, 1, 64, 64, 3>(const sn2_sa*, hipStream_t);
+template int sa_mfma_launch_bwd<8, 2, 16, 16, 2>(const sn2_sa*, float*, hipStream_t);
+template int sa_mfma_launch_bwd<8, 2, 16, 16, 3>(const sn2_sa*, float*, hipStream_t);
+template int sa_mfma_launch_bwd<16, 1, 32, 32, 3>(const sn2_sa*, float*, hipStream_t);
+template int sa_mfma_launch_bwd<32, 1, 64, 64, 3>(const sn2_sa*, float*, hipStream_t);
diff --git a/stratanet2_vegetation_coverage_maps_amd/hip_ops.py b/stratanet2_vegetation_coverage_maps_amd/hip_ops.py
--- a/stratanet2_vegetation_coverage_maps_amd/hip_ops.py
+++ b/stratanet2_vegetation_coverage_maps_amd/hip_ops.py
@@ -627,8 +627,11 @@
     _call("sn2_sa_order_group", _ptr(cnt), G, B, M, _ptr(out_all), stride, _stream(), key="sn2_sa_order")
 
 
+SA_BWD_WS_WORDS = 32 * 2 * 16 * 12
+
+
 def sa_desc(blocks, feat, cf, spos, cpos_aos, nbr, cnt, total, B, Nsrc, M, ext, arg, out, dout=None, dfeat=None,
-            with_grads=False, order=None) -> SA:
+            with_grads=False, order=None, bwd_ws=None) -> SA:
     cap = nbr.shape[1]
     cl = blocks[-1].cout
     feat_stride = _chk_rows(feat, F32, B * Nsrc, cf, "feat")
@@ -654,7 +657,9 @@
         _chk(dout, F32, (B * M, cl), "dout")
     if dfeat is not None:
         _chk(dfeat, F32, (B * Nsrc, cf), "dfeat")
-    d.dout, d.dfeat = _ptr(dout), _ptr(dfeat)
+    if bwd_ws is not None:
+        _chk(bwd_ws, F32, (SA_BWD_WS_WORDS,), "bwd_ws")
+    d.dout, d.dfeat, d.bwd_ws = _ptr(dout), _ptr(dfeat), _ptr(bwd_ws)
     return d
 
 
diff --git a/stratanet2_vegetation_coverage_maps_amd/point_net2.py b/stratanet2_vegetation_coverage_maps_amd/point_net2.py
--- a/stratanet2_vegetation_coverage_maps_amd/point_net2.py
+++ b/stratanet2_vegetation_coverage_maps_amd/point_net2.py
@@ -585,9 +585,10 @@
                                        drop_p=self.drop))
         return cov, proba, s
 
-    def _sa1_desc(self, s, dout=None, g=False):
+    def _sa1_desc(self, s, dout=None, g=False, bwd_ws=None):
         return ops.sa_desc(s.b_sa1, s.rows0[:, 0:8], 8, s.rows0[:, 8:12], s.pos1_aos, s.nbr1, s.cnt1, s.tot1, s.B, s.N,
-                           s.M1, s.ext1, s.arg1, s.x1, dout=dout, dfeat=None, with_grads=g, order=getattr(s, "ord1", None))
+                           s.M1, s.ext1, s.arg1, s.x1, dout=dout, dfeat=None, with_grads=g, order=getattr(s, "ord1", None),
+                           bwd_ws=bwd_ws)
 
     def _sa2_desc(self, s, dout=None, dfeat=None, g=False):
         return ops.sa_desc(s.b_sa2, s.x1, 16, s.pos1_aos, s.pos2_aos, s.nbr2, s.cnt2, s.tot2, s.B, s.M1, s.M2, s.ext2,
@@ -614,7 +615,7 @@
         B, N, M1, M2 = s.B, s.N, s.M1, s.M2
         params = self._params()
         sizes = OrderedDict(dy2=B * M1 * 36, dy3=B * M2 * 64, dx1=B * M1 * 16, dx2=B * M2 * 32, dx3=B * 64,
-                            dy_sa3=B * M2 * 64)
+                            dy_sa3=B * M2 * 64, sa1_ws=ops.SA_BWD_WS_WORDS)
         flat, buf, views, images, arena = self._grad_arena(params, sizes, dev)
 
         def attach(bb):
@@ -658,7 +659,7 @@
                                  views[id(bn_sa3.weight)], views[id(bn_sa3.bias)])
         ops.fp_backward(self._sa3_desc(s, dy=dy_sa3, dsrc=dx2, with_grads=True, bn_sums_done=bn_ok[3:4]))
         ops.sa_backward(self._sa2_desc(s, dout=dx2, dfeat=dx1, g=True))
-        ops.sa_backward(self._sa1_desc(s, dout=dx1, g=True))
+        ops.sa_backward(self._sa1_desc(s, dout=dx1, g=True, bwd_ws=buf["sa1_ws"]))
         if getattr(self, "defer_grad_reduce", False):
             self._grad_images_pending = (arena,) + tuple(images)
         else:
diff --git a/stratanet2_vegetation_coverage_maps_amd/point_net2_3sa.py b/stratanet2_vegetation_coverage_maps_amd/point_net2_3sa.py
--- a/stratanet2_vegetation_coverage_maps_amd/point_net2_3sa.py
+++ b/stratanet2_vegetation_coverage_maps_amd/point_net2_3sa.py
@@ -288,7 +288,7 @@
         B, N, M1, M2, M3 = s.B, s.N, s.M1, s.M2, s.M3
         params = list(self.parameters())
         sizes = OrderedDict(dy2=B * M1 * 36, dy3=B * M2 * 64, dy4=B * M3 * 64, dx1=B * M1 * 16, dx2=B * M2 * 32,
-                            dx3=B * M3 * 64, dxg=B * 64, dy_sa4=B * M3 * 64)
+                            dx3=B * M3 * 64, dxg=B * 64, dy_sa4=B * M3 * 64, sa1_ws=ops.SA_BWD_WS_WORDS)
         flat, buf, views, images, arena = self._grad_arena(params, sizes, dev)
         for bb in s.b_sa1 + s.b_sa2 + s.b_sa3 + [s.b_sa4, s.b_fp4, s.b_fp3, s.b_fp2, s.b_fp1]:
             bb.grads = (views[id(bb.lin.weight)], views[id(bb.lin.bias)], views[id(bb.bn.weight)], views[id(bb.bn.bias)])
@@ -332,7 +332,7 @@
         ops.fp_backward(self._sa4_desc(s, dy=dy_sa4, dsrc=dx3, with_grads=True))
         ops.sa_backward(self._sa3l_desc(s, dout=dx3, dfeat=dx2, g=True))
         ops.sa_backward(self._sa2_desc(s, dout=dx2, dfeat=dx1, g=True))
-        ops.sa_backward(self._sa1_desc(s, dout=dx1, g=True))
+        ops.sa_backward(self._sa1_desc(s, dout=dx1, g=True, bwd_ws=buf["sa1_ws"]))
         ops.grad_reduce(arena, flat.numel(), images)
         s.flat_grad = flat
         self._last_flat_grad = flat
```

Result: faster. 23470 plots/s (median of 6 runs) (+1.7%).
